# kakaoenterprise/JORLDY

Measured on AMD Instinct MI355X. Metric: env_steps_per_s (PPO CartPole sync, W=8 workers/GPU, T=128), higher is better.
Workload: dtype f32

## Files before the change

include/jorldy_hip.h:

```cpp
#ifndef JORLDY_HIP_H
#define JORLDY_HIP_H

#include <stdint.h>

#ifdef __cplusplus
extern "C" {
#endif

#define JH_ABI_VERSION 2

typedef enum {
  JH_OK = 0,
  JH_ERR_HIP = -1,
  JH_ERR_ARG = -2,
  JH_ERR_STATE = -3,
  JH_ERR_NOMEM = -4,
  JH_ERR_NODEVICE = -5
} jh_status;

typedef enum { JH_U8 = 0, JH_F32 = 1, JH_I64 = 2, JH_F64 = 3, JH_I32 = 4 } jh_dtype;

typedef struct jh_ctx jh_ctx;
typedef struct jh_store jh_store;
typedef struct jh_per jh_per;
// ... 89 lines not shown
                       const float* d_adv, const float* d_ret, const float* d_value_old, const float* d_logp_old, float eps_clip, float vf_coef,
                       float ent_coef, float* d_grad_heads, float* d_dv2, float* d_critic_sums, float* d_stats, jh_stream stream);
int jh_ppo_critic_select_strided(jh_ctx* ctx, int32_t B, const float* d_critic_sums, float vf_coef, float ent_coef, float* d_grad_value, int32_t ldv,
                                 const float* d_dv2, const float* d_stats_local, float* d_stats, jh_stream stream);
int jh_heads_unpack(jh_ctx* ctx, int64_t rows, int32_t A, const float* d_packed, int32_t ld, float* d_h0, float* d_h1, float* d_value, jh_stream stream);
int jh_policy_act_discrete(jh_ctx* ctx, int32_t W, int32_t A, const float* d_heads, int32_t ld, uint64_t seed, uint64_t counter, int32_t training,
                           int64_t* d_action, jh_stream stream);

#define JH_TD_DOUBLE 1
#define JH_TD_PER 2
int jh_td_loss(jh_ctx* ctx, int32_t B, int32_t A, int32_t n_step, int32_t flags, const float* d_q,
               const float* d_q_next_online, const float* d_q_next_target, const float* d_action,
               const float* d_reward, const float* d_done, const float* d_weights, float gamma, float alpha,
               float* d_grad_q, float* d_prio, float* d_stats, jh_stream stream);

int jh_mdqn_loss(jh_ctx* ctx, int32_t B, int32_t A, const float* d_q, const float* d_q_target, const float* d_q_next_target,
                 const float* d_action, const float* d_reward, const float* d_done, float gamma, float alpha, float tau, float l_0,
                 float* d_grad_q, float* d_stats, jh_stream stream);

#define JH_C51_DOUBLE 1
#define JH_C51_PER 2
#define JH_C51_SHIFT_MAX 4
int jh_c51_loss(jh_ctx* ctx, int32_t B, int32_t A, int32_t K, int32_t n_step, int32_t flags, const float* d_logit,
                const float* d_next_logit_online, const float* d_target_logit, const float* d_action,
                const float* d_reward, const float* d_done, const float* d_weights, float v_min, float v_max,
                float gamma, float alpha, float* d_grad_logit, float* d_prio, float* d_kl, float* d_stats,
                jh_stream stream);

int jh_value_act(jh_ctx* ctx, int32_t N, int32_t A, int32_t K, const float* d_logits, float v_min, float v_max,
                 const float* h_eps, const double* h_u, const int64_t* h_rand_action, int64_t* d_action,
                 float* d_q_taken, float* d_q_all, jh_stream stream);

int jh_qr_loss(jh_ctx* ctx, int32_t B, int32_t A, int32_t N, const float* d_logit, const float* d_next_logit_online,
               const float* d_target_logit, const float* d_action, const float* d_reward, const float* d_done,
               const float* d_tau, float gamma, float* d_grad_logit, float* d_stats, jh_stream stream);

int jh_quantile_act(jh_ctx* ctx, int32_t R, int32_t A, int32_t N, const float* d_logits, const float* h_eps, const double* h_u,
                    const int64_t* h_rand_action, int64_t* d_action, float* d_q_taken, float* d_q_all, jh_stream stream);

typedef struct jh_iqnnet jh_iqnnet;
int64_t jh_iqnnet_param_count_for(int32_t state_size, int32_t hidden, int32_t embedding_dim, int32_t num_sample, int32_t action_size);
int jh_iqnnet_create(jh_ctx* ctx, int32_t state_size, int32_t hidden, int32_t embedding_dim, int32_t num_sample, int32_t action_size,
                     int32_t max_batch, float* d_params, float* d_target, float* d_grads, float* d_m, float* d_v, jh_iqnnet** out);
void jh_iqnnet_destroy(jh_iqnnet* n);
int32_t jh_iqnnet_segment_count(void);
int jh_iqnnet_segment(const jh_iqnnet* n, int32_t i, int64_t* offset, int32_t* rows, int32_t* cols);
int jh_iqnnet_set_hyper(jh_iqnnet* n, double lr, double beta1, double beta2, double eps, int64_t step, jh_stream stream);
int jh_iqnnet_set_lr(jh_iqnnet* n, double lr, jh_stream stream);
int jh_iqnnet_sync_target(jh_iqnnet* n, jh_stream stream);
int jh_iqnnet_forward(jh_iqnnet* n, int32_t which, const float* d_x, int32_t rows, const float* d_tau, float* d_logits, jh_stream stream);
int jh_iqnnet_learn_forward(jh_iqnnet* n, const float* d_x, int32_t B, const float* d_tau, float* d_logits, jh_stream stream);
int jh_iqnnet_learn_forward_m(jh_iqnnet* n, const float* d_x, int32_t B, const float* d_tau, float* d_logits, jh_stream stream);
int jh_iqnnet_backward(jh_iqnnet* n, const float* d_g, jh_stream stream);
int jh_iqnnet_optim_step(jh_iqnnet* n, float max_norm, jh_stream stream);
int jh_iqn_cos_features(jh_ctx* ctx, int64_t rows, int32_t E, const float* d_tau, float* d_out, jh_stream stream);
int jh_iqn_hadamard(jh_ctx* ctx, int32_t B, int32_t N, int32_t H, const float* d_psi, const float* d_phi, float* d_out, jh_stream stream);
int jh_iqn_hadamard_backward(jh_ctx* ctx, int32_t B, int32_t N, int32_t H, const float* d_grad_embed, const float* d_psi, const float* d_phi,
                             float* d_grad_phi_pre, float* d_grad_psi_pre, jh_stream stream);
int jh_iqn_loss(jh_ctx* ctx, int32_t B, int32_t A, int32_t N, const float* d_logit, const float* d_next_logit_online,
                const float* d_target_logit, const float* d_action, const float* d_reward, const float* d_done, const float* d_tau,
                float gamma, float* d_grad_logit, float* d_stats, jh_stream stream);
int jh_miqn_loss(jh_ctx* ctx, int32_t B, int32_t A, int32_t N, const float* d_logit, const float* d_logit_again, const float* d_target_logit,
                 const float* d_action, const float* d_reward, const float* d_done, const float* d_tau, float gamma, float alpha, float tau_e,
                 float l_0, float* d_grad_logit, float* d_stats, jh_stream stream);
int jh_iqn_act(jh_ctx* ctx, int32_t R, int32_t A, int32_t N, const float* d_logits, const float* h_eps, const double* h_u,
               const int64_t* h_rand_action, int64_t* d_action, float* d_q_taken, float* d_q_all, jh_stream stream);

typedef struct jh_pponet jh_pponet;
int64_t jh_pponet_param_count(int32_t S, int32_t H, int32_t A, int32_t continuous);
int jh_pponet_create(jh_ctx* ctx, int32_t S, int32_t H, int32_t A, int32_t continuous, int32_t max_rows,
                     float* d_params, float* d_grads, float* d_m, float* d_v, uint64_t seed, jh_pponet** out);
void jh_pponet_destroy(jh_pponet* n);
int jh_pponet_set_hyper(jh_pponet* n, double lr, double beta1, double beta2, double eps, double step, jh_stream stream);
int jh_pponet_set_lr(jh_pponet* n, double lr, jh_stream stream);
int jh_pponet_forward(jh_pponet* n, int32_t B, const float* d_x, const int64_t* d_idx, float* d_head0,
                      float* d_head1, float* d_value, jh_stream stream);
int jh_pponet_backward(jh_pponet* n, int32_t B, const float* d_x, const int64_t* d_idx, const float* d_g_head0,
                       const float* d_g_head1, const float* d_g_value, jh_stream stream);
int jh_pponet_adam_step(jh_pponet* n, float max_norm, float* d_norm_out, jh_stream stream);
int jh_pponet_ppo_update(jh_pponet* n, int32_t B, const float* d_x, const int64_t* d_idx, const float* d_action,
                         const float* d_adv, const float* d_ret, const float* d_value_old, const float* d_logp_old,
                         float eps_clip, float vf_coef, float ent_coef, float max_norm, int32_t do_adam, float* d_stats,
                         jh_stream stream);
int jh_pponet_ppo_update_rows(jh_pponet* n, int32_t B, const float* d_x, const int64_t* d_idx, const float* d_action, const float* d_adv, const float* d_ret,
                              const float* d_value_old, const float* d_logp_old, float eps_clip, float vf_coef, float ent_coef, float max_norm,
                              int32_t do_adam, float* d_stats, jh_stream stream);
int jh_pponet_ppo_update_dp_begin(jh_pponet* n, int32_t B, const float* d_x, const int64_t* d_idx, const float* d_action, const float* d_adv,
                                  const float* d_ret, const float* d_value_old, const float* d_logp_old, float eps_clip, float vf_coef,
                                  float ent_coef, float* d_critic_sums, jh_stream stream);
int jh_pponet_ppo_update_dp_end(jh_pponet* n, int32_t B, const float* d_x, const int64_t* d_idx, const float* d_critic_sums, float vf_coef,
                                float ent_coef, float* d_stats, jh_stream stream);
struct jh_peer;
int jh_pponet_ppo_update_dp_end_peer(jh_pponet* n, struct jh_peer* peer, int32_t B, const float* d_x, const int64_t* d_idx, float* d_critic_sums,
                                     float vf_coef, float ent_coef, float* d_stats, jh_stream stream);
void* jh_pponet_hyper_ptr(jh_pponet* n);
int jh_pponet_act_rng(jh_pponet* n, uint64_t* seed, uint64_t* counter, int32_t set);
int jh_pponet_act_discrete(jh_pponet* n, int32_t W, const float* h_obs, int64_t* h_action, float* h_logits_out,
                           float* h_value_out, int32_t training, jh_stream stream);
int jh_pponet_act_continuous(jh_pponet* n, int32_t W, const float* h_obs, float* h_action, float* h_mu_raw_out,
                             float* h_log_std_raw_out, float* h_value_out, int32_t training, jh_stream stream);

int jh_cartpole_create(int32_t W, uint64_t seed, jh_cartpole** out);
void jh_cartpole_destroy(jh_cartpole* e);
int jh_cartpole_obs(const jh_cartpole* e, float* h_obs );
int jh_cartpole_step(jh_cartpole* e, const int64_t* h_action , float* h_next_obs ,
                     float* h_reward , uint8_t* h_done );

typedef struct jh_control jh_control;
int jh_control_create(int32_t W, int32_t S, int32_t A, uint64_t seed, jh_control** out);
void jh_control_destroy(jh_control* e);
int jh_control_obs(const jh_control* e, float* h_obs );
int jh_control_step(jh_control* e, const float* h_action , float* h_next_obs ,
                    float* h_reward , uint8_t* h_done );

typedef struct jh_collector jh_collector;

typedef struct jh_env_vtbl {
  int32_t W, S, A, continuous;
  int (*obs)(void* env, int32_t r0, int32_t r1, float* h_obs);
  int (*step)(void* env, int32_t r0, int32_t r1, const void* h_action, float* h_next_obs, float* h_reward, uint8_t* h_done);
  void* (*fork_alloc)(void* env, int32_t rows);
  void (*fork_free)(void* scratch);
  void (*copy_row)(void* dst, int32_t di, const void* src, int32_t si);
} jh_env_vtbl;
int jh_collector_create_env(jh_ctx* ctx, jh_pponet* net, const jh_env_vtbl* vt, void* env, jh_store* store, const int32_t* cols,
                            jh_collector** out);

int jh_collector_create(jh_ctx* ctx, jh_pponet* net, jh_cartpole* env, jh_store* store, const int32_t* cols,
                        jh_collector** out);
int jh_collector_create_control(jh_ctx* ctx, jh_pponet* net, jh_control* env, jh_store* store, const int32_t* cols,
                                jh_collector** out);
void jh_collector_destroy(jh_collector* c);
int jh_collector_run(jh_collector* c, int32_t T, int32_t training, jh_stream stream);
int jh_collector_set_capture(jh_collector* c, float* d_h0, float* d_h1, float* d_value, float* d_next_value, int64_t rows);
int jh_collector_begin(jh_collector* c, int32_t T, jh_stream stream);
int jh_collector_loop(jh_collector* c, int32_t training, jh_stream stream);
int jh_collector_set_ride_along(jh_collector* c, int32_t slot, const void* d_src_mapped, void* d_dst, int64_t bytes);
int jh_collector_prelaunch(jh_collector* c, int32_t T, jh_stream stream);
int jh_collector_stats(jh_collector* c, double* act_us_per_step, double* env_us_per_step, int32_t reset);
int jh_collector_stats_detail(jh_collector* c, double* out6);

int jh_normal_fill(jh_ctx* ctx, int64_t n, float* d_out, uint64_t* d_state, jh_stream stream);

typedef struct jh_rbnet jh_rbnet;
int64_t jh_rbnet_param_count_for(int32_t kind, int32_t head_cnn, int32_t channels_or_state_size, int32_t height, int32_t width,
                                 int32_t hidden, int32_t action_size, int32_t num_support);
int jh_rbnet_create(jh_ctx* ctx, int32_t kind, int32_t head_cnn, int32_t channels_or_state_size, int32_t height, int32_t width,
                    int32_t hidden, int32_t action_size, int32_t num_support, int32_t max_batch, float* d_params,
                    float* d_target, float* d_grads, float* d_m, float* d_v, jh_rbnet** out);
void jh_rbnet_destroy(jh_rbnet* n);
int64_t jh_rbnet_param_count(const jh_rbnet* n);
int32_t jh_rbnet_segment_count(void);
int jh_rbnet_segment(const jh_rbnet* n, int32_t i, int64_t* offset, int32_t* rows, int32_t* cols);
int64_t jh_rbnet_noise_len(const jh_rbnet* n);
int jh_rbnet_set_hyper(jh_rbnet* n, double lr, double beta1_or_alpha, double beta2, double eps, int64_t step, int32_t centered,
                       jh_stream stream);
int jh_rbnet_set_lr(jh_rbnet* n, double lr, jh_stream stream);
int jh_rbnet_sync_target(jh_rbnet* n, jh_stream stream);
int jh_rbnet_forward(jh_rbnet* n, int32_t which, const void* d_x, int32_t x_dtype, int32_t rows, const float* d_noise,
                     float* d_logits, jh_stream stream);
int jh_rbnet_forward_keep(jh_rbnet* n, const void* d_x, int32_t x_dtype, int32_t B, float* d_logits, jh_stream stream);
int jh_rbnet_learn_forward(jh_rbnet* n, const void* d_x, int32_t x_dtype, int32_t B, const float* d_noise, float* d_logits,
                           jh_stream stream);
int jh_rbnet_reserve_target_rows(jh_rbnet* n, int32_t rows);
int jh_rbnet_learn_forward_m(jh_rbnet* n, const void* d_x, int32_t x_dtype, int32_t B, const float* d_noise, float* d_logits,
                             jh_stream stream);
// ... 75 lines not shown
```

jorldy_amd/_lib.py:

```python
import ctypes as C
import os

_HERE = os.path.dirname(os.path.abspath(__file__))
LIB_PATH = os.path.join(_HERE, "csrc", "libjorldy_hip.so")

JH_U8, JH_F32, JH_I64, JH_F64, JH_I32 = 0, 1, 2, 3, 4
JH_TD_DOUBLE, JH_TD_PER = 1, 2
JH_C51_DOUBLE, JH_C51_PER, JH_C51_SHIFT_MAX = 1, 2, 4


class JhError(RuntimeError):
    pass


class ColDesc(C.Structure):
    _fields_ = [("dtype", C.c_int32), ("elems", C.c_int64)]


_vp, _i32, _i64, _f32, _f64 = C.c_void_p, C.c_int32, C.c_int64, C.c_float, C.c_double
_pp = C.POINTER(C.c_void_p)

_PROTOS = {
    "jh_abi_version": (C.c_int, []),
    "jh_stream_abort_capture": (C.c_int, [_vp]),
# ... 3 lines not shown
    "jh_ctx_destroy": (None, [_vp]),
    "jh_ctx_sync": (C.c_int, [_vp, _vp]),
    "jh_ctx_local_cpulist": (C.c_int, [_vp, C.c_char_p, _i64]),
    "jh_prof_enable": (C.c_int, [_i32]),
    "jh_prof_report": (C.c_int, [C.c_char_p, _i64]),
    "jh_prof_calibrate": (C.c_int, [_i32, _vp]),
    "jh_calib_stream": (C.c_int, [_vp, _vp, _i64, _i32, _vp, _vp]),
    "jh_host_wait_marks": (C.c_int, [_vp, _vp, _i32, _f32, _f64]),
    "jh_host_wait_words": (C.c_int, [_vp, _vp, _i32, C.c_uint32, _f64]),
    "jh_np_legacy_shuffles": (C.c_int, [_vp, _vp, _vp, _i64, _i32, _vp]),
    "jh_pinned_alloc": (C.c_int, [_vp, _i64, _pp, _pp]),
    "jh_pinned_free": (None, [_vp]),
    "jh_store_create": (C.c_int, [_vp, _i64, _i32, C.POINTER(ColDesc), _pp]),
    "jh_store_destroy": (None, [_vp]),
    "jh_store_push": (C.c_int, [_vp, _i64, _pp, _vp]),
    "jh_store_push_device": (C.c_int, [_vp, _i64, _pp, _vp]),
    "jh_store_stage_begin": (C.c_int, [_vp, _i64, _pp]),
    "jh_store_stage_commit": (C.c_int, [_vp, _vp]),
    "jh_store_write_rows": (C.c_int, [_vp, _i64, _vp, _pp, _vp]),
    "jh_store_gather": (C.c_int, [_vp, _i64, _vp, _i64, _i32, C.POINTER(_i32), _pp, C.POINTER(_i32), _vp]),
    "jh_store_col_ptr": (_vp, [_vp, _i32]),
    "jh_store_size": (_i64, [_vp]),
    "jh_store_index": (_i64, [_vp]),
    "jh_store_capacity": (_i64, [_vp]),
    "jh_store_clear": (None, [_vp]),
    "jh_store_set_position": (C.c_int, [_vp, _i64, _i64]),
    "jh_per_create": (C.c_int, [_vp, _i64, _f64, _pp]),
    "jh_per_destroy": (None, [_vp]),
    "jh_per_push": (C.c_int, [_vp, _i64, _vp, _vp]),
    "jh_per_push_device": (C.c_int, [_vp, _i64, _vp, _vp]),
    "jh_per_update": (C.c_int, [_vp, _i64, _vp, _vp, _i32, _vp]),
    "jh_per_sample": (C.c_int, [_vp, _i64, _f64, _i64, _vp, _vp, _vp, _vp, _vp, _vp, _vp]),
    "jh_per_state": (C.c_int, [_vp, C.POINTER(_f64), C.POINTER(_f64), C.POINTER(_i64), C.POINTER(_i64), _vp]),
    "jh_per_tree_ptr": (_vp, [_vp]),
    "jh_per_shard_stats": (C.c_int, [_vp, _i64, _vp, _vp]),
    "jh_per_weights_sharded": (C.c_int, [_vp, _i64, _f64, _vp, _i32, _vp, _vp, _vp]),
    "jh_per_tree_size": (_i64, [_vp]),
    "jh_per_load": (C.c_int, [_vp, _vp, _f64, _i64, _i64]),
    "jh_per_dump": (C.c_int, [_vp, _vp, _vp]),
    "jh_gae": (C.c_int, [_vp, _i32, _i32, _f32, _f32, _vp, _vp, _vp, _vp, _vp, _vp, _i32, _vp]),
    "jh_ppo_minibatch_rows": (C.c_int, [_vp, _i64, _vp, _i32, _vp, _vp, _vp, _vp]),
    "jh_mean_f32": (C.c_int, [_vp, _i64, _vp, _vp, _vp]),
    "jh_logp_discrete": (C.c_int, [_vp, _i64, _i32, _vp, _vp, _vp, _vp]),
    "jh_logp_continuous": (C.c_int, [_vp, _i64, _i32, _vp, _vp, _vp, _vp, _vp]),
    "jh_ppo_loss_discrete": (C.c_int, [_vp, _i32, _i32, _vp, _vp, _vp, _vp, _vp, _vp, _vp, _vp, _f32, _f32, _f32, _vp, _vp, _vp, _vp]),
    "jh_ppo_loss_continuous": (C.c_int, [_vp, _i32, _i32, _vp, _vp, _vp, _vp, _vp, _vp, _vp, _vp, _vp, _f32, _f32, _f32, _vp, _vp, _vp, _vp, _vp]),
    "jh_normal_fill": (C.c_int, [_vp, _i64, _vp, _vp, _vp]),
    "jh_value_act": (C.c_int, [_vp, _i32, _i32, _i32, _vp, _f32, _f32, _vp, _vp, _vp, _vp, _vp, _vp, _vp]),
    "jh_td_loss": (C.c_int, [_vp, _i32, _i32, _i32, _i32, _vp, _vp, _vp, _vp, _vp, _vp, _vp, _f32, _f32, _vp, _vp, _vp, _vp]),
    "jh_c51_loss": (C.c_int, [_vp, _i32, _i32, _i32, _i32, _i32, _vp, _vp, _vp, _vp, _vp, _vp, _vp, _f32, _f32, _f32, _f32, _vp, _vp, _vp, _vp, _vp]),
    "jh_mdqn_loss": (C.c_int, [_vp, _i32, _i32, _vp, _vp, _vp, _vp, _vp, _vp, _f32, _f32, _f32, _f32, _vp, _vp, _vp]),
    "jh_qr_loss": (C.c_int, [_vp, _i32, _i32, _i32, _vp, _vp, _vp, _vp, _vp, _vp, _vp, _f32, _vp, _vp, _vp]),
    "jh_quantile_act": (C.c_int, [_vp, _i32, _i32, _i32, _vp, _vp, _vp, _vp, _vp, _vp, _vp, _vp]),
    "jh_iqnnet_param_count_for": (_i64, [_i32, _i32, _i32, _i32, _i32]),
    "jh_iqnnet_create": (C.c_int, [_vp, _i32, _i32, _i32, _i32, _i32, _i32, _vp, _vp, _vp, _vp, _vp, _pp]),
    "jh_iqnnet_destroy": (None, [_vp]),
    "jh_iqnnet_segment_count": (_i32, []),
    "jh_iqnnet_segment": (C.c_int, [_vp, _i32, C.POINTER(_i64), C.POINTER(_i32), C.POINTER(_i32)]),
    "jh_iqnnet_set_hyper": (C.c_int, [_vp, _f64, _f64, _f64, _f64, _i64, _vp]),
    "jh_iqnnet_set_lr": (C.c_int, [_vp, _f64, _vp]),
    "jh_iqnnet_sync_target": (C.c_int, [_vp, _vp]),
    "jh_iqnnet_forward": (C.c_int, [_vp, _i32, _vp, _i32, _vp, _vp, _vp]),
    "jh_iqnnet_learn_forward": (C.c_int, [_vp, _vp, _i32, _vp, _vp, _vp]),
    "jh_iqnnet_learn_forward_m": (C.c_int, [_vp, _vp, _i32, _vp, _vp, _vp]),
    "jh_iqnnet_backward": (C.c_int, [_vp, _vp, _vp]),
    "jh_iqnnet_optim_step": (C.c_int, [_vp, _f32, _vp]),
    "jh_iqn_cos_features": (C.c_int, [_vp, _i64, _i32, _vp, _vp, _vp]),
    "jh_iqn_hadamard": (C.c_int, [_vp, _i32, _i32, _i32, _vp, _vp, _vp, _vp]),
    "jh_iqn_hadamard_backward": (C.c_int, [_vp, _i32, _i32, _i32, _vp, _vp, _vp, _vp, _vp, _vp]),
    "jh_iqn_loss": (C.c_int, [_vp, _i32, _i32, _i32, _vp, _vp, _vp, _vp, _vp, _vp, _vp, _f32, _vp, _vp, _vp]),
    "jh_miqn_loss": (C.c_int, [_vp, _i32, _i32, _i32, _vp, _vp, _vp, _vp, _vp, _vp, _vp, _f32, _f32, _f32, _f32, _vp, _vp, _vp]),
    "jh_iqn_act": (C.c_int, [_vp, _i32, _i32, _i32, _vp, _vp, _vp, _vp, _vp, _vp, _vp, _vp]),
    "jh_pponet_param_count": (_i64, [_i32, _i32, _i32, _i32]),
    "jh_pponet_create": (C.c_int, [_vp, _i32, _i32, _i32, _i32, _i32, _vp, _vp, _vp, _vp, C.c_uint64, _pp]),
    "jh_pponet_destroy": (None, [_vp]),
    "jh_pponet_set_hyper": (C.c_int, [_vp, _f64, _f64, _f64, _f64, _f64, _vp]),
    "jh_pponet_set_lr": (C.c_int, [_vp, _f64, _vp]),
    "jh_pponet_hyper_ptr": (_vp, [_vp]),
    "jh_pponet_act_rng": (C.c_int, [_vp, C.POINTER(C.c_uint64), C.POINTER(C.c_uint64), _i32]),
    "jh_pponet_forward": (C.c_int, [_vp, _i32, _vp, _vp, _vp, _vp, _vp, _vp]),
    "jh_pponet_backward": (C.c_int, [_vp, _i32, _vp, _vp, _vp, _vp, _vp, _vp]),
    "jh_pponet_adam_step": (C.c_int, [_vp, _f32, _vp, _vp]),
    "jh_pponet_ppo_update": (C.c_int, [_vp, _i32, _vp, _vp, _vp, _vp, _vp, _vp, _vp, _f32, _f32, _f32, _f32, _i32, _vp, _vp]),
    "jh_pponet_ppo_update_rows": (C.c_int, [_vp, _i32, _vp, _vp, _vp, _vp, _vp, _vp, _vp, _f32, _f32, _f32, _f32, _i32, _vp, _vp]),
    "jh_ppo_loss_deferred": (C.c_int, [_vp, _i32, _i32, _i32, _vp, _vp, _vp, _vp, _vp, _vp, _vp, _vp, _vp, _f32, _f32, _f32, _vp, _vp, _vp, _vp, _vp, _vp, _vp]),
    "jh_ppo_loss_packed": (C.c_int, [_vp, _i32, _i32, _i32, _vp, _i32, _vp, _vp, _vp, _vp, _vp, _vp, _f32, _f32, _f32, _vp, _vp, _vp, _vp, _vp]),
    "jh_ppo_critic_select_strided": (C.c_int, [_vp, _i32, _vp, _f32, _f32, _vp, _i32, _vp, _vp, _vp, _vp]),
    "jh_heads_unpack": (C.c_int, [_vp, _i64, _i32, _vp, _i32, _vp, _vp, _vp, _vp]),
    "jh_policy_act_discrete": (C.c_int, [_vp, _i32, _i32, _vp, _i32, C.c_uint64, C.c_uint64, _i32, _vp, _vp]),
    "jh_ppo_critic_select_rows": (C.c_int, [_vp, _i32, _vp, _f32, _f32, _vp, _vp, _vp, _vp, _vp]),
    "jh_pponet_ppo_update_dp_begin": (C.c_int, [_vp, _i32, _vp, _vp, _vp, _vp, _vp, _vp, _vp, _f32, _f32, _f32, _vp, _vp]),
    "jh_pponet_ppo_update_dp_end": (C.c_int, [_vp, _i32, _vp, _vp, _vp, _f32, _f32, _vp, _vp]),
    "jh_pponet_ppo_update_dp_end_peer": (C.c_int, [_vp, _vp, _i32, _vp, _vp, _vp, C.c_float, C.c_float, _vp, _vp]),
    "jh_pponet_act_discrete": (C.c_int, [_vp, _i32, _vp, _vp, _vp, _vp, _i32, _vp]),
    "jh_pponet_act_continuous": (C.c_int, [_vp, _i32, _vp, _vp, _vp, _vp, _vp, _i32, _vp]),
    "jh_control_create": (C.c_int, [_i32, _i32, _i32, C.c_uint64, _pp]),
    "jh_control_destroy": (None, [_vp]),
    "jh_control_obs": (C.c_int, [_vp, _vp]),
    "jh_control_step": (C.c_int, [_vp, _vp, _vp, _vp, _vp]),
    "jh_collector_create_control": (C.c_int, [_vp, _vp, _vp, _vp, C.POINTER(_i32), _pp]),
    "jh_collector_create": (C.c_int, [_vp, _vp, _vp, _vp, C.POINTER(_i32), _pp]),
    "jh_collector_create_env": (C.c_int, [_vp, _vp, _vp, _vp, _vp, C.POINTER(_i32), _pp]),
    "jh_collector_destroy": (None, [_vp]),
    "jh_rbnet_param_count_for": (_i64, [_i32, _i32, _i32, _i32, _i32, _i32, _i32, _i32]),
    "jh_rbnet_create": (C.c_int, [_vp, _i32, _i32, _i32, _i32, _i32, _i32, _i32, _i32, _i32, _vp, _vp, _vp, _vp, _vp, _pp]),
    "jh_rbnet_destroy": (None, [_vp]),
    "jh_rbnet_param_count": (_i64, [_vp]),
    "jh_rbnet_segment_count": (_i32, []),
    "jh_rbnet_segment": (C.c_int, [_vp, _i32, C.POINTER(_i64), C.POINTER(_i32), C.POINTER(_i32)]),
    "jh_rbnet_noise_len": (_i64, [_vp]),
    "jh_rbnet_set_hyper": (C.c_int, [_vp, _f64, _f64, _f64, _f64, _i64, _i32, _vp]),
    "jh_rbnet_optim_step": (C.c_int, [_vp, _i32, _f32, _vp]),
    "jh_rbnet_set_lr": (C.c_int, [_vp, _f64, _vp]),
    "jh_rbnet_sync_target": (C.c_int, [_vp, _vp]),
    "jh_rbnet_forward": (C.c_int, [_vp, _i32, _vp, _i32, _i32, _vp, _vp, _vp]),
    "jh_rbnet_forward_keep": (C.c_int, [_vp, _vp, _i32, _i32, _vp, _vp]),
    "jh_rbnet_learn_forward": (C.c_int, [_vp, _vp, _i32, _i32, _vp, _vp, _vp]),
    "jh_rbnet_learn_forward_m": (C.c_int, [_vp, _vp, _i32, _i32, _vp, _vp, _vp]),
    "jh_rbnet_reserve_target_rows": (C.c_int, [_vp, _i32]),
    "jh_rbnet_prepare_noise": (C.c_int, [_vp, _vp, _vp]),
    "jh_rbnet_learn_trunk": (C.c_int, [_vp, _vp, _i32, _i32, _vp]),
    "jh_rbnet_learn_heads": (C.c_int, [_vp, _i32, _vp, _vp, _vp]),
    "jh_rbnet_backward": (C.c_int, [_vp, _vp, _vp]),
    "jh_rbnet_backward_deferred": (C.c_int, [_vp, _vp, _vp]),
    "jh_rbnet_flush_grads": (C.c_int, [_vp, _vp]),
    "jh_rbnet_learn_heads_raw": (C.c_int, [_vp, _i32, _vp, _vp]),
    "jh_rbnet_c51_step": (C.c_int, [_vp, _vp, _i32, _i32, _i32, _vp, _vp, _vp, _vp, _vp, _f32, _f32, _f32, _f32, _vp, _vp, _vp, _vp, _vp]),
    "jh_rbnet_adam_step": (C.c_int, [_vp, _vp]),
    "jh_tgemm_dense": (C.c_int, [_vp, _i32, _i32, _i32, _vp, _i32, _i32, _vp, _i32, _i32, _vp, _i32, _i32, _vp, _vp, _i32, _vp, _vp]),
    "jh_tgemm_dense_group": (C.c_int, [_vp, _i32, _i32, _i32, _i32, _vp, _vp, _vp, _vp]),
    "jh_tgemm_set_cfg": (C.c_int, [C.c_char_p]),
    "jh_ring_create": (C.c_int, [_vp, _i64, _i32, C.POINTER(ColDesc), _i32, _pp]),
    "jh_ring_destroy": (None, [_vp]),
    "jh_ring_produce": (C.c_int, [_vp, _i64, _pp, _vp, _i32]),
    "jh_ring_drain": (C.c_int, [_vp, _vp, _vp, _i64, _vp, C.POINTER(_i64)]),
    "jh_ring_consume_host": (C.c_int, [_vp, _i64, _pp, _vp, C.POINTER(_i64)]),
    "jh_ring_reclaim": (C.c_int, [_vp, _i32]),
    "jh_ring_stats": (C.c_int, [_vp, C.POINTER(_i64), C.POINTER(_i64), C.POINTER(_f64)]),
    "jh_feed_create": (C.c_int, [_vp, _i32, _i32, _i64, _i32, _f32, _i64, _i64, _pp]),
    "jh_feed_destroy": (None, [_vp]),
    "jh_feed_tick": (C.c_int, [_vp, _vp, _vp, _vp, _vp, _vp, _vp, _vp, _f64, _vp, _vp, _vp, _vp, _vp, _vp, C.POINTER(_i32), _vp]),
    "jh_feed_push_stacks": (C.c_int, [_vp, _vp, _vp, _vp, _vp]),
    "jh_feed_push_frames": (C.c_int, [_vp, _vp, _vp, _vp, _vp, _vp]),
    "jh_feed_emit": (C.c_int, [_vp, _vp, _vp, _vp, _vp, _f64, _vp, _vp, _vp, _vp, _vp, _vp, C.POINTER(_i32), _vp]),
    "jh_feed_state": (C.c_int, [_vp, C.POINTER(_i32), C.POINTER(_i64), _vp]),
    "jh_feed_state_bytes": (_i64, [_vp]),
    "jh_feed_save": (C.c_int, [_vp, _vp, _i64, _vp]),
    "jh_feed_load": (C.c_int, [_vp, _vp, _i64, _vp]),
    "jh_collector_stats": (C.c_int, [_vp, C.POINTER(_f64), C.POINTER(_f64), _i32]),
    "jh_collector_run": (C.c_int, [_vp, _i32, _i32, _vp]),
    "jh_collector_stats_detail": (C.c_int, [_vp, C.POINTER(_f64)]),
    "jh_collector_set_capture": (C.c_int, [_vp, _vp, _vp, _vp, _vp, _i64]),
    "jh_collector_prelaunch": (C.c_int, [_vp, _i32, _vp]),
    "jh_collector_begin": (C.c_int, [_vp, _i32, _vp]),
    "jh_collector_loop": (C.c_int, [_vp, _i32, _vp]),
    "jh_collector_set_ride_along": (C.c_int, [_vp, _i32, _vp, _vp, _i64]),
    "jh_cartpole_create": (C.c_int, [_i32, C.c_uint64, _pp]),
    "jh_cartpole_destroy": (None, [_vp]),
    "jh_cartpole_obs": (C.c_int, [_vp, _vp]),
    "jh_cartpole_step": (C.c_int, [_vp, _vp, _vp, _vp, _vp]),
    "jh_comm_unique_id": (C.c_int, [_vp]),
    "jh_comm_create": (C.c_int, [_vp, _i32, _i32, _vp, _pp]),
    "jh_comm_destroy": (None, [_vp]),
    "jh_comm_info": (C.c_int, [_vp, C.POINTER(_i32), C.POINTER(_i32)]),
    "jh_comm_allreduce_mean_f32": (C.c_int, [_vp, _vp, _i64, _vp]),
    "jh_comm_broadcast": (C.c_int, [_vp, _vp, _i64, _i32, _vp]),
# ... 74 lines not shown
```

jorldy_amd/core/agent/ppo.py:

```python
import os

import numpy as np
import torch

from ... import np_rng, ops
from ..buffer import RolloutBuffer
from ..network import Network
from ..optimizer import Optimizer
from .base import BaseAgent


MAX_HEAD_OUTPUTS = 40
NATIVE_ELIGIBLE = ("PPO runs on libjorldy_hip only: network in {discrete_policy_value, continuous_policy_value}, head='mlp', int state_size, "
                   "hidden_size % 16 == 0, optim_config name 'adam' without weight_decay / amsgrad, and action_size + 1 (discrete) or "
                   f"2 * action_size + 1 (continuous) <= {MAX_HEAD_OUTPUTS} head outputs (config.ppo.cartpole, config.ppo.mujoco on all its envs; up to 8 outputs "
                   "-- CartPole, Hopper -- on the four-launch minibatch update and the persistent acting kernel, beyond that on the separate calls / the tiled engine); "
                   "head='cnn' with a (C, H, W) state_size and network 'discrete_policy_value' runs on the convolutional engine (core/agent/ppo_cnn.py: config.ppo.atari, ppo.procgen)")


class PPO(BaseAgent):

    def __new__(cls, *args, **kwargs):
        if cls is PPO and kwargs.get("head", args[4] if len(args) > 4 else "mlp") == "cnn":
            from .ppo_cnn import PPOConv
# ... 149 lines not shown
        if os.environ.get("JH_PPO_MAPPED_STATS", "1") == "1":
            pin = ops.PinnedBuffer((n_upd + 1, 8), np.float32, self.device.index)
            pin.np[:] = 0.0
            st["stats_pin"] = pin
            st["stats"] = ops._wrap_device(pin.dev_ptr.value, (n_upd + 1, 8), torch.float32, self.device, owner=pin)
        E = self.n_epoch
        if self.fused_update and all(self._net.fused_ok(min(B, M - o)) for o in range(0, M, B)):
            srcs = [st["tr"]["state"], st["tr"]["action"], st["adv"], st["ret"], st["value"], st["logp_old"]]
            st["mb"] = [f(E * M, int(t.numel() // M)) for t in srcs]
            st["rows"] = ops.MinibatchRows(srcs, st["mb"])
        st["idx_pin"] = [ops.PinnedBuffer((self.n_epoch * M,), np.int64, self.device.index) for _ in range(2)]
        st["idx_alias"] = [ops._wrap_device(p.dev_ptr.value, (self.n_epoch * M,), torch.int64, self.device, owner=p) for p in st["idx_pin"]]
        st["idx_ev"] = [None, None]
        st["idx_k"] = 0
        st["idx_ready"] = False
        self._stats = st["stats"]
        return st

    def _capture_targets(self, M):
        self._grow_native(2 * M if 2 * M <= 8192 else M)
        if self._static is None or self._static["M"] != M:
            self._drop_rides()
            self._static, self._graphs = self._alloc_static(M), {}
        st = self._static
        return st["h0"], st["h1"], st["value"], st["next_value"]

    def _drop_rides(self):
        if self._ride is not None:
            self._ride.clear_rides()
        self._ride_wait.clear()
        if self._static is not None:
            self._static["idx_ready"] = False

    def _upload_idx(self, st, draw, ride=False):
        k = st["idx_k"]
        st["idx_k"] = 1 - k
        if st["idx_ev"][k] is not None:
            st["idx_ev"][k].synchronize()
            st["idx_ev"][k] = None
        ok = draw(st["idx_pin"][k].np)
        if ok is False:
            return False
        if ride and self._ride is not None:
            self._ride.ride_along(0, st["idx_pin"][k].dev_ptr.value, st["idx"].data_ptr(), st["idx"].numel() * 8, keep=(st["idx_pin"][k], st["idx"]))
            self._ride_wait["idx"] = k
            return True
        self._ride_wait.pop("idx", None)
        st["idx"].copy_(st["idx_alias"][k])
        ev = torch.cuda.Event()
        ev.record()
        st["idx_ev"][k] = ev
        return True

    def _enqueue_learn(self, st):
        self._enqueue_pre(st)
        self._enqueue_main(st)

    def _enqueue_pre(self, st, captured=False):
        net, M = self._net, st["M"]
        cont = net.cont
        tr = st["tr"]
        self.memory._store.gather(st["arange"], as_float=True, out={k: tr[k] for k in tr})
        if captured:
            pass
        elif 2 * M <= min(net.max_rows, 8192):
            net.forward(st["x_all"], out=(st["h0_all"], st["h1_all"], st["v_all"]))
        else:
            net.forward(tr["next_state"], out=(st["nh0"], st["nh1"], st["next_value"]))
            net.forward(tr["state"], out=(st["h0"], st["h1"], st["value"]))
        if cont:
            logp_old = ops.logp_continuous(st["h0"], st["h1"], tr["action"], out=st["logp_old"])
        else:
            logp_old = ops.logp_discrete(st["h0"], tr["action"], out=st["logp_old"])
        adv, ret = ops.gae(tr["reward"], tr["done"], st["value"], st["next_value"], self.n_step, self.gamma, self._lambda, self.use_standardization,
                           out=(st["adv"], st["ret"]))
        ops.mean_into(ret, st["stats"][st["n_upd"], 0:1])

    def _enqueue_main(self, st):
        net, M, B = self._net, st["M"], self.batch_size
        cont = net.cont
        tr, adv, ret, logp_old = st["tr"], st["adv"], st["ret"], st["logp_old"]
        k = 0
        if "rows" in st:
            xs, acts, advs, rets, vals, lps = st["rows"](st["idx"])
            exact = self.grad_sync is not None and self.dp_exact_critic
            if exact and "critic_sums" not in st:
                st["critic_sums"] = torch.zeros(st["n_upd"], 2, dtype=torch.float32, device=self.device)
            for e in range(self.n_epoch):
                for offset in range(0, M, B):
                    o0, o1 = e * M + offset, e * M + min(offset + B, M)
                    if exact:
                        net.ppo_update_dp(xs[o0:o1], None, acts[o0:o1], advs[o0:o1], rets[o0:o1], vals[o0:o1], lps[o0:o1], self.epsilon_clip, self.vf_coef,
                                          self.ent_coef, st["stats"][k], self.grad_sync.reduce_flat, st["critic_sums"][k],
                                          peer=getattr(getattr(self.grad_sync, "transport", None), "peer", None))
                    else:
                        net.ppo_update(xs[o0:o1], None, acts[o0:o1], advs[o0:o1], rets[o0:o1], vals[o0:o1], lps[o0:o1], self.epsilon_clip, self.vf_coef,
                                       self.ent_coef, self.clip_grad_norm, st["stats"][k], do_adam=self.grad_sync is None)
                    if self.grad_sync is not None:
                        self.grad_sync.reduce_flat(net.grads)
                        net.adam_step(self.clip_grad_norm)
                    k += 1
            return
        exact = self.grad_sync is not None and self.dp_exact_critic
        if exact and "dp_work" not in st:
            st["dp_work"] = torch.zeros(st["n_upd"], B + 16, dtype=torch.float32, device=self.device)
        onepass = not exact and os.environ.get("JH_PPO_ONEPASS", "1") == "1"
        for e in range(self.n_epoch):
            for offset in range(0, M, B):
                b = min(B, M - offset)
                idx = st["idx"][e * M + offset : e * M + offset + b]
                if onepass:
                    net.ppo_update_rows(tr["state"], idx, tr["action"], adv, ret, st["value"], logp_old, self.epsilon_clip, self.vf_coef, self.ent_coef, self.clip_grad_norm,
                                        st["stats"][k], do_adam=self.grad_sync is None)
                    if self.grad_sync is not None:
                        self.grad_sync.reduce_flat(net.grads)
                        net.adam_step(self.clip_grad_norm)
                    k += 1
                    continue
                if cont:
                    mu, ls, vp = net.forward(tr["state"], idx=idx, out=(st["mb_h0"][:b], st["mb_h1"][:b], st["mb_v"][:b]))
                    if exact:
                        g_mu, g_ls, g_v = ops.ppo_loss_dp(mu, ls, vp, idx, tr["action"], adv, ret, st["value"], logp_old, self.epsilon_clip, self.vf_coef, self.ent_coef,
                                                          st["stats"][k], self.grad_sync.reduce_flat, st["dp_work"][k])
                    else:
                        g_mu, g_ls, g_v, _ = ops.ppo_loss_continuous(mu, ls, vp, idx, tr["action"], adv, ret, st["value"], logp_old, self.epsilon_clip, self.vf_coef, self.ent_coef, stats=st["stats"][k])
                    net.backward(tr["state"], idx, g_mu, g_ls, g_v)
                else:
                    z, vp = net.forward(tr["state"], idx=idx, out=(st["mb_h0"][:b], None, st["mb_v"][:b]))
                    if exact:
                        g_z, g_v = ops.ppo_loss_dp(z, None, vp, idx, tr["action"], adv, ret, st["value"], logp_old, self.epsilon_clip, self.vf_coef, self.ent_coef,
                                                   st["stats"][k], self.grad_sync.reduce_flat, st["dp_work"][k])
                    else:
                        g_z, g_v, _ = ops.ppo_loss_discrete(z, vp, idx, tr["action"], adv, ret, st["value"], logp_old, self.epsilon_clip, self.vf_coef, self.ent_coef, stats=st["stats"][k])
                    net.backward(tr["state"], idx, g_z, None, g_v)
                if self.grad_sync is not None:
                    self.grad_sync.reduce_flat(net.grads)
                net.adam_step(self.clip_grad_norm)
                k += 1

    def _learn_native(self):
        self._learn_launch()
        return self._learn_finish()

    def early_ready(self):
        st = self._static
        return bool(st is not None and st["idx_ready"] and ("one", True) in getattr(self, "_graphs", {}) and self._predraw is not None and self._predraw.valid)

    def _learn_launch(self, allow_capture=True):
        M = self.memory.size
        self._grow_native(2 * M if 2 * M <= 8192 else M)
        if self._static is None or self._static["M"] != M:
            self._drop_rides()
            self._static, self._graphs = self._alloc_static(M), {}
        st = self._static
        E = self.n_epoch
        captured = self._captured == M
        self._captured = 0
        rode, self._ride_done = self._ride_done, False
        if self._ride_wait and not rode:
            if "lr" in self._ride_wait:
                self._net.set_lr(float(self._lr_word.np[0]))
            if "idx" in self._ride_wait and st["idx_ready"]:
                st["idx"].copy_(st["idx_alias"][self._ride_wait["idx"]])
        self._ride_wait.clear()

        def shuffles():
            self._upload_idx(st, lambda out: np_rng.epoch_shuffles(M, E, out))

        pin = st.get("stats_pin")
        if pin is not None:
            pin.np[st["n_upd"] - 1, 2] = -1.0
            pin.np[st["n_upd"] - 1, 7] = -1.0
        graphable = (self.use_graph and not ops._PROF["on"] and not ops._PROF["lib"] and not getattr(self, "_graph_failed", False)
                     and (self.grad_sync is None or (self.graph_with_collective and getattr(self.grad_sync, "capturable", True))))
        have_idx = bool(st["idx_ready"]) and self._predraw is not None and self._predraw.commit(M, E)
        st["idx_ready"] = False
        split = not have_idx and os.environ.get("JH_PPO_SPLIT_GRAPH", "1") == "1"
        key = ("split" if split else "one", captured)
        graphs = getattr(self, "_graphs", None)
        if graphs is None:
            graphs = self._graphs = {}
        warm = getattr(self, "_warm_keys", None)
        if warm is None:
            warm = self._warm_keys = set()
# ... 163 lines not shown
```

jorldy_amd/csrc/jh_common.h:

```cpp
#pragma once
#include <hip/hip_runtime.h>
#include <math.h>
#include <stdint.h>
#include <stdio.h>
#include <string.h>

#include <deque>
#include <mutex>
#include <string>
#include <vector>

#include "../../include/jorldy_hip.h"

#define JH_EXPORT extern "C" __attribute__((visibility("default")))

std::string& jh_err_slot();
int jh_fail(int code, const char* fmt, ...);

#define JH_HIP(expr)                                                                          \
  do {                                                                                        \
    hipError_t _e = (expr);                                                                   \
    if (_e != hipSuccess)                                                                     \
      return jh_fail(JH_ERR_HIP, "%s:%d %s -> %s", __FILE__, __LINE__, #expr, hipGetErrorString(_e)); \
  } while (0)
// ... 65 lines not shown
int jh_ctx_slab_release(jh_ctx* ctx, jh_pinned_slab* slab, hipStream_t stream);
int jh_ctx_scratch(jh_ctx* ctx, size_t bytes, void** out);
struct jh_draws {
  jh_pinned_slab* slab;
  const float* eps;
  const double* u;
  const int64_t* rand_action;
};
int jh_ctx_stage_draws(jh_ctx* ctx, size_t rows, const float* h_eps, const double* h_u, const int64_t* h_rand_action, jh_draws* out);

struct jh_store {
  jh_ctx* ctx = nullptr;
  int64_t capacity = 0;
  int n_cols = 0;
  std::vector<jh_col_desc> cols;
  std::vector<void*> dev;
  std::vector<size_t> row_bytes;
  int64_t index = 0;
  int64_t counter = 0;
  jh_pinned_slab* staged = nullptr;
  int64_t staged_n = 0;
  std::vector<size_t> staged_off;
};

int jh_store_append(jh_store* s, int64_t n, const void* const* cols, hipMemcpyKind kind, hipStream_t st);
int jh_store_stage_commit_extra(jh_store* s, int n_extra, const void* const* x_src, void* const* x_dst, const int64_t* x_bytes, hipStream_t st);
bool jh_store_commit_is_one_launch(const jh_store* s, int64_t n);
int jh_store_stage_abort(jh_store* s, hipStream_t st);
int jh_store_stage_commit_gated(jh_store* s, int n_extra, const void* const* x_src, void* const* x_dst, const int64_t* x_bytes, const unsigned* gate,
                                unsigned gate_val, hipStream_t st);

struct jh_cartpole {
  int W = 0;
  std::vector<double> s;
  std::vector<int64_t> t;
  std::vector<uint64_t> rng;
};

struct jh_control {
  int W = 0, S = 0, A = 0;
  std::vector<double> s;
  std::vector<int64_t> t;
  std::vector<uint64_t> rng;
};

void jh_cartpole_obs_rows(const jh_cartpole* e, int r0, int r1, float* h_obs);
void jh_cartpole_step_rows(jh_cartpole* e, int r0, int r1, const int64_t* h_action, float* h_next_obs, float* h_reward, uint8_t* h_done);
struct jh_control;
void jh_control_obs_rows(const jh_control* e, int r0, int r1, float* h_obs);
void jh_control_step_rows(jh_control* e, int r0, int r1, const float* h_action, float* h_next_obs, float* h_reward, uint8_t* h_done);

struct jh_pponet {
  jh_ctx* ctx = nullptr;
  int S = 0, H = 0, A = 0, cont = 0, max_rows = 0;
  int n_out = 0;
  int gld = 8;
  int64_t n_params = 0;
  float *params = nullptr, *grads = nullptr, *m = nullptr, *v = nullptr;
  int64_t o_w1, o_b1, o_w2, o_b2, o_wh0, o_bh0, o_wh1, o_bh1, o_wv, o_bv;
  float *h1 = nullptr, *h2 = nullptr, *dh1 = nullptr, *dh2 = nullptr;
  float* g_all = nullptr;
  float* dv2 = nullptr;
  float* stats_tmp = nullptr;
  int max_act_rows = 0;
  float *obs_pin_h = nullptr, *obs_pin_d = nullptr;
  float *part_pin_h = nullptr, *part_pin_d = nullptr;
  unsigned *flag_pin_h = nullptr, *flag_pin_d = nullptr;
  unsigned act_seq = 0;
  float *act_out_h = nullptr, *act_out_d = nullptr;
  uint64_t act_seed = 0, act_ctr = 0;
  float* fwd_part = nullptr;
  float* part_w1 = nullptr;
  float* ssq_part = nullptr;
  float* norm_partial = nullptr;
  int norm_slots = 0;
  float* hyper = nullptr;
  float* upd_ws = nullptr;
  size_t upd_floats = 0;
  float* xg = nullptr;
  float* tg_ws = nullptr;
  size_t tg_ws_floats = 0;
  unsigned* tg_cnt = nullptr;
  int tg_cnt_slots = 0;
};

static inline uint64_t jh_mix64(uint64_t x) {
  x += 0x9E3779B97F4A7C15ull;
  x = (x ^ (x >> 30)) * 0xBF58476D1CE4E5B9ull;
  x = (x ^ (x >> 27)) * 0x94D049BB133111EBull;
  return x ^ (x >> 31);
}
static inline double jh_u01_of(uint64_t key) { return (double)(jh_mix64(key) >> 11) * (1.0 / 9007199254740992.0); }

static inline int64_t jh_sample_discrete(const jh_pponet* n, const float* z, int wq, int training) {
  const int A = n->A;
  int act = 0;
  float mx = z[0];
  for (int k = 1; k < A; ++k)
    if (z[k] > mx) { mx = z[k]; act = k; }
  if (!training) return act;
  float e[40], se = 0.f;
  for (int k = 0; k < A; ++k) { e[k] = expf(z[k] - mx); se += e[k]; }
  const float u = (float)jh_u01_of(n->act_seed * 0x100000001B3ull + n->act_ctr * 0x9E3779B97F4A7C15ull + (uint64_t)wq) * se;
  float c = 0.f;
  act = A - 1;
  for (int k = 0; k < A; ++k) {
    c += e[k];
    if (u < c) { act = k; break; }
  }
  return act;
}

static inline void jh_sample_continuous(const jh_pponet* n, const float* z, int wq, int training, float* action) {
  const int A = n->A;
  for (int k = 0; k < A; ++k) {
    const float mu = fminf(fmaxf(z[k], -5.f), 5.f);
    float v = mu;
    if (training) {
      const float sd = expf(tanhf(z[A + k]));
      const uint64_t key = n->act_seed * 0x100000001B3ull + n->act_ctr * 0x9E3779B97F4A7C15ull + (uint64_t)wq * 64u + (uint64_t)k;
      const double u1 = 1.0 - jh_u01_of(key * 2 + 1), u2 = jh_u01_of(key * 2 + 2);
      v = mu + sd * (float)(sqrt(-2.0 * log(u1)) * cos(6.283185307179586 * u2));
    }
    action[k] = tanhf(v);
  }
}

enum {
  JH_HY_LR = 0, JH_HY_B1 = 1, JH_HY_B2 = 2, JH_HY_EPS = 3, JH_HY_STEP = 4,
  JH_HY_BC1 = 5,
  JH_HY_BC2S = 6,
  JH_HY_OMB1 = 7,
  JH_HY_OMB2 = 8,
  JH_HY_B1D = 10,
  JH_HY_B2D = 12,
  JH_HY_FLOATS = 16
};
static inline void jh_hyper_fill(float* h, double lr, double beta1, double beta2, double eps, double step) {
  h[JH_HY_LR] = (float)lr; h[JH_HY_B1] = (float)beta1; h[JH_HY_B2] = (float)beta2; h[JH_HY_EPS] = (float)eps; h[JH_HY_STEP] = (float)step;
  h[JH_HY_BC1] = 0.f; h[JH_HY_BC2S] = 0.f;
  h[JH_HY_OMB1] = (float)(1.0 - beta1); h[JH_HY_OMB2] = (float)(1.0 - beta2); h[9] = 0.f;
  memcpy(h + JH_HY_B1D, &beta1, 8); memcpy(h + JH_HY_B2D, &beta2, 8);
  h[14] = h[15] = 0.f;
}

#ifdef __HIPCC__
__device__ __forceinline__ void jh_adam_bias_corrections(const float* hyper, float t, float& bc1, float& bc2s) {
  const double b1 = *reinterpret_cast<const double*>(hyper + JH_HY_B1D), b2 = *reinterpret_cast<const double*>(hyper + JH_HY_B2D);
  bc1 = (float)(1.0 - pow(b1, (double)t));
  bc2s = (float)sqrt(1.0 - pow(b2, (double)t));
}
__device__ __forceinline__ void jh_adam_advance(float* hyper) {
  const float t = hyper[JH_HY_STEP] + 1.f;
  float bc1, bc2s;
  jh_adam_bias_corrections(hyper, t, bc1, bc2s);
  hyper[JH_HY_STEP] = t;
  hyper[JH_HY_BC1] = bc1;
  hyper[JH_HY_BC2S] = bc2s;
}
__device__ __forceinline__ float jh_wave_sum(float v) {
#pragma unroll
  for (int o = 32; o > 0; o >>= 1) v += __shfl_xor(v, o, 64);
  return v;
}
__device__ __forceinline__ double jh_wave_sum(double v) {
#pragma unroll
  for (int o = 32; o > 0; o >>= 1) v += __shfl_xor(v, o, 64);
  return v;
}
__device__ __forceinline__ float jh_wave_max(float v) {
#pragma unroll
  for (int o = 32; o > 0; o >>= 1) v = fmaxf(v, __shfl_xor(v, o, 64));
  return v;
}
__device__ __forceinline__ float jh_wave_min(float v) {
#pragma unroll
  for (int o = 32; o > 0; o >>= 1) v = fminf(v, __shfl_xor(v, o, 64));
  return v;
}
__device__ __forceinline__ double jh_wave_max(double v) {
#pragma unroll
  for (int o = 32; o > 0; o >>= 1) v = fmax(v, __shfl_xor(v, o, 64));
  return v;
}
template <typename T, typename Op>
__device__ __forceinline__ T jh_block_reduce(T v, T* red, Op op, T ident) {
  const int lane = threadIdx.x & 63, wid = threadIdx.x >> 6, nw = (blockDim.x + 63) >> 6;
#pragma unroll
  for (int o = 32; o > 0; o >>= 1) v = op(v, __shfl_xor(v, o, 64));
  __syncthreads();
  if (lane == 0) red[wid] = v;
  __syncthreads();
  T r = ident;
  for (int w = 0; w < nw; ++w) r = op(r, red[w]);
  return r;
}
struct JhAdd { template <typename T> __device__ T operator()(T a, T b) const { return a + b; } };
struct JhMax { template <typename T> __device__ T operator()(T a, T b) const { return a > b ? a : b; } };
struct JhMin { template <typename T> __device__ T operator()(T a, T b) const { return a < b ? a : b; } };
#endif
```

jorldy_amd/csrc/jh_mlp.hip:

```cpp
#include "jh_ppo_mb.h"
#include "jh_tgemm.h"
#include "jh_ppo_finish.h"

typedef float f32x4 __attribute__((ext_vector_type(4)));

namespace {
constexpr int kNormBlocks = 256;
constexpr int kNormSlots = kNormBlocks + 256;
constexpr int kMaxHeadOutputs = 40;
}

constexpr int kL1Rows = 16;
__global__ void __launch_bounds__(256) jh_mlp_l1_kernel(int B, int S, int H, const float* __restrict__ x,
                                                        const int64_t* __restrict__ idx, const float* __restrict__ W1,
                                                        const float* __restrict__ b1, float* __restrict__ h1) {
  __shared__ __attribute__((aligned(16))) float sx[kL1Rows][16];
  const int jb = (H + 255) / 256;
  const int rb = blockIdx.x / jb, j = (blockIdx.x - rb * jb) * 256 + threadIdx.x;
  const int b0 = rb * kL1Rows, nb = b0 + kL1Rows < B ? kL1Rows : B - b0;
  const bool lds_rows = S <= 16;
  if (lds_rows) {
    const int rr = threadIdx.x >> 4, sc = threadIdx.x & 15;
    float v = 0.f;
    if (rr < nb && sc < S) {
// ... 351 lines not shown
  if (!on && !(dv2 && fin.partial)) return;
  const int b = on ? (int)(i4 / h4) : 0, k = on ? 4 * (int)(i4 - (int64_t)b * h4) : 0;
  float gv[8];
  float4 w[8];
#pragma unroll
  for (int o = 0; o < 8; ++o) {
    gv[o] = hf.g[o][(size_t)b * hf.ld[o]];
    w[o] = *reinterpret_cast<const float4*>(hf.w[o] + k);
  }
  if (dv2) {
    float w1, w2;
    const float g2 = dv2[b];
    if (fin.partial) {
      float t[6];
      ppo_reduce_partials_wave(fin.partial, fin.nb, t);
      ppo_finish_stats(t[0], t[1], t[2], t[3], t[4], t[5], fin.B, fin.ent_count, fin.vf, fin.ent, w1, w2, (blockIdx.x == 0 && threadIdx.x == 0) ? fin.stats : nullptr);
    } else {
      w1 = mix[0]; w2 = mix[1];
    }
    if (!on) return;
#pragma unroll
    for (int o = 0; o < 8; ++o)
      if (o == ov) gv[o] = w1 * gv[o] + w2 * g2;
  }
  float4 acc = first ? make_float4(0.f, 0.f, 0.f, 0.f) : *reinterpret_cast<const float4*>(dh2 + (size_t)b * H + k);
  const float4 hv = *reinterpret_cast<const float4*>(h2 + (size_t)b * H + k);
  float mine[4] = {0.f, 0.f, 0.f, 0.f};
#pragma unroll
  for (int o = 0; o < 8; ++o) {
    if (o < hf.n) {
      acc.x = fmaf(gv[o], w[o].x, acc.x); acc.y = fmaf(gv[o], w[o].y, acc.y); acc.z = fmaf(gv[o], w[o].z, acc.z); acc.w = fmaf(gv[o], w[o].w, acc.w);
#pragma unroll
      for (int j = 0; j < 4; ++j) mine[j] = (o0 + o == k + j) ? gv[o] : mine[j];
    }
  }
  if (last) acc = make_float4(hv.x > 0.f ? acc.x : 0.f, hv.y > 0.f ? acc.y : 0.f, hv.z > 0.f ? acc.z : 0.f, hv.w > 0.f ? acc.w : 0.f);
  *reinterpret_cast<float4*>(dh2 + (size_t)b * H + k) = acc;
  if (k < gld) {
    float* dst = g_all + (size_t)b * gld + k;
    if (first) {
      *reinterpret_cast<float4*>(dst) = make_float4(mine[0], mine[1], mine[2], mine[3]);
    } else {
#pragma unroll
      for (int j = 0; j < 4; ++j)
        if (k + j >= o0 && k + j < o0 + hf.n) dst[j] = mine[j];
    }
  }
  if (H < gld && k == H - 4) {
    for (int kk = H; kk < gld; kk += 4) {
      float* dst = g_all + (size_t)b * gld + kk;
#pragma unroll
      for (int j = 0; j < 4; ++j) {
        float v = 0.f;
#pragma unroll
        for (int o = 0; o < 8; ++o) v = (o < hf.n && o0 + o == kk + j) ? gv[o] : v;
        if (first || (kk + j >= o0 && kk + j < o0 + hf.n)) dst[j] = v;
      }
    }
  }
}

__global__ void __launch_bounds__(256) jh_gradnorm_kernel(int64_t n, const float* __restrict__ g,
                                                          float* __restrict__ partial, float* __restrict__ hyper) {
  __shared__ float s_red[16];
  float acc = 0.f;
  const int64_t stride = (int64_t)gridDim.x * 256;
  for (int64_t i0 = (int64_t)blockIdx.x * 256 + threadIdx.x; i0 < n; i0 += 8 * stride) {
    float v[8];
#pragma unroll
    for (int u = 0; u < 8; ++u) {
      const int64_t i = i0 + u * stride;
      v[u] = g[i < n ? i : i0];
    }
#pragma unroll
    for (int u = 0; u < 8; ++u)
      if (i0 + u * stride < n) acc = fmaf(v[u], v[u], acc);
  }
  acc = jh_block_reduce(acc, s_red, JhAdd(), 0.f);
  if (threadIdx.x == 0) partial[blockIdx.x] = acc;
  if (blockIdx.x == 0 && threadIdx.x == 0) jh_adam_advance(hyper);
}

template <bool FUSED>
__global__ void __launch_bounds__(256) jh_adam_kernel(int64_t n, float* __restrict__ p, float* __restrict__ g,
                                                      float* __restrict__ m, float* __restrict__ v,
                                                      const float* __restrict__ partial, int n_partial,
                                                      const float* __restrict__ hyper, float max_norm,
                                                      float* __restrict__ norm_out, const float* __restrict__ part,
                                                      int tiles_m, int64_t n_head) {
  __shared__ float s_red[16];
  const int64_t n4 = n >> 2;
  float4 *p4 = reinterpret_cast<float4*>(p), *g4 = reinterpret_cast<float4*>(g), *m4 = reinterpret_cast<float4*>(m), *v4 = reinterpret_cast<float4*>(v);
  const int64_t i_first = (int64_t)blockIdx.x * 256 + threadIdx.x;
  const int64_t i_fc = i_first < n4 ? i_first : 0;
  const float4 pp0 = p4[i_fc], mm0 = m4[i_fc], vv0 = v4[i_fc], gg0 = g4[i_fc];
  float acc = 0.f;
  bool partials_added = false;
  auto add_partials = [&]() {
    const int ia = threadIdx.x, ib = threadIdx.x + 256;
    const float pa = partial[ia < n_partial ? ia : 0], pb = partial[ib < n_partial ? ib : 0];
    acc += ia < n_partial ? pa : 0.f;
    acc += ib < n_partial ? pb : 0.f;
    for (int i = threadIdx.x + 512; i < n_partial; i += 256) acc += partial[i];
    partials_added = true;
  };
  float4 mine = make_float4(0.f, 0.f, 0.f, 0.f);
  const int64_t h4 = n_head >> 2;
  if (FUSED) {
    const float4* part4 = reinterpret_cast<const float4*>(part);
    constexpr int JU = 3, TU = 16;
    for (int64_t j0 = 0; j0 * 256 < h4; j0 += JU) {
      float4 w[JU][TU];
#pragma unroll
      for (int ju = 0; ju < JU; ++ju) {
        const int64_t i = threadIdx.x + 256 * (j0 + ju);
        const int64_t ic = i < h4 ? i : h4 - 1;
#pragma unroll
        for (int tu = 0; tu < TU; ++tu) w[ju][tu] = part4[(size_t)(tu < tiles_m ? tu : tiles_m - 1) * h4 + ic];
      }
      if (!partials_added) add_partials();
#pragma unroll
      for (int ju = 0; ju < JU; ++ju) {
        const int64_t i = threadIdx.x + 256 * (j0 + ju);
        float4 q = make_float4(0.f, 0.f, 0.f, 0.f);
#pragma unroll
        for (int tu = 0; tu < TU; ++tu)
          if (tu < tiles_m) { q.x += w[ju][tu].x; q.y += w[ju][tu].y; q.z += w[ju][tu].z; q.w += w[ju][tu].w; }
        if (i < h4) {
          acc = fmaf(q.x, q.x, acc); acc = fmaf(q.y, q.y, acc); acc = fmaf(q.z, q.z, acc); acc = fmaf(q.w, q.w, acc);
          if (j0 + ju == blockIdx.x) mine = q;
        }
      }
    }
  }
  if (!partials_added) add_partials();
  const float total = sqrtf(jh_block_reduce(acc, s_red, JhAdd(), 0.f));
  const float bc1 = hyper[5], bc2s = hyper[6];
  float coef = 1.f;
  if (max_norm > 0.f) coef = fminf(max_norm / (total + 1e-6f), 1.f);
  if (blockIdx.x == 0 && threadIdx.x == 0 && norm_out) *norm_out = total;
  const float lr = hyper[JH_HY_LR], b2 = hyper[JH_HY_B2], eps = hyper[JH_HY_EPS];
  const float omb1 = hyper[JH_HY_OMB1], omb2 = hyper[JH_HY_OMB2];
  const float step_size = lr / bc1;
  auto upd = [&](float& pi, float& gi_, float& mi_, float& vi_) {
    const float gi = gi_ * coef;
    gi_ = gi;
    const float mi = mi_ + omb1 * (gi - mi_);
    const float vi = vi_ * b2 + omb2 * gi * gi;
    mi_ = mi;
    vi_ = vi;
    const float denom = sqrtf(vi) / bc2s + eps;
    pi = pi - step_size * (mi / denom);
  };
  for (int64_t i = i_first; i < n4; i += (int64_t)gridDim.x * 256) {
    const bool first = i == i_first;
    float4 pp = first ? pp0 : p4[i], mm = first ? mm0 : m4[i], vv = first ? vv0 : v4[i];
    float4 gg = (FUSED && i < h4) ? mine : (first ? gg0 : g4[i]);
    upd(pp.x, gg.x, mm.x, vv.x); upd(pp.y, gg.y, mm.y, vv.y); upd(pp.z, gg.z, mm.z, vv.z); upd(pp.w, gg.w, mm.w, vv.w);
    p4[i] = pp; g4[i] = gg; m4[i] = mm; v4[i] = vv;
  }
  if (blockIdx.x == 0 && threadIdx.x < (int)(n - (n4 << 2))) {
    const int64_t i = (n4 << 2) + threadIdx.x;
    upd(p[i], g[i], m[i], v[i]);
  }
}

static int64_t pponet_layout(jh_pponet* n) {
  const int64_t S = n->S, H = n->H, A = n->A;
  int64_t o = 0;
  n->o_w1 = o; o += H * S;
  n->o_b1 = o; o += H;
  n->o_w2 = o; o += H * H;
  n->o_b2 = o; o += H;
  n->o_wh0 = o; o += A * H;
  n->o_bh0 = o; o += A;
  if (n->cont) {
    n->o_wh1 = o; o += A * H;
    n->o_bh1 = o; o += A;
  } else {
    n->o_wh1 = n->o_bh1 = -1;
  }
  n->o_wv = o; o += H;
  n->o_bv = o; o += 1;
  return o;
}

JH_EXPORT int64_t jh_pponet_param_count(int32_t S, int32_t H, int32_t A, int32_t continuous) {
  jh_pponet t;
  t.S = S; t.H = H; t.A = A; t.cont = continuous;
  return pponet_layout(&t);
}

JH_EXPORT int jh_pponet_create(jh_ctx* ctx, int32_t S, int32_t H, int32_t A, int32_t continuous, int32_t max_rows,
                               float* d_params, float* d_grads, float* d_m, float* d_v, uint64_t seed,
                               jh_pponet** out) {
  JH_ARG(ctx && out && d_params && d_grads && d_m && d_v);
  JH_ARG(S > 0 && A > 0 && max_rows > 0);
  JH_ARG(H >= 16 && H % 16 == 0);
  JH_ARG((continuous ? 2 * A + 1 : A + 1) <= kMaxHeadOutputs);
  JH_HIP(hipSetDevice(ctx->device));
  jh_pponet* n = new jh_pponet();
  n->ctx = ctx; n->S = S; n->H = H; n->A = A; n->cont = continuous ? 1 : 0; n->max_rows = max_rows;
  n->n_params = pponet_layout(n);
  n->params = d_params; n->grads = d_grads; n->m = d_m; n->v = d_v;
  const size_t act = sizeof(float) * (size_t)max_rows * (size_t)H;
  JH_HIP(hipMalloc((void**)&n->h1, act));
  JH_HIP(hipMalloc((void**)&n->h2, act));
  JH_HIP(hipMalloc((void**)&n->dh1, act));
  JH_HIP(hipMalloc((void**)&n->dh2, act));
  n->n_out = continuous ? 2 * A + 1 : A + 1;
  n->gld = n->n_out <= 8 ? 8 : (n->n_out + 3) / 4 * 4;
  JH_HIP(hipMalloc((void**)&n->g_all, sizeof(float) * (size_t)n->gld * (size_t)max_rows));
  n->max_act_rows = max_rows < 1024 ? max_rows : 1024;
  {
    const size_t tiles = (size_t)((n->max_act_rows + 15) / 16) * (size_t)(H / 16);
    JH_HIP(hipHostMalloc((void**)&n->obs_pin_h, sizeof(float) * (size_t)n->max_act_rows * (size_t)S, hipHostMallocMapped));
    JH_HIP(hipHostGetDevicePointer((void**)&n->obs_pin_d, n->obs_pin_h, 0));
    JH_HIP(hipHostMalloc((void**)&n->part_pin_h, sizeof(float) * 8 * (size_t)n->max_act_rows * (size_t)(H / 16), hipHostMallocMapped));
    JH_HIP(hipHostGetDevicePointer((void**)&n->part_pin_d, n->part_pin_h, 0));
    JH_HIP(hipHostMalloc((void**)&n->flag_pin_h, sizeof(unsigned) * tiles, hipHostMallocMapped));
    JH_HIP(hipHostGetDevicePointer((void**)&n->flag_pin_d, n->flag_pin_h, 0));
    memset(n->flag_pin_h, 0, sizeof(unsigned) * tiles);
    n->act_seed = seed;
    if (n->n_out > 8) {
      JH_HIP(hipHostMalloc((void**)&n->act_out_h, sizeof(float) * (size_t)n->max_act_rows * (size_t)n->n_out, hipHostMallocMapped));
      JH_HIP(hipHostGetDevicePointer((void**)&n->act_out_d, n->act_out_h, 0));
    }
  }
  n->tg_ws_floats = (size_t)4 << 20;
  n->tg_cnt_slots = 4096;
  JH_HIP(hipMalloc((void**)&n->xg, sizeof(float) * (size_t)max_rows * (size_t)S));
  JH_HIP(hipMalloc((void**)&n->tg_ws, sizeof(float) * n->tg_ws_floats));
  JH_HIP(hipMalloc((void**)&n->tg_cnt, sizeof(unsigned) * (size_t)n->tg_cnt_slots * kTgemmCntStride));
  JH_HIP(hipMemset(n->tg_cnt, 0, sizeof(unsigned) * (size_t)n->tg_cnt_slots * kTgemmCntStride));
  {
    const size_t part_bytes = sizeof(float) * 8 * (size_t)max_rows * (size_t)(H / 16);
    JH_HIP(hipMalloc((void**)&n->fwd_part, part_bytes));
    JH_HIP(hipMemset(n->fwd_part, 0, part_bytes));
    JH_HIP(hipMemset(n->g_all, 0, sizeof(float) * (size_t)n->gld * (size_t)max_rows));
    JH_HIP(hipMalloc((void**)&n->dv2, sizeof(float) * ((size_t)(max_rows < 1024 ? max_rows : 1024) + 8)));
    n->stats_tmp = n->dv2 + (max_rows < 1024 ? max_rows : 1024);
    const size_t slabs = (size_t)(((max_rows < 1024 ? max_rows : 1024) + 15) / 16);
    JH_HIP(hipMalloc((void**)&n->part_w1, sizeof(float) * slabs * ((size_t)H * S + H + 8 * (size_t)H)));
    JH_HIP(hipMalloc((void**)&n->ssq_part, sizeof(float) * ((size_t)(H / 32) * (H / 32) + H / 32 + 1)));
  }
  {
    const size_t rows = (size_t)max_rows, per = 4 * (size_t)A + 3;
    n->upd_floats = rows * per + 8 * ((rows + 255) / 256) + 16;
    JH_HIP(hipMalloc((void**)&n->upd_ws, sizeof(float) * n->upd_floats));
    JH_HIP(hipMemset(n->upd_ws, 0, sizeof(float) * n->upd_floats));
  }
  JH_HIP(hipMalloc((void**)&n->norm_partial, sizeof(float) * kNormSlots));
  JH_HIP(hipMalloc((void**)&n->hyper, sizeof(float) * JH_HY_FLOATS));
  float hy[JH_HY_FLOATS];
  jh_hyper_fill(hy, 1e-3, 0.9, 0.999, 1e-8, 0.0);
  JH_HIP(hipMemcpy(n->hyper, hy, sizeof(hy), hipMemcpyHostToDevice));
  *out = n;
  return JH_OK;
}

JH_EXPORT void jh_pponet_destroy(jh_pponet* n) {
  if (!n) return;
  (void)hipSetDevice(n->ctx->device);
  (void)hipDeviceSynchronize();
  (void)hipFree(n->h1); (void)hipFree(n->h2); (void)hipFree(n->dh1); (void)hipFree(n->dh2);
  (void)hipFree(n->g_all);
  (void)hipHostFree(n->obs_pin_h); (void)hipHostFree(n->part_pin_h); (void)hipHostFree(n->flag_pin_h);
  if (n->act_out_h) (void)hipHostFree(n->act_out_h);
  (void)hipFree(n->norm_partial); (void)hipFree(n->hyper); (void)hipFree(n->dv2);
  (void)hipFree(n->fwd_part); (void)hipFree(n->part_w1); (void)hipFree(n->ssq_part);
  (void)hipFree(n->tg_ws); (void)hipFree(n->tg_cnt); (void)hipFree(n->xg); (void)hipFree(n->upd_ws);
  delete n;
}

JH_EXPORT void* jh_pponet_hyper_ptr(jh_pponet* n) { return n ? (void*)n->hyper : nullptr; }

JH_EXPORT int jh_pponet_act_rng(jh_pponet* n, uint64_t* seed, uint64_t* counter, int32_t set) {
  JH_ARG(n && seed && counter);
  if (set) { n->act_seed = *seed; n->act_ctr = *counter; }
  else { *seed = n->act_seed; *counter = n->act_ctr; }
  return JH_OK;
}

JH_EXPORT int jh_pponet_set_hyper(jh_pponet* n, double lr, double beta1, double beta2, double eps, double step,
                                  jh_stream stream) {
  JH_ARG(n != nullptr);
  jh_pinned_slab* slab = nullptr;
  int rc = jh_ctx_slab(n->ctx, 64, &slab);
  if (rc) return rc;
  float* h = (float*)slab->host;
  jh_hyper_fill(h, lr, beta1, beta2, eps, step < 0 ? 0.0 : step);
  if (step >= 0) {
    JH_HIP(hipMemcpyAsync(n->hyper, h, sizeof(float) * JH_HY_FLOATS, hipMemcpyHostToDevice, jh_s(stream)));
  } else {
    JH_HIP(hipMemcpyAsync(n->hyper, h, sizeof(float) * 4, hipMemcpyHostToDevice, jh_s(stream)));
    JH_HIP(hipMemcpyAsync(n->hyper + JH_HY_OMB1, h + JH_HY_OMB1, sizeof(float) * (JH_HY_FLOATS - JH_HY_OMB1), hipMemcpyHostToDevice, jh_s(stream)));
  }
  return jh_ctx_slab_release(n->ctx, slab, jh_s(stream));
}

JH_EXPORT int jh_pponet_set_lr(jh_pponet* n, double lr, jh_stream stream) {
  JH_ARG(n != nullptr);
  jh_pinned_slab* slab = nullptr;
  int rc = jh_ctx_slab(n->ctx, 64, &slab);
  if (rc) return rc;
  *(float*)slab->host = (float)lr;
  JH_HIP(hipMemcpyAsync(n->hyper, slab->host, sizeof(float), hipMemcpyHostToDevice, jh_s(stream)));
  return jh_ctx_slab_release(n->ctx, slab, jh_s(stream));
}

static HeadPtrs head_ptrs(jh_pponet* n, float* out0, float* out1, float* outv, const float* g0, const float* g1,
                          const float* gv) {
  HeadPtrs hp{};
  int g = 0;
  hp.w[g] = n->params + n->o_wh0; hp.b[g] = n->params + n->o_bh0; hp.out[g] = out0; hp.g[g] = g0; hp.n[g] = n->A; ++g;
  if (n->cont) {
    hp.w[g] = n->params + n->o_wh1; hp.b[g] = n->params + n->o_bh1; hp.out[g] = out1; hp.g[g] = g1; hp.n[g] = n->A; ++g;
  }
  hp.w[g] = n->params + n->o_wv; hp.b[g] = n->params + n->o_bv; hp.out[g] = outv; hp.g[g] = gv; hp.n[g] = 1; ++g;
  hp.groups = g;
  return hp;
}

static HeadFlat head_flat(jh_pponet* n, const HeadPtrs& hp, int o0) {
  HeadFlat hf{};
  int o_flat = 0, k = 0;
  for (int g = 0; g < hp.groups; ++g)
    for (int o = 0; o < hp.n[g]; ++o, ++o_flat) {
      if (o_flat < o0 || k >= 8) continue;
      hf.w[k] = hp.w[g] + (size_t)o * n->H;
      hf.b[k] = hp.b[g] + o;
      hf.out[k] = hp.out[g] ? hp.out[g] + o : nullptr;
      hf.g[k] = hp.g[g] ? hp.g[g] + o : nullptr;
      hf.ld[k] = hp.n[g];
      ++k;
    }
  hf.n = k;
  for (; k < 8; ++k) {
    hf.w[k] = hf.w[0]; hf.b[k] = hf.b[0]; hf.out[k] = hf.out[0]; hf.g[k] = hf.g[0]; hf.ld[k] = hf.ld[0];
  }
  return hf;
}

static int head_rows(jh_pponet* n, const float** w, float** dw, const float** b, float** db) {
  int o = 0;
  for (int a = 0; a < n->A; ++a, ++o) {
    w[o] = n->params + n->o_wh0 + (int64_t)a * n->H; dw[o] = n->grads + n->o_wh0 + (int64_t)a * n->H;
    b[o] = n->params + n->o_bh0 + a; db[o] = n->grads + n->o_bh0 + a;
  }
  if (n->cont)
    for (int a = 0; a < n->A; ++a, ++o) {
      w[o] = n->params + n->o_wh1 + (int64_t)a * n->H; dw[o] = n->grads + n->o_wh1 + (int64_t)a * n->H;
      b[o] = n->params + n->o_bh1 + a; db[o] = n->grads + n->o_bh1 + a;
    }
  w[o] = n->params + n->o_wv; dw[o] = n->grads + n->o_wv; b[o] = n->params + n->o_bv; db[o] = n->grads + n->o_bv;
  return o + 1;
}

constexpr int kTiledRows = 1024;
static inline bool pponet_use_tiled(int B) { return B >= kTiledRows; }

static PmbHeads pmb_heads(jh_pponet* n) {
  PmbHeads hd{};
  hd.n_out = head_rows(n, hd.w, hd.dw, hd.b, hd.db);
  return hd;
}

__global__ void __launch_bounds__(256) jh_rowgather_f32_kernel(int B, int S, const float* __restrict__ x, const int64_t* __restrict__ idx, float* __restrict__ out) {
  const int64_t i = (int64_t)blockIdx.x * 256 + threadIdx.x;
  if (i >= (int64_t)B * S) return;
  const int b = (int)(i / S), s = (int)(i - (int64_t)b * S);
  out[i] = x[(idx ? idx[b] : (int64_t)b) * S + s];
}

constexpr int kNormFoldY = 8;
struct NormJob {
  const float* g;
  int64_t n;
  float* partial;
  int y0;
};
template <int SP>
__global__ void __launch_bounds__(256) jh_ppo_dw1_partial_kernel(int B, int H, int S, int rows_per, const float* __restrict__ dh1, const float* __restrict__ x,
                                                                 const int64_t* __restrict__ idx, float* __restrict__ partial, const float* __restrict__ h2,
                                                                 const float* __restrict__ g8, NormJob nj) {
  extern __shared__ float s_dyn[];
  if (nj.g && (int)blockIdx.y >= nj.y0) {
    const int id = ((int)blockIdx.y - nj.y0) * (int)gridDim.x + (int)blockIdx.x, nblk = kNormFoldY * (int)gridDim.x;
    float acc = 0.f;
    const int64_t stride = (int64_t)nblk * 256;
    for (int64_t i0 = (int64_t)id * 256 + threadIdx.x; i0 < nj.n; i0 += 8 * stride) {
      float v[8];
#pragma unroll
      for (int u = 0; u < 8; ++u) {
        const int64_t i = i0 + u * stride;
        v[u] = nj.g[i < nj.n ? i : i0];
      }
#pragma unroll
      for (int u = 0; u < 8; ++u)
        if (i0 + u * stride < nj.n) acc = fmaf(v[u], v[u], acc);
    }
    acc = jh_block_reduce(acc, s_dyn, JhAdd(), 0.f);
    if (threadIdx.x == 0) nj.partial[id] = acc;
    return;
  }
  const bool heads = h2 != nullptr;
  constexpr int NA = SP + 1 + 8;
  float* s_x = s_dyn;
  float* s_g = s_dyn + (size_t)rows_per * SP;
  float* s_acc = s_g + (size_t)rows_per * 8;
  const int hl = threadIdx.x & 63, rl = threadIdx.x >> 6;
  const int h = blockIdx.x * 64 + hl;
  const int z = blockIdx.y, b0 = z * rows_per;
  int nb = B - b0;
  if (nb > rows_per) nb = rows_per;
  constexpr int RU = 8;
  const int hc = h < H ? h : H - 1;
  const float* h2c = heads ? h2 : dh1;
  auto fetch = [&](int r0, float (&g)[RU], float (&a2)[RU]) {
#pragma unroll
    for (int u = 0; u < RU; ++u) {
      const int r = r0 + 4 * u;
      const int rc = r < nb ? r : nb - 1;
      g[u] = dh1[(size_t)(b0 + rc) * H + hc];
      a2[u] = h2c[(size_t)(b0 + rc) * H + hc];
    }
  };
  float gA[RU], aA[RU], gB[RU], aB[RU];
  fetch(rl, gA, aA);
  fetch(rl + 4 * RU, gB, aB);
  float* dummy = s_acc + threadIdx.x;
  const float4* g4 = (const float4*)((heads ? g8 : dh1) + (size_t)b0 * 8);
  const int ng = heads ? nb * 2 : 0;
  const float4 g_first = g4[(int)threadIdx.x < ng ? threadIdx.x : 0];
  __builtin_amdgcn_sched_barrier(0);
  {
    constexpr int SU = 4;
    const int nx = nb * SP;
    for (int i0 = threadIdx.x; i0 < nx; i0 += 256 * SU) {
      int64_t row[SU];
      int qq[SU];
#pragma unroll
      for (int u = 0; u < SU; ++u) {
        const int i = i0 + 256 * u;
        const int ic = i < nx ? i : nx - 1;
        const int r = ic / SP;
        qq[u] = ic - r * SP;
        row[u] = idx ? idx[b0 + r] : (int64_t)(b0 + r);
      }
// ... 107 lines not shown
    wrote = true;
    if (q < S) dW1[(size_t)h * S + q] = v;
    else if (q == S) db1[h] = v;
    else if (q - S - 1 < hg.n_out) hg.dw[q - S - 1][h] = v;
    else wrote = false;
  }
  if (ssq) {
    const float sq = jh_block_reduce(wrote ? v * v : 0.f, s_ssq, JhAdd(), 0.f);
    if (threadIdx.x == 0) ssq[blockIdx.x] = sq;
  }
}

static size_t pponet_dw1_plan(int B, int S, int* slabs_out, int* rows_per_out) {
  int slabs = (B + 63) / 64;
  if (slabs > 64) slabs = 64;
  const int rows_per = (B + slabs - 1) / slabs;
  slabs = (B + rows_per - 1) / rows_per;
  const int sp = (S + 3) / 4 * 4;
  if (slabs_out) *slabs_out = slabs;
  if (rows_per_out) *rows_per_out = rows_per;
  return sizeof(float) * ((size_t)rows_per * (sp + 8) + 4 * 64 * (size_t)(sp + 1 + 8));
}
static bool pponet_dw1_reduce_fits(int B, int S) { return S <= 16 && pponet_dw1_plan(B, S, nullptr, nullptr) <= 60 * 1024; }

static int pponet_dw1_reduce(jh_pponet* n, int B, const float* d_x, const int64_t* d_idx, bool heads, hipStream_t st, bool with_norm = false) {
  const int H = n->H, S = n->S;
  int slabs, rows_per;
  const size_t lds = pponet_dw1_plan(B, S, &slabs, &rows_per);
  const dim3 grid((unsigned)((H + 63) / 64), (unsigned)(slabs + (with_norm ? kNormFoldY : 0)));
  NormJob nj{};
  const int n_rest = kNormFoldY * (int)grid.x;
  if (with_norm) {
    nj.g = n->grads + n->o_w2; nj.n = (heads ? n->o_wh0 : n->n_params) - n->o_w2; nj.partial = n->norm_partial; nj.y0 = slabs;
  }
  const int sp = (S + 3) / 4 * 4;
  if (lds > 60 * 1024) return jh_fail(JH_ERR_ARG, "dW1 reduction: %zu bytes of LDS for %d rows per slab", lds, rows_per);
  HeadGradOut hg{};
  const float* h2 = nullptr;
  if (heads) {
    const float* w[8]; const float* b[8];
    hg.n_out = head_rows(n, w, hg.dw, b, hg.db);
    hg.g8 = n->g_all; hg.B = B;
    h2 = n->h2;
  }
  const double flops = 2.0 * B * (double)H * (S + 1 + (heads ? hg.n_out : 0));
  if (sp == 4) JH_LAUNCH_IDEM("jh_ppo_dw1_partial", flops, jh_ppo_dw1_partial_kernel<4>, grid, dim3(256), lds, st, B, H, S, rows_per, (const float*)n->dh1, d_x, d_idx, n->part_w1, h2, hg.g8, nj);
  else if (sp == 8) JH_LAUNCH_IDEM("jh_ppo_dw1_partial", flops, jh_ppo_dw1_partial_kernel<8>, grid, dim3(256), lds, st, B, H, S, rows_per, (const float*)n->dh1, d_x, d_idx, n->part_w1, h2, hg.g8, nj);
  else if (sp == 12) JH_LAUNCH_IDEM("jh_ppo_dw1_partial", flops, jh_ppo_dw1_partial_kernel<12>, grid, dim3(256), lds, st, B, H, S, rows_per, (const float*)n->dh1, d_x, d_idx, n->part_w1, h2, hg.g8, nj);
  else if (sp == 16) JH_LAUNCH_IDEM("jh_ppo_dw1_partial", flops, jh_ppo_dw1_partial_kernel<16>, grid, dim3(256), lds, st, B, H, S, rows_per, (const float*)n->dh1, d_x, d_idx, n->part_w1, h2, hg.g8, nj);
  else return jh_fail(JH_ERR_ARG, "dW1 reduction: observation width %d", S);
  JH_LAUNCH_CHECK();
  const int PS = S + 1 + (heads ? 8 : 0);
  const int n_comb = (H * PS + 255) / 256 + (heads ? 1 : 0);
  if (with_norm && n_rest + n_comb > kNormSlots) return jh_fail(JH_ERR_ARG, "dW1 reduction: %d norm slots", n_rest + n_comb);
  JH_LAUNCH(jh_ppo_dw1_combine_kernel, dim3((unsigned)n_comb), dim3(256), 0, st, H, S, slabs, (const float*)n->part_w1, n->grads + n->o_w1,
            n->grads + n->o_b1, hg, with_norm ? n->norm_partial + n_rest : nullptr, with_norm ? n->hyper : nullptr);
  JH_LAUNCH_CHECK();
  n->norm_slots = with_norm ? n_rest + n_comb : 0;
  return JH_OK;
}

static int pponet_l1(jh_pponet* n, int B, const float* d_x, const int64_t* d_idx, hipStream_t st) {
  const unsigned grid = (unsigned)(((B + kL1Rows - 1) / kL1Rows) * ((n->H + 255) / 256));
  JH_LAUNCH(jh_mlp_l1_kernel, dim3(grid), dim3(256), 0, st, B, n->S, n->H, d_x, d_idx,
            n->params + n->o_w1, n->params + n->o_b1, n->h1);
  JH_LAUNCH_CHECK();
  return JH_OK;
}

static int pponet_forward_partials(jh_pponet* n, int B, const float* d_x, const int64_t* d_idx, hipStream_t st) {
  const PmbHeads hd = pmb_heads(n);
  static const int gen_max = (getenv("JH_PMB_GEN16") && atoi(getenv("JH_PMB_GEN16")) == 1) ? 16 : 8;
  if (n->S <= gen_max) return jh_pmb_forward(n, B, d_x, d_idx, hd, nullptr, true, st);
  int rc = pponet_l1(n, B, d_x, d_idx, st);
  if (rc) return rc;
  return jh_pmb_forward(n, B, d_x, d_idx, hd, n->h1, true, st);
}

JH_EXPORT int jh_pponet_forward(jh_pponet* n, int32_t B, const float* d_x, const int64_t* d_idx, float* d_head0,
                                float* d_head1, float* d_value, jh_stream stream) {
  JH_ARG(n && d_x && d_head0 && d_value);
  JH_ARG(B > 0 && B <= n->max_rows);
  JH_ARG(!n->cont || d_head1);
  hipStream_t st = jh_s(stream);
  const int H = n->H;
  static const int kFwdTiledRows = getenv("JH_PPO_FWD_TILED_ROWS") ? atoi(getenv("JH_PPO_FWD_TILED_ROWS")) : 2048;
  if (jh_pmb_eligible(n, B) && B < kFwdTiledRows) {
    int rc = pponet_forward_partials(n, B, d_x, d_idx, st);
    if (rc) return rc;
    return jh_pmb_heads_finish(n, B, d_head0, d_head1, d_value, st);
  }
  int rc = pponet_l1(n, B, d_x, d_idx, st);
  if (rc) return rc;
  if (pponet_use_tiled(B)) {
    TGemm tg = mk_gemm(B, H, H, op_dense(OP_KCONT, n->h1, H), op_dense(OP_KCONT, n->params + n->o_w2, H), n->h2, H, TEPI_BIAS_RELU, n->params + n->o_b2);
    TGemmWorkspace tw;
    tw.ws = n->tg_ws; tw.ws_floats = n->tg_ws_floats; tw.cnt = n->tg_cnt; tw.cnt_slots = n->tg_cnt_slots;
    rc = jh_tgemm_launch(tw, "jh_tgemm_ppo_fwd_h2", &tg, 1, st);
  } else {
    GemmArgs g{};
    g.M = B; g.N = H; g.K = H; g.A = n->h1; g.lda = H; g.B = n->params + n->o_w2; g.ldb = H; g.C = n->h2; g.ldc = H;
    g.aux = n->params + n->o_b2;
    rc = launch_gemm<0, true, EPI_BIAS_RELU, false, 1, 1>("jh_gemm16_fwd_h2", g, st);
  }
  if (rc) return rc;
  HeadPtrs hp = head_ptrs(n, d_head0, d_head1, d_value, nullptr, nullptr, nullptr);
  for (int o0 = 0; o0 < n->n_out; o0 += 8) {
    JH_LAUNCH(jh_mlp_heads_fwd_kernel, dim3((B + 3) / 4), dim3(256), 0, st, B, H, n->h2, head_flat(n, hp, o0));
    JH_LAUNCH_CHECK();
  }
  return JH_OK;
}

static int pponet_backward(jh_pponet* n, int32_t B, const float* d_x, const int64_t* d_idx, const float* d_g_head0, const float* d_g_head1,
                           const float* d_g_value, const float* d_dv2, const float* d_mix, hipStream_t st, bool with_norm = false, const PpoFinish* fin = nullptr);
JH_EXPORT int jh_pponet_backward(jh_pponet* n, int32_t B, const float* d_x, const int64_t* d_idx,
                                 const float* d_g_head0, const float* d_g_head1, const float* d_g_value,
                                 jh_stream stream) {
  JH_ARG(n && d_x && d_g_head0 && d_g_value);
  JH_ARG(B > 0 && B <= n->max_rows);
  JH_ARG(!n->cont || d_g_head1);
  return pponet_backward(n, B, d_x, d_idx, d_g_head0, d_g_head1, d_g_value, nullptr, nullptr, jh_s(stream));
}
static int pponet_backward(jh_pponet* n, int32_t B, const float* d_x, const int64_t* d_idx, const float* d_g_head0, const float* d_g_head1,
                           const float* d_g_value, const float* d_dv2, const float* d_mix, hipStream_t st, bool with_norm, const PpoFinish* fin) {
  const int H = n->H, S = n->S;
  n->norm_slots = 0;
  const int64_t bh = (int64_t)B * H;
  HeadPtrs hp = head_ptrs(n, nullptr, nullptr, nullptr, d_g_head0, d_g_head1, d_g_value);
  for (int o0 = 0; o0 < n->n_out; o0 += 8) {
    const int ov = n->n_out - 1 - o0;
    JH_LAUNCH(jh_mlp_heads_bwd_dh_kernel, dim3((unsigned)((bh / 4 + 255) / 256)), dim3(256), 0, st, B, H, n->h2, n->dh2,
              n->g_all, head_flat(n, hp, o0), n->gld, o0, o0 == 0 ? 1 : 0, o0 + 8 >= n->n_out ? 1 : 0,
              (d_dv2 && ov >= 0 && ov < 8) ? d_dv2 : nullptr, d_mix, ov, fin ? *fin : PpoFinish{});
    JH_LAUNCH_CHECK();
  }
  const float* w[kMaxHeadOutputs]; float* dw[kMaxHeadOutputs]; const float* b[kMaxHeadOutputs]; float* db[kMaxHeadOutputs];
  const int n_out = head_rows(n, w, dw, b, db);
  const int gld = n->gld;
  int rc;
  if (pponet_use_tiled(B)) {
    const int A = n->A;
    TGemm g[6];
    int ng = 0;
    (void)n_out;
    g[ng++] = mk_gemm(H, H, B, op_dense(OP_XCONT, n->dh2, H), op_dense(OP_XCONT, n->h1, H), n->grads + n->o_w2, H, TEPI_NONE, nullptr, nullptr, 0, n->grads + n->o_b2);
    g[ng++] = mk_gemm(B, H, H, op_dense(OP_KCONT, n->dh2, H), op_dense(OP_XCONT, n->params + n->o_w2, H), n->dh1, H, TEPI_MASK, nullptr, n->h1, H);
    static const bool kDw1Gemm = getenv("JH_PPO_DW1_GEMM") && atoi(getenv("JH_PPO_DW1_GEMM")) != 0;
    const bool reduce = !kDw1Gemm && pponet_dw1_reduce_fits(B, S);
    const bool reduce_heads = reduce && n->n_out <= 8;
    if (!reduce_heads) {
      g[ng++] = mk_gemm(A, H, B, op_dense(OP_XCONT, n->g_all, gld), op_dense(OP_XCONT, n->h2, H), n->grads + n->o_wh0, H, TEPI_NONE, nullptr, nullptr, 0, n->grads + n->o_bh0);
      int col = A;
      if (n->cont) {
        g[ng++] = mk_gemm(A, H, B, op_dense(OP_XCONT, n->g_all + col, gld), op_dense(OP_XCONT, n->h2, H), n->grads + n->o_wh1, H, TEPI_NONE, nullptr, nullptr, 0, n->grads + n->o_bh1);
        col += A;
      }
      g[ng++] = mk_gemm(1, H, B, op_dense(OP_XCONT, n->g_all + col, gld), op_dense(OP_XCONT, n->h2, H), n->grads + n->o_wv, H, TEPI_NONE, nullptr, nullptr, 0, n->grads + n->o_bv);
    }
    TGemmWorkspace tw;
    tw.ws = n->tg_ws; tw.ws_floats = n->tg_ws_floats; tw.cnt = n->tg_cnt; tw.cnt_slots = n->tg_cnt_slots;
    rc = jh_tgemm_launch(tw, "jh_tgemm_ppo_bwd", g, ng, st);
    if (rc) return rc;
    if (reduce) return pponet_dw1_reduce(n, B, d_x, d_idx, reduce_heads, st, with_norm);
    JH_LAUNCH(jh_rowgather_f32_kernel, dim3((unsigned)(((int64_t)B * S + 255) / 256)), dim3(256), 0, st, B, S, d_x, d_idx, n->xg);
    JH_LAUNCH_CHECK();
    g[0] = mk_gemm(H, S, B, op_dense(OP_XCONT, n->dh1, H), op_dense(OP_XCONT, n->xg, S), n->grads + n->o_w1, S, TEPI_NONE, nullptr, nullptr, 0, n->grads + n->o_b1);
    return jh_tgemm_launch(tw, "jh_tgemm_ppo_bwd_dW1", g, 1, st);
  }
  for (int o0 = 0; o0 < n_out; o0 += 8) {
    GemmArgs g{};
    g.M = n_out - o0 < 8 ? n_out - o0 : 8; g.N = H; g.K = B; g.A = n->g_all + o0; g.lda = gld; g.B = n->h2; g.ldb = H;
    for (int o = 0; o < g.M; ++o) { g.rowptr[o] = dw[o0 + o]; g.rowsum_ptr[o] = db[o0 + o]; }
    rc = launch_gemm<1, false, EPI_ROWPTR, true, 1, 1>("jh_gemm16_bwd_dWheads", g, st);
    if (rc) return rc;
  }
  {
    GemmArgs g{};
    g.M = H; g.N = H; g.K = B; g.A = n->dh2; g.lda = H; g.B = n->h1; g.ldb = H; g.C = n->grads + n->o_w2; g.ldc = H;
    g.rowsum = n->grads + n->o_b2;
    rc = launch_gemm<1, false, EPI_NONE, true, 1, 1>("jh_gemm16_bwd_dW2", g, st);
    if (rc) return rc;
  }
  {
    GemmArgs g{};
    g.M = B; g.N = H; g.K = H; g.A = n->dh2; g.lda = H; g.B = n->params + n->o_w2; g.ldb = H; g.C = n->dh1; g.ldc = H;
    g.aux = n->h1; g.ldaux = H;
    rc = launch_gemm<0, false, EPI_MASK, false, 1, 1>("jh_gemm16_bwd_dh1", g, st);
    if (rc) return rc;
  }
  {
    GemmArgs g{};
    g.M = H; g.N = S; g.K = B; g.A = n->dh1; g.lda = H; g.B = d_x; g.ldb = S; g.b_rows = d_idx;
    g.C = n->grads + n->o_w1; g.ldc = S; g.rowsum = n->grads + n->o_b1;
    rc = launch_gemm<1, false, EPI_NONE, true, 1, 1>("jh_gemm16_bwd_dW1", g, st);
    if (rc) return rc;
  }
  return JH_OK;
}

static int pponet_adam(jh_pponet* n, float max_norm, float* d_norm_out, hipStream_t st, int n_partial = kNormBlocks) {
  JH_LAUNCH(jh_adam_kernel<false>, dim3(kNormBlocks), dim3(256), 0, st, n->n_params, n->params, n->grads, n->m, n->v,
            n->norm_partial, n_partial, n->hyper, max_norm, d_norm_out, (const float*)nullptr, 0, (int64_t)0);
  JH_LAUNCH_CHECK();
  return JH_OK;
}

static bool pponet_adam_fused_ok(const jh_pponet* n, int B) {
  static const bool off = getenv("JH_PMB_NO_FUSED_ADAM") != nullptr;
  const int64_t n_head = (int64_t)n->H * n->S + n->H;
  const int64_t tiles_m = (B + 15) / 16;
  return !off && tiles_m <= 16 && n_head * tiles_m <= 65536 && n_head / 4 <= (int64_t)kNormBlocks * 256;
}
static int pponet_adam_fused(jh_pponet* n, int B, float max_norm, float* d_norm_out, hipStream_t st) {
  const int t32 = n->H / 32;
  JH_LAUNCH(jh_adam_kernel<true>, dim3(kNormBlocks), dim3(256), 0, st, n->n_params, n->params, n->grads, n->m, n->v,
            n->ssq_part, t32 * t32 + t32, n->hyper, max_norm, d_norm_out, (const float*)n->part_w1, (B + 15) / 16,
            (int64_t)n->H * n->S + n->H);
  JH_LAUNCH_CHECK();
  return JH_OK;
}

JH_EXPORT int jh_pponet_adam_step(jh_pponet* n, float max_norm, float* d_norm_out, jh_stream stream) {
  JH_ARG(n != nullptr);
  hipStream_t st = jh_s(stream);
  JH_LAUNCH(jh_gradnorm_kernel, dim3(kNormBlocks), dim3(256), 0, st, n->n_params, n->grads, n->norm_partial, n->hyper);
  JH_LAUNCH_CHECK();
  return pponet_adam(n, max_norm, d_norm_out, st);
}

int jh_ppo_loss_from_partials(jh_ctx* ctx, int continuous, int B, int A, const float* d_hpart, int tiles, int part_rows, int part_ld,
                              const int64_t* d_idx, const float* d_action, const float* d_adv, const float* d_ret,
                              const float* d_value_old, const float* d_logp_old, float eps_clip, float vf_coef, float ent_coef,
                              float* d_g_all, float* d_stats, float* d_hyper_advance, float* d_defer_dv2, float* d_critic_sums, hipStream_t st);
struct jh_peer;
int jh_ppo_critic_select(int B, float* d_sums, float vf, float ent, float* d_gv, int ldv, const float* d_dv2, const float* d_stats_local,
                         float* d_stats_out, hipStream_t st, jh_peer* peer);

JH_EXPORT int jh_pponet_ppo_update(jh_pponet* n, int32_t B, const float* d_x, const int64_t* d_idx, const float* d_action,
                                   const float* d_adv, const float* d_ret, const float* d_value_old,
                                   const float* d_logp_old, float eps_clip, float vf_coef, float ent_coef, float max_norm,
                                   int32_t do_adam, float* d_stats, jh_stream stream) {
  JH_ARG(n && d_x && d_action && d_adv && d_ret && d_value_old && d_logp_old);
  JH_ARG(B > 0 && B <= 1024 && B <= n->max_rows);
  if (!jh_pmb_eligible(n, B)) return jh_fail(JH_ERR_ARG, "jh_pponet_ppo_update needs hidden_size %% 32 == 0 and at most 8 head outputs (H = %d, %d outputs: A + 1 discrete, 2 A + 1 continuous)", n->H, n->n_out);
  hipStream_t st = jh_s(stream);
  int rc = pponet_forward_partials(n, B, d_x, d_idx, st);
  if (rc) return rc;
  const bool fused = do_adam && pponet_adam_fused_ok(n, B);
  rc = jh_ppo_loss_from_partials(n->ctx, n->cont, B, n->A, n->fwd_part, n->H / 16, n->max_rows, (n->cont ? 2 * n->A + 1 : n->A + 1) <= 4 ? 4 : 8, d_idx, d_action, d_adv, d_ret,
                                 d_value_old, d_logp_old, eps_clip, vf_coef, ent_coef, n->g_all, d_stats, fused ? n->hyper : nullptr, nullptr, nullptr, st);
  if (rc) return rc;
  rc = jh_pmb_backward(n, B, d_x, d_idx, pmb_heads(n), fused, st);
  if (rc) return rc;
  if (fused) return pponet_adam_fused(n, B, max_norm, nullptr, st);
  rc = jh_pmb_finalize(n, B, do_adam != 0, st);
  if (rc) return rc;
  return do_adam ? pponet_adam(n, max_norm, nullptr, st) : JH_OK;
}

int jh_ppo_loss_onepass(int continuous, int B, int A, const float* d_head0, const float* d_head1, const float* d_value_pred, const int64_t* d_idx,
                        const float* d_action, const float* d_adv, const float* d_ret, const float* d_value_old, const float* d_logp_old, float eps_clip,
                        float vf_coef, float ent_coef, float* d_g0, float* d_g1, float* d_gv, float* d_dv2, float* d_mix, unsigned* d_ticket, float* d_partial,
                        float* d_stats, hipStream_t st);
JH_EXPORT int jh_pponet_ppo_update_rows(jh_pponet* n, int32_t B, const float* d_x, const int64_t* d_idx, const float* d_action, const float* d_adv,
                                        const float* d_ret, const float* d_value_old, const float* d_logp_old, float eps_clip, float vf_coef, float ent_coef,
                                        float max_norm, int32_t do_adam, float* d_stats, jh_stream stream) {
  JH_ARG(n && d_x && d_action && d_adv && d_ret && d_value_old && d_logp_old);
  JH_ARG(B > 0 && B <= n->max_rows);
  const size_t rows = (size_t)n->max_rows, A = (size_t)n->A;
  float* ws = n->upd_ws;
  float *h0 = ws, *h1 = h0 + rows * A, *hv = h1 + rows * A, *g0 = hv + rows, *g1 = g0 + rows * A, *gv = g1 + rows * A, *dv2 = gv + rows;
  float* partial = dv2 + rows;
  float* mix = partial + 8 * ((rows + 255) / 256);
  unsigned* ticket = reinterpret_cast<unsigned*>(mix + 8);
  int rc = jh_pponet_forward(n, B, d_x, d_idx, h0, n->cont ? h1 : nullptr, hv, stream);
  if (rc) return rc;
  hipStream_t st = jh_s(stream);
  const bool fold = do_adam && max_norm > 0.f && !(getenv("JH_PPO_NORM_FOLD") && atoi(getenv("JH_PPO_NORM_FOLD")) == 0);
  if (B <= 1024) {
    rc = n->cont ? jh_ppo_loss_continuous(n->ctx, B, n->A, h0, h1, hv, d_idx, d_action, d_adv, d_ret, d_value_old, d_logp_old, eps_clip, vf_coef, ent_coef, g0, g1, gv, d_stats, stream)
                 : jh_ppo_loss_discrete(n->ctx, B, n->A, h0, hv, d_idx, d_action, d_adv, d_ret, d_value_old, d_logp_old, eps_clip, vf_coef, ent_coef, g0, gv, d_stats, stream);
    if (rc) return rc;
    rc = pponet_backward(n, B, d_x, d_idx, g0, n->cont ? g1 : nullptr, gv, nullptr, nullptr, st, fold);
  } else {
    const int nb = (B + 255) / 256;
    const bool by_consumer = nb <= 64 && !(getenv("JH_PPO_LOSS_TICKET") && atoi(getenv("JH_PPO_LOSS_TICKET")) != 0);
    rc = jh_ppo_loss_onepass(n->cont, B, n->A, h0, n->cont ? h1 : nullptr, hv, d_idx, d_action, d_adv, d_ret, d_value_old, d_logp_old, eps_clip, vf_coef, ent_coef,
                             g0, n->cont ? g1 : nullptr, gv, dv2, mix, by_consumer ? nullptr : ticket, partial, by_consumer ? nullptr : d_stats, st);
    if (rc) return rc;
    PpoFinish fin{};
    if (by_consumer) { fin.partial = partial; fin.nb = nb; fin.B = B; fin.ent_count = n->cont ? B * n->A : B; fin.vf = vf_coef; fin.ent = ent_coef; fin.stats = d_stats; }
    rc = pponet_backward(n, B, d_x, d_idx, g0, n->cont ? g1 : nullptr, gv, dv2, mix, st, fold, by_consumer ? &fin : nullptr);
  }
  if (rc || !do_adam) return rc;
  if (n->norm_slots > 0) return pponet_adam(n, max_norm, nullptr, st, n->norm_slots);
  return jh_pponet_adam_step(n, max_norm, nullptr, stream);
}

JH_EXPORT int jh_pponet_ppo_update_dp_begin(jh_pponet* n, int32_t B, const float* d_x, const int64_t* d_idx, const float* d_action, const float* d_adv,
                                            const float* d_ret, const float* d_value_old, const float* d_logp_old, float eps_clip, float vf_coef,
                                            float ent_coef, float* d_critic_sums, jh_stream stream) {
  JH_ARG(n && d_x && d_action && d_adv && d_ret && d_value_old && d_logp_old && d_critic_sums);
  JH_ARG(B > 0 && B <= 1024 && B <= n->max_rows);
  if (!jh_pmb_eligible(n, B)) return jh_fail(JH_ERR_ARG, "jh_pponet_ppo_update_dp_begin needs hidden_size %% 32 == 0 and at most 8 head outputs (H = %d, %d outputs: A + 1 discrete, 2 A + 1 continuous)", n->H, n->n_out);
  hipStream_t st = jh_s(stream);
  int rc = pponet_forward_partials(n, B, d_x, d_idx, st);
  if (rc) return rc;
  return jh_ppo_loss_from_partials(n->ctx, n->cont, B, n->A, n->fwd_part, n->H / 16, n->max_rows, (n->cont ? 2 * n->A + 1 : n->A + 1) <= 4 ? 4 : 8, d_idx, d_action, d_adv,
                                   d_ret, d_value_old, d_logp_old, eps_clip, vf_coef, ent_coef, n->g_all, n->stats_tmp, nullptr, n->dv2, d_critic_sums, st);
}

static int pponet_dp_end(jh_pponet* n, jh_peer* peer, int32_t B, const float* d_x, const int64_t* d_idx, float* d_critic_sums, float vf_coef, float ent_coef,
                         float* d_stats, jh_stream stream, const char* who) {
  JH_ARG(n && d_x && d_critic_sums);
  JH_ARG(B > 0 && B <= 1024 && B <= n->max_rows);
  if (!jh_pmb_eligible(n, B))
    return jh_fail(JH_ERR_ARG, "%s needs hidden_size %% 32 == 0 and at most 8 head outputs (H = %d, %d outputs: A + 1 discrete, 2 A + 1 continuous)", who, n->H, n->n_out);
  hipStream_t st = jh_s(stream);
  const int vcol = n->cont ? 2 * n->A : n->A;
  int rc = jh_ppo_critic_select(B, d_critic_sums, vf_coef, ent_coef, n->g_all + vcol, n->gld, n->dv2, n->stats_tmp, d_stats, st, peer);
  if (rc) return rc;
  rc = jh_pmb_backward(n, B, d_x, d_idx, pmb_heads(n), false, st);
  if (rc) return rc;
  return jh_pmb_finalize(n, B, false, st);
}

JH_EXPORT int jh_pponet_ppo_update_dp_end(jh_pponet* n, int32_t B, const float* d_x, const int64_t* d_idx, const float* d_critic_sums, float vf_coef,
                                          float ent_coef, float* d_stats, jh_stream stream) {
  return pponet_dp_end(n, nullptr, B, d_x, d_idx, const_cast<float*>(d_critic_sums), vf_coef, ent_coef, d_stats, stream, "jh_pponet_ppo_update_dp_end");
}

JH_EXPORT int jh_pponet_ppo_update_dp_end_peer(jh_pponet* n, jh_peer* peer, int32_t B, const float* d_x, const int64_t* d_idx, float* d_critic_sums, float vf_coef,
                                               float ent_coef, float* d_stats, jh_stream stream) {
  JH_ARG(peer != nullptr);
  return pponet_dp_end(n, peer, B, d_x, d_idx, d_critic_sums, vf_coef, ent_coef, d_stats, stream, "jh_pponet_ppo_update_dp_end_peer");
}

static inline int pponet_zld(const jh_pponet* n) { return n->n_out <= 8 ? 8 : n->n_out; }
static int pponet_act_raw(jh_pponet* n, int32_t W, const float* h_obs, float* z_out, hipStream_t st) {
  const int H = n->H;
  if (n->n_out > 8) {
    memcpy(n->obs_pin_h, h_obs, sizeof(float) * (size_t)W * n->S);
    const int A = n->A;
    float* d0 = n->act_out_d;
    float* d1 = n->cont ? d0 + (size_t)W * A : nullptr;
    float* dv = d0 + (size_t)(n->cont ? 2 : 1) * W * A;
    int rc = jh_pponet_forward(n, W, n->obs_pin_d, nullptr, d0, d1, dv, (jh_stream)st);
    if (rc) return rc;
    JH_HIP(hipStreamSynchronize(st));
    const float *h0 = n->act_out_h, *h1 = h0 + (size_t)W * A, *hv = h0 + (size_t)(n->cont ? 2 : 1) * W * A;
    for (int wq = 0; wq < W; ++wq) {
      float* z = z_out + (size_t)n->n_out * wq;
      memcpy(z, h0 + (size_t)wq * A, sizeof(float) * A);
      if (n->cont) memcpy(z + A, h1 + (size_t)wq * A, sizeof(float) * A);
      z[n->n_out - 1] = hv[wq];
    }
    return JH_OK;
  }
  const int tiles_n = H / 16, tiles = ((W + 15) / 16) * tiles_n;
  memcpy(n->obs_pin_h, h_obs, sizeof(float) * (size_t)W * n->S);
  const float* w[8]; float* dw[8]; const float* b[8]; float* db[8];
  const int n_out = head_rows(n, w, dw, b, db);
  GemmArgs g{};
  g.M = W; g.N = H; g.K = H; g.B = n->params + n->o_w2; g.ldb = H; g.C = nullptr; g.aux = n->params + n->o_b2;
  g.x = n->obs_pin_d; g.x_rows = nullptr; g.W1 = n->params + n->o_w1; g.b1 = n->params + n->o_b1; g.S = n->S;
  for (int o = 0; o < n_out; ++o) { g.wh[o] = w[o]; g.hbias[o] = b[o]; }
  g.n_out = n_out; g.part = n->part_pin_d; g.part_rows = n->max_act_rows;
  const unsigned seq = ++n->act_seq;
  g.tile_flag = n->flag_pin_d; g.flag_seq = seq;
  int rc = launch_gemm<2, true, EPI_HEADPART, false, 1, 1>("jh_gemm16_act_fused", g, st);
  if (rc) return rc;
  volatile unsigned* flags = n->flag_pin_h;
  bool all = false;
  for (long spin = 0; spin < 50000000L && !all; ++spin) {
    all = true;
    for (int t = 0; t < tiles; ++t)
      if (flags[t] != seq) { all = false; break; }
    if (!all) __builtin_ia32_pause();
  }
  if (!all) {
    JH_HIP(hipStreamSynchronize(st));
    for (int t = 0; t < tiles; ++t)
      if (flags[t] != seq) return jh_fail(JH_ERR_STATE, "acting kernel finished without publishing tile %d", t);
  }
  __atomic_thread_fence(__ATOMIC_ACQUIRE);
  const float* part = n->part_pin_h;
  for (int wq = 0; wq < W; ++wq) {
    float* z = z_out + 8 * (size_t)wq;
    for (int o = 0; o < 8; ++o) z[o] = 0.f;
    for (int t = 0; t < tiles_n; ++t) {
      const float* p = part + ((size_t)t * n->max_act_rows + wq) * 8;
      for (int o = 0; o < n_out; ++o) z[o] += p[o];
    }
  }
  return JH_OK;
}

JH_EXPORT int jh_pponet_act_discrete(jh_pponet* n, int32_t W, const float* h_obs, int64_t* h_action,
                                     float* h_logits_out, float* h_value_out, int32_t training, jh_stream stream) {
  JH_ARG(n && h_obs && h_action);
  JH_ARG(!n->cont);
  JH_ARG(W > 0 && W <= n->max_act_rows);
  const size_t zld = (size_t)pponet_zld(n);
  std::vector<float> z(zld * (size_t)W);
  int rc = pponet_act_raw(n, W, h_obs, z.data(), jh_s(stream));
  if (rc) return rc;
  for (int wq = 0; wq < W; ++wq) {
    h_action[wq] = jh_sample_discrete(n, z.data() + zld * (size_t)wq, wq, training);
    if (h_logits_out) memcpy(h_logits_out + (size_t)wq * n->A, z.data() + zld * (size_t)wq, sizeof(float) * n->A);
    if (h_value_out) h_value_out[wq] = z[zld * (size_t)wq + n->A];
  }
  n->act_ctr += 1;
  return JH_OK;
}

JH_EXPORT int jh_pponet_act_continuous(jh_pponet* n, int32_t W, const float* h_obs, float* h_action, float* h_mu_raw_out,
                                       float* h_log_std_raw_out, float* h_value_out, int32_t training, jh_stream stream) {
  JH_ARG(n && h_obs && h_action);
  JH_ARG(n->cont);
  JH_ARG(W > 0 && W <= n->max_act_rows);
  const size_t zld = (size_t)pponet_zld(n);
  std::vector<float> z(zld * (size_t)W);
// ... 13 lines not shown
```

jorldy_amd/csrc/jh_persist.hip:

```cpp
#if defined(__x86_64__)
#include <emmintrin.h>
#endif

#include "jh_common.h"

typedef float f32x4 __attribute__((ext_vector_type(4)));

struct PersistArgs {
  int W, S, H, n_out, T, G;
  const float *W1, *b1, *W2, *b2;
  const float* wh[12];
  const float* hbias[12];
  const unsigned long long* obs_gran;
  float4* part;
  int rows_ld;
  unsigned* abort_flag;
  unsigned seq0;
  long max_polls;
  unsigned long long* dbg;
  int period;
  unsigned long long* mbox;
  float4* dpart;
  int split;
};
// ... 275 lines not shown
    }
    if (p.dbg && blockIdx.x == 0 && threadIdx.x == 0) { p.dbg[(t - 1) * 8 + 4] = wall_clock64(); p.dbg[(t - 1) * 8 + 5] = __builtin_readcyclecounter(); }
  }
  asm volatile("s_waitcnt vmcnt(0)" ::: "memory");
}

constexpr int kPersistMaxGranules = 512;
struct jh_persist {
  jh_pponet* net = nullptr;
  unsigned long long* gran_h = nullptr;
  unsigned long long* gran_d = nullptr;
  float4 *part_h = nullptr, *part_d = nullptr;
  unsigned *flag_h = nullptr, *flag_d = nullptr;
  unsigned seq = 0;
  int tiles = 0, n_out = 0, G = 0;
  int rows_ld = 16;
  unsigned long long *dbg_h = nullptr, *dbg_d = nullptr;
  unsigned long long* mbox = nullptr;
  float4* dpart = nullptr;
  bool reduced = false;
  int rows_published = 0;
  bool split = false;
};

static int persist_heads(const jh_pponet* n) { return (n->cont ? 2 * n->A : n->A) + 1; }

int jh_persist_create(jh_pponet* n, jh_persist** out) {
  JH_ARG(n && out);
  const int H = n->H, S = n->S;
  JH_ARG(S >= 1 && S <= 16 && (H == 64 || H == 128 || H == 256 || H == 512) && persist_heads(n) <= 12);
  jh_persist* p = new jh_persist();
  p->net = n;
  p->tiles = H / 16;
  p->n_out = persist_heads(n);
  p->G = (p->n_out + 2) / 3;
  JH_HIP(hipHostMalloc((void**)&p->gran_h, sizeof(unsigned long long) * kPersistMaxGranules, hipHostMallocMapped));
  JH_HIP(hipHostGetDevicePointer((void**)&p->gran_d, p->gran_h, 0));
  const size_t part_bytes = sizeof(float4) * 32 * (size_t)p->tiles * p->G;
  JH_HIP(hipHostMalloc((void**)&p->part_h, part_bytes, hipHostMallocMapped));
  memset(p->part_h, 0, part_bytes);
  JH_HIP(hipHostGetDevicePointer((void**)&p->part_d, p->part_h, 0));
  JH_HIP(hipHostMalloc((void**)&p->flag_h, sizeof(unsigned) * 16, hipHostMallocMapped));
  JH_HIP(hipHostGetDevicePointer((void**)&p->flag_d, p->flag_h, 0));
  JH_HIP(hipMalloc((void**)&p->mbox, sizeof(unsigned long long) * kPersistMaxGranules));
  JH_HIP(hipMemset(p->mbox, 0, sizeof(unsigned long long) * kPersistMaxGranules));
  JH_HIP(hipMalloc((void**)&p->dpart, sizeof(float4) * (2 * 4 * 16 * (size_t)p->tiles + 8)));
  JH_HIP(hipMemset(p->dpart, 0, sizeof(float4) * (2 * 4 * 16 * (size_t)p->tiles + 8)));
  memset(p->gran_h, 0, sizeof(unsigned long long) * kPersistMaxGranules);
  memset(p->flag_h, 0, sizeof(unsigned) * 16);
  if (getenv("JH_PERSIST_DEBUG")) {
    p->dbg_h = (unsigned long long*)malloc(sizeof(unsigned long long) * 8 * 4096);
    JH_HIP(hipMalloc((void**)&p->dbg_d, sizeof(unsigned long long) * 8 * 4096));
  }
  p->seq = 1000;
  *out = p;
  return JH_OK;
}

void jh_persist_destroy(jh_persist* p) {
  if (!p) return;
  (void)hipHostFree(p->gran_h);
  (void)hipHostFree(p->part_h);
  (void)hipHostFree(p->flag_h);
  (void)hipFree(p->mbox);
  (void)hipFree(p->dpart);
  if (p->dbg_d) (void)hipFree(p->dbg_d);
  free(p->dbg_h);
  delete p;
}

template <int SP, int NCH>
static void persist_launch(int depth, int pi, int grid, hipStream_t st, const PersistArgs& a) {
  if (pi == 2) JH_LAUNCH_NAMED("jh_act_persist_kernel", (jh_act_persist_kernel<SP, NCH, 4, 2>), dim3(grid), dim3(256), 0, st, a);
  else if (pi == 3) JH_LAUNCH_NAMED("jh_act_persist_kernel", (jh_act_persist_kernel<SP, NCH, 4, 3>), dim3(grid), dim3(256), 0, st, a);
  else if (pi == 4) JH_LAUNCH_NAMED("jh_act_persist_kernel", (jh_act_persist_kernel<SP, NCH, 4, 4>), dim3(grid), dim3(256), 0, st, a);
  else if (depth >= 4) JH_LAUNCH_NAMED("jh_act_persist_kernel", (jh_act_persist_kernel<SP, NCH, 4, 1>), dim3(grid), dim3(256), 0, st, a);
  else if (depth >= 2) JH_LAUNCH_NAMED("jh_act_persist_kernel", (jh_act_persist_kernel<SP, NCH, 2, 1>), dim3(grid), dim3(256), 0, st, a);
  else JH_LAUNCH_NAMED("jh_act_persist_kernel", (jh_act_persist_kernel<SP, NCH, 1, 1>), dim3(grid), dim3(256), 0, st, a);
}

int jh_persist_begin(jh_persist* p, int W, int T, hipStream_t st, int split) {
  jh_pponet* n = p->net;
  JH_ARG(W > 0 && W <= 32 && W * n->S <= kPersistMaxGranules && T > 0 && (!split || W == 32));
  const int win = split ? 16 * n->S : W * n->S;
  const int pi = ((win + 1) / 2 + 63) / 64;
  PersistArgs a{};
  a.W = W; a.S = n->S; a.H = n->H; a.T = T; a.G = p->G;
  a.W1 = n->params + n->o_w1; a.b1 = n->params + n->o_b1; a.W2 = n->params + n->o_w2; a.b2 = n->params + n->o_b2;
  int o = 0;
  for (int k = 0; k < n->A; ++k, ++o) { a.wh[o] = n->params + n->o_wh0 + (int64_t)k * n->H; a.hbias[o] = n->params + n->o_bh0 + k; }
  if (n->cont)
    for (int k = 0; k < n->A; ++k, ++o) { a.wh[o] = n->params + n->o_wh1 + (int64_t)k * n->H; a.hbias[o] = n->params + n->o_bh1 + k; }
  a.wh[o] = n->params + n->o_wv; a.hbias[o] = n->params + n->o_bv; ++o;
  a.n_out = o;
  a.obs_gran = p->gran_d; a.part = p->part_d; a.abort_flag = p->flag_d;
  a.seq0 = p->seq;
  a.dbg = p->dbg_d;
  static const int depth = getenv("JH_PERSIST_DEPTH") ? atoi(getenv("JH_PERSIST_DEPTH")) : 4;
  static const int period = getenv("JH_PERSIST_PERIOD") ? atoi(getenv("JH_PERSIST_PERIOD")) : 10;
  a.period = depth > 1 ? period : 0;
  static const int relay = getenv("JH_PERSIST_RELAY") ? atoi(getenv("JH_PERSIST_RELAY")) : 1;
  a.mbox = relay ? p->mbox : nullptr;
  const int reduce = getenv("JH_PERSIST_REDUCE") ? atoi(getenv("JH_PERSIST_REDUCE")) : (split ? 1 : 0);
  p->reduced = reduce == 1;
  a.dpart = p->reduced ? p->dpart : nullptr;
  a.split = split ? 1 : 0;
  p->split = split != 0;
  a.max_polls = 600000;
  p->flag_h[0] = 0;
  const int nch = n->H / 64;
  const int sp = (n->S + 3) / 4 * 4;
  const int rt = W > 16 ? 2 : 1;
  p->rows_ld = 16 * rt;
  a.rows_ld = p->rows_ld;
  const int grid = p->tiles * rt;
#define JH_PERSIST_CASE(NCH)                                   \
  if (nch == NCH) {                                            \
    if (sp == 4) persist_launch<4, NCH>(depth, pi, grid, st, a);   \
    else if (sp == 8) persist_launch<8, NCH>(depth, pi, grid, st, a);   \
    else if (sp == 12) persist_launch<12, NCH>(depth, pi, grid, st, a); \
    else persist_launch<16, NCH>(depth, pi, grid, st, a);          \
  }
  JH_PERSIST_CASE(1) else JH_PERSIST_CASE(2) else JH_PERSIST_CASE(4) else JH_PERSIST_CASE(8)
#undef JH_PERSIST_CASE
  JH_LAUNCH_CHECK();
  return JH_OK;
}

unsigned jh_persist_publish(jh_persist* p, int W, const float* h_obs) {
  const unsigned tag = ++p->seq;
  p->rows_published = W;
  const int n = W * p->net->S;
  for (int i = 0; i < n; ++i) {
    unsigned bits;
    memcpy(&bits, h_obs + i, 4);
    __atomic_store_n(p->gran_h + i, ((unsigned long long)tag << 32) | bits, __ATOMIC_RELEASE);
  }
  return tag;
}

unsigned jh_persist_seq(const jh_persist* p) { return p->seq; }
void jh_persist_publish_rows(jh_persist* p, int r0, int r1, const float* h_obs, unsigned tag) {
  const int S = p->net->S;
  if (r1 > p->rows_published) p->rows_published = r1;
  for (int i = r0 * S; i < r1 * S; ++i) {
    unsigned bits;
    memcpy(&bits, h_obs + i, 4);
    __atomic_store_n(p->gran_h + i, ((unsigned long long)tag << 32) | bits, __ATOMIC_RELEASE);
  }
  if ((int)(tag - p->seq) > 0) p->seq = tag;
}

static int persist_collect(jh_persist* p, const int* rows, int n_rows, unsigned tag, float* h_heads, int r_first, bool block_order);
int jh_persist_collect_rows(jh_persist* p, const int* rows, int n_rows, unsigned tag, float* h_heads) {
  return persist_collect(p, rows, n_rows, tag, h_heads, 0, !rows && n_rows > 16);
}
int jh_persist_collect_range(jh_persist* p, int r0, int n_rows, unsigned tag, float* h_heads) { return persist_collect(p, nullptr, n_rows, tag, h_heads, r0, true); }
static int persist_collect(jh_persist* p, const int* rows, int n_rows, unsigned tag, float* h_heads, int r_first, bool block_order) {
  const int n_out = p->n_out, G = p->G, ld = p->rows_ld, tiles = p->reduced ? 1 : p->tiles;
  volatile unsigned* abort_w = p->flag_h;
  struct alignas(16) Gran16 { unsigned w[4]; };
  const Gran16* part = reinterpret_cast<const Gran16*>(p->part_h);
  float z[32][12];
  unsigned char have[32];
  JH_ARG(n_rows <= 32);
  if (block_order) {
// ... 102 lines not shown
```

jorldy_amd/csrc/jh_ppo_mb.h:

```cpp
#pragma once
#include "jh_common.h"

struct PmbHeads {
  const float* w[8];
  const float* b[8];
  float* dw[8];
  float* db[8];
  int n_out;
};

bool jh_pmb_eligible(const jh_pponet* n, int B);
int jh_pmb_forward(jh_pponet* n, int M, const float* d_x, const int64_t* d_idx, const PmbHeads& hd, const float* h1_in,
                   bool store_act, hipStream_t st);
int jh_pmb_heads_finish(jh_pponet* n, int M, float* d_head0, float* d_head1, float* d_value, hipStream_t st);
int jh_pmb_backward(jh_pponet* n, int B, const float* d_x, const int64_t* d_idx, const PmbHeads& hd, bool emit_ssq, hipStream_t st);
int jh_pmb_finalize(jh_pponet* n, int B, bool with_norm, hipStream_t st);
```

jorldy_amd/csrc/jh_ppo_mb.hip:

```cpp
#include "jh_ppo_mb.h"

typedef float f32x4 __attribute__((ext_vector_type(4)));

struct PmbFwd {
  int M, H, S;
  const float* x;
  const int64_t* x_rows;
  const float *W1, *b1, *W2, *b2;
  const float* h1_in;
  float* h1_out;
  float* h2_out;
  const float* wh[8];
  const float* hb[8];
  int n_out;
  float* part;
  int part_rows, part_ld;
};

template <int SV, bool GEN, int U>
__global__ void __launch_bounds__(256) jh_pmb_fwd_kernel(PmbFwd g) {
  constexpr bool VEC = SV == 1 || SV == 2;
  constexpr int XS = SV == 3 ? 16 : 8;
  __shared__ float s_acc[4][64][4];
  extern __shared__ __attribute__((aligned(16))) float s_dyn[];
  const int lane = threadIdx.x & 63, wid = threadIdx.x >> 6, r = lane & 15, kq = lane >> 4;
  const int K = g.H, tiles_n = K / 16;
  const int tm = blockIdx.x / tiles_n, tn = blockIdx.x - tm * tiles_n;
  const int m0 = tm * 16, n = tn * 16 + r;
  const int kper = ((K + 63) / 64) * 16, kbeg = wid * kper;
  const int kend = kbeg + kper < K ? kbeg + kper : K;
  const int m = m0 + r;
  const bool m_ok = m < g.M;
  const int mc = m_ok ? m : g.M - 1;
  float xr[XS];
  int64_t row = mc;
  if (GEN && g.x_rows) row = g.x_rows[mc];
  const int ws = SV == 3 ? ((g.S + 3) & ~3) : g.S;
  float* w1s = s_dyn + (size_t)wid * kper * (ws + 1);
  float* b1s = w1s + (size_t)kper * ws;
  const int kn = kend > kbeg ? kend - kbeg : 0;
  constexpr int WB = 4;
  float4 w1t0 = make_float4(0.f, 0.f, 0.f, 0.f), w1t1 = w1t0, w1t2 = w1t0, w1t3 = w1t0, b1t = w1t0;
  const int n_el = kn * g.S;
  const int wi0 = lane * 4 < n_el ? lane * 4 : 0, wi1 = (lane + 64) * 4 < n_el ? (lane + 64) * 4 : 0;
  const int wi2 = (lane + 128) * 4 < n_el ? (lane + 128) * 4 : 0, wi3 = (lane + 192) * 4 < n_el ? (lane + 192) * 4 : 0;
  const int bi0 = 4 * lane < kn ? 4 * lane : 0;
  if (GEN && VEC) {
    const int kb0 = kn > 0 ? kbeg : 0;
    const float* src = g.W1 + (size_t)kb0 * g.S;
    w1t0 = *reinterpret_cast<const float4*>(src + wi0);
    w1t1 = *reinterpret_cast<const float4*>(src + wi1);
    w1t2 = *reinterpret_cast<const float4*>(src + wi2);
    w1t3 = *reinterpret_cast<const float4*>(src + wi3);
    b1t = *reinterpret_cast<const float4*>(g.b1 + kb0 + bi0);
    __builtin_amdgcn_sched_barrier(0);
  }
  if (GEN) {
    if (VEC) {
#pragma unroll
      for (int q = 0; q < SV; ++q) {
        const float4 v = *reinterpret_cast<const float4*>(g.x + row * g.S + 4 * q);
        xr[4 * q] = v.x; xr[4 * q + 1] = v.y; xr[4 * q + 2] = v.z; xr[4 * q + 3] = v.w;
      }
    } else {
#pragma unroll
      for (int s = 0; s < XS; ++s) xr[s] = s < g.S ? g.x[row * g.S + s] : 0.f;
    }
  }
  float4 bw[U];
#pragma unroll
  for (int u = 0; u < U; ++u) {
    const int kb = kbeg + 16 * u + 4 * kq;
    const int kc = kb < kend ? kb : (kbeg < K ? kbeg : 0);
    bw[u] = *reinterpret_cast<const float4*>(g.W2 + (size_t)n * K + kc);
  }
  const float b2 = g.b2[n];
  float whv[8];
#pragma unroll
  for (int o = 0; o < 8; ++o) whv[o] = o < g.n_out ? g.wh[o][n] : 0.f;
  if (GEN) {
    if (VEC) {
      *reinterpret_cast<float4*>(w1s + wi0) = w1t0;
      *reinterpret_cast<float4*>(w1s + wi1) = w1t1;
      *reinterpret_cast<float4*>(w1s + wi2) = w1t2;
      *reinterpret_cast<float4*>(w1s + wi3) = w1t3;
      for (int i = (lane + 64 * WB) * 4; i < n_el; i += 256) *reinterpret_cast<float4*>(w1s + i) = *reinterpret_cast<const float4*>(g.W1 + (size_t)kbeg * g.S + i);
      *reinterpret_cast<float4*>(b1s + bi0) = b1t;
      for (int i = 4 * (lane + 64); i < kn; i += 256) *reinterpret_cast<float4*>(b1s + i) = *reinterpret_cast<const float4*>(g.b1 + kbeg + i);
    } else {
      const float* src = g.W1 + (size_t)kbeg * g.S;
      if (SV == 3) {
        for (int i = lane; i < n_el; i += 64) {
          const int rr = i / g.S, cc = i - rr * g.S;
          w1s[rr * ws + cc] = src[i];
        }
        for (int i = lane; i < kn * (ws - g.S); i += 64) {
          const int rr = i / (ws - g.S), cc = g.S + (i - rr * (ws - g.S));
          w1s[rr * ws + cc] = 0.f;
        }
      } else {
        for (int i = lane; i < n_el; i += 64) w1s[i] = src[i];
      }
      for (int i = lane; i < kn; i += 64) b1s[i] = g.b1[kbeg + i];
    }
    __builtin_amdgcn_wave_barrier();
    __builtin_amdgcn_fence(__ATOMIC_RELEASE, "workgroup");
  }
  f32x4 acc = (f32x4){0.f, 0.f, 0.f, 0.f};
  const bool st_h1 = GEN && g.h1_out && tn == 0;
  for (int k0 = kbeg; k0 < kend; k0 += 16 * U) {
    float4 av[U], bwn[U];
    if (!GEN) {
#pragma unroll
      for (int u = 0; u < U; ++u) {
        const int kb = k0 + 16 * u + 4 * kq;
        const int kc = kb < kend ? kb : kbeg;
        av[u] = *reinterpret_cast<const float4*>(g.h1_in + (size_t)mc * K + kc);
      }
    }
    const bool more = k0 + 16 * U < kend;
    if (more) {
#pragma unroll
      for (int u = 0; u < U; ++u) {
        const int kb = k0 + 16 * U + 16 * u + 4 * kq;
        const int kc = kb < kend ? kb : kbeg;
        bwn[u] = *reinterpret_cast<const float4*>(g.W2 + (size_t)n * K + kc);
      }
    }
#pragma unroll
    for (int u = 0; u < U; ++u) {
      const int kb = k0 + 16 * u + 4 * kq;
      const int kc = kb < kend ? kb : kbeg;
      const bool ok = m_ok && kb < kend;
      if (GEN) {
        const float4 bb = *reinterpret_cast<const float4*>(b1s + (kc - kbeg));
        const float bj[4] = {bb.x, bb.y, bb.z, bb.w};
        float a[4];
#pragma unroll
        for (int j = 0; j < 4; ++j) {
          float t = 0.f;
          if (VEC) {
#pragma unroll
            for (int q = 0; q < SV; ++q) {
              const float4 w = *reinterpret_cast<const float4*>(w1s + (size_t)(kc - kbeg + j) * g.S + 4 * q);
              t = fmaf(xr[4 * q], w.x, t); t = fmaf(xr[4 * q + 1], w.y, t); t = fmaf(xr[4 * q + 2], w.z, t); t = fmaf(xr[4 * q + 3], w.w, t);
            }
          } else if (SV == 3) {
#pragma unroll
            for (int q = 0; q < XS / 4; ++q) {
              if (4 * q < ws) {
                const float4 w = *reinterpret_cast<const float4*>(w1s + (size_t)(kc - kbeg + j) * ws + 4 * q);
                t = fmaf(xr[4 * q], w.x, t); t = fmaf(xr[4 * q + 1], w.y, t); t = fmaf(xr[4 * q + 2], w.z, t); t = fmaf(xr[4 * q + 3], w.w, t);
              }
            }
          } else {
#pragma unroll
            for (int s = 0; s < XS; ++s)
              if (s < g.S) t = fmaf(xr[s], w1s[(size_t)(kc - kbeg + j) * g.S + s], t);
          }
          t += bj[j];
          a[j] = t > 0.f ? t : 0.f;
        }
        av[u] = make_float4(a[0], a[1], a[2], a[3]);
        if (st_h1 && ok) *reinterpret_cast<float4*>(g.h1_out + (size_t)m * K + kb) = av[u];
      }
      if (!ok) av[u] = make_float4(0.f, 0.f, 0.f, 0.f);
    }
#pragma unroll
    for (int u = 0; u < U; ++u) {
      acc = __builtin_amdgcn_mfma_f32_16x16x4f32(av[u].x, bw[u].x, acc, 0, 0, 0);
      acc = __builtin_amdgcn_mfma_f32_16x16x4f32(av[u].y, bw[u].y, acc, 0, 0, 0);
      acc = __builtin_amdgcn_mfma_f32_16x16x4f32(av[u].z, bw[u].z, acc, 0, 0, 0);
      acc = __builtin_amdgcn_mfma_f32_16x16x4f32(av[u].w, bw[u].w, acc, 0, 0, 0);
    }
    if (more) {
#pragma unroll
      for (int u = 0; u < U; ++u) bw[u] = bwn[u];
    }
  }
#pragma unroll
  for (int i = 0; i < 4; ++i) s_acc[wid][lane][i] = acc[i];
  __syncthreads();
  if (wid != 0) return;
  float hv[4];
#pragma unroll
  for (int i = 0; i < 4; ++i) {
    const int mm = m0 + kq * 4 + i;
    float v = ((s_acc[0][lane][i] + s_acc[1][lane][i]) + s_acc[2][lane][i]) + s_acc[3][lane][i];
    v += b2;
    v = v > 0.f ? v : 0.f;
    hv[i] = mm < g.M ? v : 0.f;
    if (mm < g.M && g.h2_out) g.h2_out[(size_t)mm * K + n] = v;
  }
#pragma unroll
  for (int o = 0; o < 8; ++o) {
    if (o >= g.n_out) break;
    const float w = whv[o];
#pragma unroll
    for (int i = 0; i < 4; ++i) {
      float p = hv[i] * w;
      p += __shfl_xor(p, 1, 64);
      p += __shfl_xor(p, 2, 64);
      p += __shfl_xor(p, 4, 64);
      p += __shfl_xor(p, 8, 64);
      const int mm = m0 + kq * 4 + i;
      if (r == 0 && mm < g.M) {
        if (tn == 0) p += *g.hb[o];
        g.part[((size_t)tn * g.part_rows + mm) * g.part_ld + o] = p;
      }
    }
  }
}

__global__ void __launch_bounds__(256) jh_pmb_heads_finish_kernel(int M, int tiles, int part_rows, int part_ld, const float* __restrict__ part,
                                                                  int A, int cont, float* __restrict__ h0, float* __restrict__ h1,
                                                                  float* __restrict__ v) {
  const int i = blockIdx.x * 256 + threadIdx.x;
  if (i >= M) return;
  float z[8] = {0.f, 0.f, 0.f, 0.f, 0.f, 0.f, 0.f, 0.f};
  const bool wide = part_ld == 8;
  for (int t0 = 0; t0 < tiles; t0 += 8) {
    float4 q0[8], q1[8];
#pragma unroll
    for (int u = 0; u < 8; ++u) {
      const int t = t0 + u < tiles ? t0 + u : tiles - 1;
      const float4* q = reinterpret_cast<const float4*>(part + ((size_t)t * part_rows + i) * part_ld);
      q0[u] = q[0];
      if (wide) q1[u] = q[1];
    }
#pragma unroll
    for (int u = 0; u < 8; ++u) {
      if (t0 + u < tiles) {
        z[0] += q0[u].x; z[1] += q0[u].y; z[2] += q0[u].z; z[3] += q0[u].w;
        if (wide) { z[4] += q1[u].x; z[5] += q1[u].y; z[6] += q1[u].z; z[7] += q1[u].w; }
      }
    }
  }
#pragma unroll
  for (int k = 0; k < 8; ++k) {
    if (k < A) h0[(size_t)i * A + k] = z[k];
    if (cont && k >= A && k < 2 * A) h1[(size_t)i * A + (k - A)] = z[k];
    if (k == (cont ? 2 * A : A)) v[i] = z[k];
  }
}

struct PmbBwd {
  int B, H, S, n_out;
  const float* x;
  const int64_t* x_rows;
  const float *h1, *h2, *g_all, *W2;
  const float* wh[8];
  float* dW2;
  float* db2;
  float* dwh[8];
  float* dbh[8];
  float* part_w1;
  int n_dh1, n_dw2;
  float* ssq_part;
};

__device__ __forceinline__ float pmb_wave_sum(float v) {
#pragma unroll
  for (int o = 32; o > 0; o >>= 1) v += __shfl_xor(v, o, 64);
  return v;
}

template <int NO, int U, bool ROWS>
__device__ __forceinline__ void pmb_role_dh1(const PmbBwd& g, int blk, float (*s_acc)[4][64][4], float* s_wh) {
  const int lane = threadIdx.x & 63, wid = threadIdx.x >> 6, r = lane & 15, kq = lane >> 4;
  const int H = g.H, tiles_n = H / 32;
  const int tm = blk / tiles_n, tn = blk - tm * tiles_n;
  const int m0 = tm * 16, i0 = tn * 32;
  const int m = m0 + r;
  const bool m_ok = m < g.B;
  const int mc = m_ok ? m : g.B - 1;
  constexpr int KW = 2;
  const int wk0 = threadIdx.x < H ? threadIdx.x : 0, wk1 = threadIdx.x + 256 < H ? threadIdx.x + 256 : 0;
  float whs[NO][KW];
#pragma unroll
  for (int j = 0; j < NO; ++j) {
    whs[j][0] = whs[j][1] = 0.f;
    if (j < g.n_out) { whs[j][0] = g.wh[j][wk0]; whs[j][1] = g.wh[j][wk1]; }
  }
  float gj[NO];
  {
    const float4 a = *reinterpret_cast<const float4*>(g.g_all + (size_t)mc * 8);
    gj[0] = a.x; gj[1] = a.y; gj[2] = a.z; gj[3] = a.w;
    if (NO > 4) {
      const float4 b = *reinterpret_cast<const float4*>(g.g_all + (size_t)mc * 8 + 4);
      gj[4] = b.x; gj[5] = b.y; gj[6] = b.z; gj[7] = b.w;
    }
// ... 243 lines not shown
    }
  }
  if (g.ssq_part) {
    hsq = pmb_wave_sum(hsq);
    if (lane == 0) g.ssq_part[g.n_dw2 + tm] = hsq;
  }
}

template <int NO, int U1>
__global__ void __launch_bounds__(256) jh_pmb_bwd_kernel(PmbBwd g) {
  __shared__ float s_acc[4][4][64][4];
  __shared__ float s_rs[4][2][64];
  __shared__ float s_hacc[4][2][64][4];
  __shared__ float s_hrs[4][64];
  extern __shared__ __attribute__((aligned(16))) float s_wh[];
  const int b = blockIdx.x;
  if (b < g.n_dh1) {
    if (g.x_rows) pmb_role_dh1<NO, U1, true>(g, b, s_acc, s_wh);
    else pmb_role_dh1<NO, U1, false>(g, b, s_acc, s_wh);
  } else if ((b - g.n_dh1) % (g.H / 32) == 0) {
    pmb_role_dw2<NO, true>(g, b - g.n_dh1, s_acc, s_rs, s_hacc, s_hrs);
  } else {
    pmb_role_dw2<NO, false>(g, b - g.n_dh1, s_acc, s_rs, s_hacc, s_hrs);
  }
}

__global__ void __launch_bounds__(256) jh_pmb_norm_kernel(int64_t n, float* __restrict__ grads, const float* __restrict__ part,
                                                          int tiles_m, int64_t n_head, float* __restrict__ partial,
                                                          float* __restrict__ hyper, int do_norm) {
  __shared__ float s_red[16];
  float acc = 0.f;
  const int64_t n4 = n >> 2, h4 = n_head >> 2;
  const int64_t lim4 = do_norm ? n4 : h4;
  float4* g4 = reinterpret_cast<float4*>(grads);
  const float4* p4 = reinterpret_cast<const float4*>(part);
  for (int64_t i = (int64_t)blockIdx.x * 256 + threadIdx.x; i < lim4; i += (int64_t)gridDim.x * 256) {
    float4 v;
    if (i < h4) {
      v = make_float4(0.f, 0.f, 0.f, 0.f);
      for (int t0 = 0; t0 < tiles_m; t0 += 8) {
        float4 q[8];
#pragma unroll
        for (int u = 0; u < 8; ++u) q[u] = p4[(size_t)(t0 + u < tiles_m ? t0 + u : tiles_m - 1) * h4 + i];
#pragma unroll
        for (int u = 0; u < 8; ++u)
          if (t0 + u < tiles_m) { v.x += q[u].x; v.y += q[u].y; v.z += q[u].z; v.w += q[u].w; }
      }
      g4[i] = v;
    } else {
      v = g4[i];
    }
    acc = fmaf(v.x, v.x, acc); acc = fmaf(v.y, v.y, acc); acc = fmaf(v.z, v.z, acc); acc = fmaf(v.w, v.w, acc);
  }
  if (!do_norm) return;
  if (blockIdx.x == 0 && threadIdx.x < (int)(n - (n4 << 2))) {
    const float v = grads[(n4 << 2) + threadIdx.x];
    acc = fmaf(v, v, acc);
  }
  acc = jh_block_reduce(acc, s_red, JhAdd(), 0.f);
  if (threadIdx.x == 0) partial[blockIdx.x] = acc;
  if (blockIdx.x == 0 && threadIdx.x == 0) jh_adam_advance(hyper);
}

bool jh_pmb_eligible(const jh_pponet* n, int B) { return n->H % 32 == 0 && B > 0 && B <= n->max_rows && n->n_out <= 8; }

template <int SV, bool GEN>
static int pmb_fwd_launch(const PmbFwd& g, hipStream_t st) {
  const int tiles = ((g.M + 15) / 16) * (g.H / 16);
  const int kper = ((g.H + 63) / 64) * 16;
  const double fl = 2.0 * g.M * (double)g.H * ((GEN ? g.S : 0) + g.H + g.n_out);
  const char* nm = g.M > 1024 ? "jh_pmb_fwd_nograd" : "jh_pmb_fwd";
  const size_t lds = GEN ? sizeof(float) * 4 * (size_t)kper * ((SV == 3 ? ((g.S + 3) & ~3) : g.S) + 1) : 0;
  if (kper > 64) JH_LAUNCH_IDEM(nm, fl, (jh_pmb_fwd_kernel<SV, GEN, 8>), dim3(tiles), dim3(256), lds, st, g);
  else if (kper > 32) JH_LAUNCH_IDEM(nm, fl, (jh_pmb_fwd_kernel<SV, GEN, 4>), dim3(tiles), dim3(256), lds, st, g);
  else JH_LAUNCH_IDEM(nm, fl, (jh_pmb_fwd_kernel<SV, GEN, 2>), dim3(tiles), dim3(256), lds, st, g);
  JH_LAUNCH_CHECK();
  return JH_OK;
}

int jh_pmb_forward(jh_pponet* n, int M, const float* d_x, const int64_t* d_idx, const PmbHeads& hd, const float* h1_in,
                   bool store_act, hipStream_t st) {
  PmbFwd g{};
  g.M = M; g.H = n->H; g.S = n->S; g.x = d_x; g.x_rows = d_idx;
  g.W1 = n->params + n->o_w1; g.b1 = n->params + n->o_b1; g.W2 = n->params + n->o_w2; g.b2 = n->params + n->o_b2;
  g.h1_in = h1_in; g.h1_out = store_act ? n->h1 : nullptr; g.h2_out = store_act ? n->h2 : nullptr;
  for (int o = 0; o < hd.n_out; ++o) { g.wh[o] = hd.w[o]; g.hb[o] = hd.b[o]; }
  g.n_out = hd.n_out; g.part = n->fwd_part; g.part_rows = n->max_rows; g.part_ld = hd.n_out <= 4 ? 4 : 8;
  if (h1_in) return pmb_fwd_launch<0, false>(g, st);
  const bool al = (((uintptr_t)d_x) & 15) == 0 && (((uintptr_t)g.W1) & 15) == 0;
  if (n->S == 4 && al) return pmb_fwd_launch<1, true>(g, st);
  if (n->S == 8 && al) return pmb_fwd_launch<2, true>(g, st);
  if (n->S > 8) return pmb_fwd_launch<3, true>(g, st);
  return pmb_fwd_launch<0, true>(g, st);
}

int jh_pmb_heads_finish(jh_pponet* n, int M, float* d_head0, float* d_head1, float* d_value, hipStream_t st) {
  JH_LAUNCH(jh_pmb_heads_finish_kernel, dim3((M + 255) / 256), dim3(256), 0, st, M, n->H / 16, n->max_rows, (n->cont ? 2 * n->A + 1 : n->A + 1) <= 4 ? 4 : 8, n->fwd_part, n->A,
            n->cont, d_head0, d_head1, d_value);
  JH_LAUNCH_CHECK();
  return JH_OK;
}

int jh_pmb_backward(jh_pponet* n, int B, const float* d_x, const int64_t* d_idx, const PmbHeads& hd, bool emit_ssq, hipStream_t st) {
  PmbBwd g{};
  g.B = B; g.H = n->H; g.S = n->S; g.n_out = hd.n_out; g.x = d_x; g.x_rows = d_idx;
  g.h1 = n->h1; g.h2 = n->h2; g.g_all = n->g_all; g.W2 = n->params + n->o_w2;
  g.dW2 = n->grads + n->o_w2; g.db2 = n->grads + n->o_b2;
  for (int o = 0; o < hd.n_out; ++o) { g.wh[o] = hd.w[o]; g.dwh[o] = hd.dw[o]; g.dbh[o] = hd.db[o]; }
  g.part_w1 = n->part_w1;
  g.ssq_part = emit_ssq ? n->ssq_part : nullptr;
  const int t32 = n->H / 32;
  g.n_dh1 = ((B + 15) / 16) * t32;
  g.n_dw2 = t32 * t32;
  const int grid = g.n_dh1 + g.n_dw2;
  static const int u1 = getenv("JH_PMB_U1") ? atoi(getenv("JH_PMB_U1")) : 8;
  const bool deep = u1 >= 8 && n->H >= 512;
  const double fl = 2.0 * B * (double)n->H * (2.0 * n->H + hd.n_out + n->S + 2.0 * hd.n_out);
  if (hd.n_out <= 4) {
    if (deep) JH_LAUNCH_IDEM("jh_pmb_bwd", fl, (jh_pmb_bwd_kernel<4, 8>), dim3(grid), dim3(256), sizeof(float) * 4 * (size_t)n->H, st, g);
    else JH_LAUNCH_IDEM("jh_pmb_bwd", fl, (jh_pmb_bwd_kernel<4, 4>), dim3(grid), dim3(256), sizeof(float) * 4 * (size_t)n->H, st, g);
  } else {
    if (deep) JH_LAUNCH_IDEM("jh_pmb_bwd", fl, (jh_pmb_bwd_kernel<8, 8>), dim3(grid), dim3(256), sizeof(float) * 8 * (size_t)n->H, st, g);
    else JH_LAUNCH_IDEM("jh_pmb_bwd", fl, (jh_pmb_bwd_kernel<8, 4>), dim3(grid), dim3(256), sizeof(float) * 8 * (size_t)n->H, st, g);
  }
  JH_LAUNCH_CHECK();
  return JH_OK;
}

int jh_pmb_finalize(jh_pponet* n, int B, bool with_norm, hipStream_t st) {
  const int64_t n_head = (int64_t)n->H * n->S + n->H;
  const int tiles_m = (B + 15) / 16;
  const int blocks = with_norm ? 256 : (int)((n_head / 4 + 255) / 256);
  JH_LAUNCH(jh_pmb_norm_kernel, dim3(blocks), dim3(256), 0, st, n->n_params, n->grads, n->part_w1, tiles_m, n_head, n->norm_partial,
            n->hyper, with_norm ? 1 : 0);
  JH_LAUNCH_CHECK();
  return JH_OK;
}
```

jorldy_amd/ops.py:

```python
import contextlib
import ctypes as C

import numpy as np
import torch

from . import _lib as L

_DT = {torch.uint8: L.JH_U8, torch.float32: L.JH_F32, torch.int64: L.JH_I64, torch.float64: L.JH_F64, torch.int32: L.JH_I32, torch.bool: L.JH_U8}
_NP_DT = {np.dtype("uint8"): L.JH_U8, np.dtype("float32"): L.JH_F32, np.dtype("int64"): L.JH_I64, np.dtype("float64"): L.JH_F64, np.dtype("int32"): L.JH_I32, np.dtype("bool"): L.JH_U8}
_TORCH_OF = {L.JH_U8: torch.uint8, L.JH_F32: torch.float32, L.JH_I64: torch.int64, L.JH_F64: torch.float64, L.JH_I32: torch.int32}
_NP_OF = {L.JH_U8: np.uint8, L.JH_F32: np.float32, L.JH_I64: np.int64, L.JH_F64: np.float64, L.JH_I32: np.int32}


_PROF = {"on": False, "ev": {}, "lib": False}


class _timed:
    def __init__(self, name, nbytes, bound="hbm"):
        self.name, self.nbytes, self.bound = name, nbytes, bound

    def __enter__(self):
        if _PROF["on"]:
            self.e0 = torch.cuda.Event(enable_timing=True)
            self.e0.record()
# ... 477 lines not shown
        self.dev_ptr = C.c_void_p(d.value)
        buf = (C.c_char * max(n, 8)).from_address(h.value)
        self.np = np.frombuffer(buf, dtype=dtype, count=int(np.prod(shape))).reshape(shape)

    def __del__(self):
        try:
            if getattr(self, "_h", None):
                self.np = None
                self.lib.jh_pinned_free(self._h)
                self._h = None
        except Exception:
            pass


class PPONet:

    def __init__(self, S, H, A, continuous, max_rows, device, seed=0):
        self.lib = L.load()
        self.device = torch.device(device)
        self.ctx = L.ctx(self.device.index)
        self.S, self.H, self.A, self.cont, self.max_rows = int(S), int(H), int(A), bool(continuous), int(max_rows)
        self.n_params = int(self.lib.jh_pponet_param_count(self.S, self.H, self.A, int(self.cont)))
        mk = lambda: torch.zeros(self.n_params, dtype=torch.float32, device=self.device)
        self.params, self.grads, self.m, self.v = mk(), mk(), mk(), mk()
        self.h = C.c_void_p()
        L.check(self.lib.jh_pponet_create(self.ctx, self.S, self.H, self.A, int(self.cont), self.max_rows, L.ptr(self.params), L.ptr(self.grads), L.ptr(self.m), L.ptr(self.v), C.c_uint64(int(seed)), C.byref(self.h)))
        self._act = None

    def __del__(self):
        try:
            if getattr(self, "h", None):
                self.lib.jh_pponet_destroy(self.h)
                self.h = None
        except Exception:
            pass

    def set_hyper(self, lr, beta1=0.9, beta2=0.999, eps=1e-8, step=-1.0):
        L.check(self.lib.jh_pponet_set_hyper(self.h, float(lr), float(beta1), float(beta2), float(eps), float(step), L.stream_ptr()))

    def set_lr(self, lr):
        L.check(self.lib.jh_pponet_set_lr(self.h, float(lr), L.stream_ptr()))

    def hyper_ptr(self):
        return int(self.lib.jh_pponet_hyper_ptr(self.h))

    def act_rng(self, state=None):
        s, c = C.c_uint64(0), C.c_uint64(0)
        if state is not None:
            s, c = C.c_uint64(int(state[0])), C.c_uint64(int(state[1]))
        L.check(self.lib.jh_pponet_act_rng(self.h, C.byref(s), C.byref(c), int(state is not None)))
        return int(s.value), int(c.value)

    def forward(self, x, idx=None, B=None, out=None):
        B = int(idx.numel()) if idx is not None else (int(x.shape[0]) if B is None else int(B))
        if out is None:
            h0 = torch.empty(B, self.A, dtype=torch.float32, device=self.device)
            h1 = torch.empty(B, self.A, dtype=torch.float32, device=self.device) if self.cont else None
            val = torch.empty(B, 1, dtype=torch.float32, device=self.device)
        else:
            h0, h1, val = out
        flops = 2.0 * B * self.H * (self.S + self.H + (2 * self.A + 1 if self.cont else self.A + 1))
        with _timed("jh_pponet_forward", flops, "mfma"):
            L.check(self.lib.jh_pponet_forward(self.h, B, L.ptr(_f32(x)), L.ptr(idx), L.ptr(h0), L.ptr(h1), L.ptr(val), L.stream_ptr()))
        return (h0, h1, val) if self.cont else (h0, val)

    def backward(self, x, idx, g_head0, g_head1, g_value, B=None):
        B = int(idx.numel()) if idx is not None else (int(x.shape[0]) if B is None else int(B))
        flops = 4.0 * B * self.H * (self.S + self.H + (2 * self.A + 1 if self.cont else self.A + 1))
        with _timed("jh_pponet_backward", flops, "mfma"):
            L.check(self.lib.jh_pponet_backward(self.h, B, L.ptr(_f32(x)), L.ptr(idx), L.ptr(g_head0), L.ptr(g_head1), L.ptr(g_value), L.stream_ptr()))

    def adam_step(self, max_norm, norm_out=None):
        with _timed("jh_gradnorm+adam", 4.0 * self.n_params * 8):
            L.check(self.lib.jh_pponet_adam_step(self.h, float(max_norm if max_norm else 0.0), L.ptr(norm_out), L.stream_ptr()))

    def fused_ok(self, B):
        n_out = (2 * self.A + 1) if self.cont else (self.A + 1)
        return self.H % 32 == 0 and 0 < B < 1024 and n_out <= 8

    def ppo_update(self, x, idx, action, adv, ret, value_old, logp_old, eps_clip, vf_coef, ent_coef, max_norm, stats, do_adam=True):
        B = int(idx.numel()) if idx is not None else int(x.shape[0])
        L.check(self.lib.jh_pponet_ppo_update(self.h, B, L.ptr(_f32(x)), L.ptr(idx), L.ptr(_f32(action)), L.ptr(_f32(adv).reshape(-1)), L.ptr(_f32(ret).reshape(-1)),
                                              L.ptr(_f32(value_old).reshape(-1)), L.ptr(_f32(logp_old)), float(eps_clip), float(vf_coef), float(ent_coef),
                                              float(max_norm if max_norm else 0.0), int(bool(do_adam)), L.ptr(stats), L.stream_ptr()))

    def ppo_update_rows(self, x, idx, action, adv, ret, value_old, logp_old, eps_clip, vf_coef, ent_coef, max_norm, stats, do_adam=True):
        B = int(idx.numel()) if idx is not None else int(x.shape[0])
        L.check(self.lib.jh_pponet_ppo_update_rows(self.h, B, L.ptr(_f32(x)), L.ptr(idx), L.ptr(_f32(action)), L.ptr(_f32(adv).reshape(-1)), L.ptr(_f32(ret).reshape(-1)),
                                                   L.ptr(_f32(value_old).reshape(-1)), L.ptr(_f32(logp_old)), float(eps_clip), float(vf_coef), float(ent_coef),
                                                   float(max_norm if max_norm else 0.0), int(bool(do_adam)), L.ptr(stats), L.stream_ptr()))

    def ppo_update_dp(self, x, idx, action, adv, ret, value_old, logp_old, eps_clip, vf_coef, ent_coef, stats, reduce_mean, critic_sums, peer=None):
        B = int(idx.numel()) if idx is not None else int(x.shape[0])
        L.check(self.lib.jh_pponet_ppo_update_dp_begin(self.h, B, L.ptr(_f32(x)), L.ptr(idx), L.ptr(_f32(action)), L.ptr(_f32(adv).reshape(-1)), L.ptr(_f32(ret).reshape(-1)),
                                                       L.ptr(_f32(value_old).reshape(-1)), L.ptr(_f32(logp_old)), float(eps_clip), float(vf_coef), float(ent_coef),
                                                       L.ptr(critic_sums), L.stream_ptr()))
        if peer is not None and B <= 256:
            L.check(self.lib.jh_pponet_ppo_update_dp_end_peer(self.h, peer, B, L.ptr(_f32(x)), L.ptr(idx), L.ptr(critic_sums), float(vf_coef), float(ent_coef), L.ptr(stats), L.stream_ptr()))
            return
        reduce_mean(critic_sums)
        L.check(self.lib.jh_pponet_ppo_update_dp_end(self.h, B, L.ptr(_f32(x)), L.ptr(idx), L.ptr(critic_sums), float(vf_coef), float(ent_coef), L.ptr(stats), L.stream_ptr()))

    def act_discrete(self, obs, training=True, want_logits=False):
        obs = np.ascontiguousarray(obs, dtype=np.float32)
        W = int(obs.shape[0])
        act = np.empty((W, 1), np.int64)
        logits = np.empty((W, self.A), np.float32) if want_logits else None
        val = np.empty((W, 1), np.float32) if want_logits else None
        L.check(self.lib.jh_pponet_act_discrete(self.h, W, L.ptr(obs), L.ptr(act), L.ptr(logits), L.ptr(val), int(bool(training)), L.stream_ptr()))
        return (act, logits, val) if want_logits else act


class NormalSource:

    def __init__(self, device, seed=None):
        self.lib = L.load()
        self.device = torch.device(device)
        self.ctx = L.ctx(self.device.index)
        if seed is None:
            seed = int(torch.randint(0, 2**62, (1,)).item())
        self.state = torch.tensor([int(seed), 0, 0, 0], dtype=torch.int64, device=self.device)

    def fill(self, t):
        assert t.is_cuda and t.dtype == torch.float32 and t.is_contiguous()
        L.check(self.lib.jh_normal_fill(self.ctx, int(t.numel()), L.ptr(t), L.ptr(self.state), L.stream_ptr()))
        return t


def _act_buffers(R, A, dev, eps, u, rand_action, out, want_q_all):
    act, q = (torch.empty(R, dtype=torch.int64, device=dev), torch.empty(R, dtype=torch.float32, device=dev)) if out is None else out
    q_all = torch.empty(R, A, dtype=torch.float32, device=dev) if want_q_all else None
    if eps is not None:
        eps, u, rand_action = (np.ascontiguousarray(eps, dtype=np.float32), np.ascontiguousarray(u, dtype=np.float64), np.ascontiguousarray(rand_action, dtype=np.int64))
        assert eps.size == R and u.size == R and rand_action.size == R
    return act, q, q_all, eps, u, rand_action


def value_act(logits, v_min=0.0, v_max=0.0, eps=None, u=None, rand_action=None, out=None, want_q_all=False):
    lg = _f32(logits)
    N, A, K = (int(v) for v in lg.shape)
    act, q, q_all, eps, u, rand_action = _act_buffers(N, A, lg.device, eps, u, rand_action, out, want_q_all)
    L.check(L.load().jh_value_act(L.ctx(_dev(lg)), N, A, K, L.ptr(lg), float(v_min), float(v_max), L.ptr(eps), L.ptr(u), L.ptr(rand_action), L.ptr(act), L.ptr(q),
                                  L.ptr(q_all), L.stream_ptr()))
    return act, q, q_all


def _pponet_act_continuous(self, obs, training=True, want_heads=False):
    obs = np.ascontiguousarray(obs, dtype=np.float32)
    W = int(obs.shape[0])
    act = np.empty((W, self.A), np.float32)
    mu = np.empty((W, self.A), np.float32) if want_heads else None
    ls = np.empty((W, self.A), np.float32) if want_heads else None
    L.check(self.lib.jh_pponet_act_continuous(self.h, W, L.ptr(obs), L.ptr(act), L.ptr(mu), L.ptr(ls), None, int(bool(training)), L.stream_ptr()))
    return (act, mu, ls) if want_heads else act


PPONet.act_continuous = _pponet_act_continuous


def td_loss(q, q_next_target, action, reward, done, gamma, q_next_online=None, weights=None, alpha=0.0, n_step=0, stats=None):
    lib = L.load()
    q = _f32(q)
    B, A = q.shape
    flags = (L.JH_TD_DOUBLE if q_next_online is not None else 0) | (L.JH_TD_PER if weights is not None else 0)
    g = torch.empty_like(q)
    prio = torch.empty(B, dtype=torch.float32, device=q.device)
    if stats is None:
# ... 626 lines not shown
```

Before: 1.169 million.

## Defer PPO Adam step and fuse it into the next minibatch forward

Adds a deferred optimizer mode for PPO updates. The Adam step from one minibatch is left pending and applied inside the next minibatch's forward kernel, which reads the old params, m and v from one buffer set and writes the updated state into a shadow double buffer. A final flush applies the last pending step. This removes one separate Adam kernel launch and one pass over the parameters per minibatch. In exchange it adds shadow parameter and optimizer-state buffers, pending-state guards on other entry points, and a more complex forward kernel.

```diff
diff --git a/include/jorldy_hip.h b/include/jorldy_hip.h
--- a/include/jorldy_hip.h
+++ b/include/jorldy_hip.h
@@ -195,6 +195,8 @@
                          const float* d_adv, const float* d_ret, const float* d_value_old, const float* d_logp_old,
                          float eps_clip, float vf_coef, float ent_coef, float max_norm, int32_t do_adam, float* d_stats,
                          jh_stream stream);
+int jh_pponet_adam_flush(jh_pponet* n, jh_stream stream);
+int32_t jh_pponet_adam_pending(const jh_pponet* n);
 int jh_pponet_ppo_update_rows(jh_pponet* n, int32_t B, const float* d_x, const int64_t* d_idx, const float* d_action, const float* d_adv, const float* d_ret,
                               const float* d_value_old, const float* d_logp_old, float eps_clip, float vf_coef, float ent_coef, float max_norm,
                               int32_t do_adam, float* d_stats, jh_stream stream);
diff --git a/jorldy_amd/_lib.py b/jorldy_amd/_lib.py
--- a/jorldy_amd/_lib.py
+++ b/jorldy_amd/_lib.py
@@ -109,6 +109,8 @@
     "jh_pponet_backward": (C.c_int, [_vp, _i32, _vp, _vp, _vp, _vp, _vp, _vp]),
     "jh_pponet_adam_step": (C.c_int, [_vp, _f32, _vp, _vp]),
     "jh_pponet_ppo_update": (C.c_int, [_vp, _i32, _vp, _vp, _vp, _vp, _vp, _vp, _vp, _f32, _f32, _f32, _f32, _i32, _vp, _vp]),
+    "jh_pponet_adam_flush": (C.c_int, [_vp, _vp]),
+    "jh_pponet_adam_pending": (_i32, [_vp]),
     "jh_pponet_ppo_update_rows": (C.c_int, [_vp, _i32, _vp, _vp, _vp, _vp, _vp, _vp, _vp, _f32, _f32, _f32, _f32, _i32, _vp, _vp]),
     "jh_ppo_loss_deferred": (C.c_int, [_vp, _i32, _i32, _i32, _vp, _vp, _vp, _vp, _vp, _vp, _vp, _vp, _vp, _f32, _f32, _f32, _vp, _vp, _vp, _vp, _vp, _vp, _vp]),
     "jh_ppo_loss_packed": (C.c_int, [_vp, _i32, _i32, _i32, _vp, _i32, _vp, _vp, _vp, _vp, _vp, _vp, _f32, _f32, _f32, _vp, _vp, _vp, _vp, _vp]),
diff --git a/jorldy_amd/core/agent/ppo.py b/jorldy_amd/core/agent/ppo.py
--- a/jorldy_amd/core/agent/ppo.py
+++ b/jorldy_amd/core/agent/ppo.py
@@ -255,6 +255,7 @@
         tr, adv, ret, logp_old = st["tr"], st["adv"], st["ret"], st["logp_old"]
         k = 0
         if "rows" in st:
+            step = "defer" if self.grad_sync is None else False
             xs, acts, advs, rets, vals, lps = st["rows"](st["idx"])
             exact = self.grad_sync is not None and self.dp_exact_critic
             if exact and "critic_sums" not in st:
@@ -268,11 +269,12 @@
                                           peer=getattr(getattr(self.grad_sync, "transport", None), "peer", None))
                     else:
                         net.ppo_update(xs[o0:o1], None, acts[o0:o1], advs[o0:o1], rets[o0:o1], vals[o0:o1], lps[o0:o1], self.epsilon_clip, self.vf_coef,
-                                       self.ent_coef, self.clip_grad_norm, st["stats"][k], do_adam=self.grad_sync is None)
+                                       self.ent_coef, self.clip_grad_norm, st["stats"][k], do_adam=step)
                     if self.grad_sync is not None:
                         self.grad_sync.reduce_flat(net.grads)
                         net.adam_step(self.clip_grad_norm)
                     k += 1
+            net.adam_flush()
             return
         exact = self.grad_sync is not None and self.dp_exact_critic
         if exact and "dp_work" not in st:
diff --git a/jorldy_amd/csrc/jh_common.h b/jorldy_amd/csrc/jh_common.h
--- a/jorldy_amd/csrc/jh_common.h
+++ b/jorldy_amd/csrc/jh_common.h
@@ -171,7 +171,15 @@
   size_t tg_ws_floats = 0;
   unsigned* tg_cnt = nullptr;
   int tg_cnt_slots = 0;
-};
+  float *sh_params = nullptr, *sh_m = nullptr, *sh_v = nullptr;
+  int cur = 0;
+  int pend = 0;
+  int pend_B = 0;
+  float pend_max_norm = 0.f;
+};
+static inline float* jh_pponet_cur_p(const jh_pponet* n) { return n->cur ? n->sh_params : n->params; }
+static inline float* jh_pponet_cur_m(const jh_pponet* n) { return n->cur ? n->sh_m : n->m; }
+static inline float* jh_pponet_cur_v(const jh_pponet* n) { return n->cur ? n->sh_v : n->v; }
 
 static inline uint64_t jh_mix64(uint64_t x) {
   x += 0x9E3779B97F4A7C15ull;
@@ -287,4 +295,74 @@
 struct JhAdd { template <typename T> __device__ T operator()(T a, T b) const { return a + b; } };
 struct JhMax { template <typename T> __device__ T operator()(T a, T b) const { return a > b ? a : b; } };
 struct JhMin { template <typename T> __device__ T operator()(T a, T b) const { return a < b ? a : b; } };
+
+template <bool FUSED, typename Keep>
+__device__ __forceinline__ float jh_adam_total_norm(const float* __restrict__ partial, int n_partial, const float* __restrict__ part, int tiles_m,
+                                                    int64_t h4, float* s_red, Keep keep) {
+  float acc = 0.f;
+  bool partials_added = false;
+  auto add_partials = [&]() {
+    const int ia = threadIdx.x, ib = threadIdx.x + 256;
+    const float pa = partial[ia < n_partial ? ia : 0], pb = partial[ib < n_partial ? ib : 0];
+    acc += ia < n_partial ? pa : 0.f;
+    acc += ib < n_partial ? pb : 0.f;
+    for (int i = threadIdx.x + 512; i < n_partial; i += 256) acc += partial[i];
+    partials_added = true;
+  };
+  if (FUSED) {
+    const float4* part4 = reinterpret_cast<const float4*>(part);
+    constexpr int JU = 3, TU = 16;
+    for (int64_t j0 = 0; j0 * 256 < h4; j0 += JU) {
+      float4 w[JU][TU];
+#pragma unroll
+      for (int ju = 0; ju < JU; ++ju) {
+        const int64_t i = threadIdx.x + 256 * (j0 + ju);
+        const int64_t ic = i < h4 ? i : h4 - 1;
+#pragma unroll
+        for (int tu = 0; tu < TU; ++tu) w[ju][tu] = part4[(size_t)(tu < tiles_m ? tu : tiles_m - 1) * h4 + ic];
+      }
+      if (!partials_added) add_partials();
+#pragma unroll
+      for (int ju = 0; ju < JU; ++ju) {
+        const int64_t i = threadIdx.x + 256 * (j0 + ju);
+        float4 q = make_float4(0.f, 0.f, 0.f, 0.f);
+#pragma unroll
+        for (int tu = 0; tu < TU; ++tu)
+          if (tu < tiles_m) { q.x += w[ju][tu].x; q.y += w[ju][tu].y; q.z += w[ju][tu].z; q.w += w[ju][tu].w; }
+        if (i < h4) {
+          acc = fmaf(q.x, q.x, acc); acc = fmaf(q.y, q.y, acc); acc = fmaf(q.z, q.z, acc); acc = fmaf(q.w, q.w, acc);
+          keep(i, q);
+        }
+      }
+    }
+  }
+  if (!partials_added) add_partials();
+  return sqrtf(jh_block_reduce(acc, s_red, JhAdd(), 0.f));
+}
+struct JhAdamStep { float coef, b2, eps, omb1, omb2, bc2s, step_size; };
+__device__ __forceinline__ JhAdamStep jh_adam_step_scalars(const float* __restrict__ hyper, float total, float max_norm) {
+  JhAdamStep a;
+  const float bc1 = hyper[JH_HY_BC1];
+  a.bc2s = hyper[JH_HY_BC2S];
+  a.coef = 1.f;
+  if (max_norm > 0.f) a.coef = fminf(max_norm / (total + 1e-6f), 1.f);
+  const float lr = hyper[JH_HY_LR];
+  a.b2 = hyper[JH_HY_B2]; a.eps = hyper[JH_HY_EPS];
+  a.omb1 = hyper[JH_HY_OMB1]; a.omb2 = hyper[JH_HY_OMB2];
+  a.step_size = lr / bc1;
+  return a;
+}
+__device__ __forceinline__ void jh_adam_upd(const JhAdamStep& a, float& pi, float& gi_, float& mi_, float& vi_) {
+  const float gi = gi_ * a.coef;
+  gi_ = gi;
+  const float mi = mi_ + a.omb1 * (gi - mi_);
+  const float vi = vi_ * a.b2 + a.omb2 * gi * gi;
+  mi_ = mi;
+  vi_ = vi;
+  const float denom = sqrtf(vi) / a.bc2s + a.eps;
+  pi = pi - a.step_size * (mi / denom);
+}
+__device__ __forceinline__ void jh_adam_upd4(const JhAdamStep& a, float4& p, float4& g, float4& m, float4& v) {
+  jh_adam_upd(a, p.x, g.x, m.x, v.x); jh_adam_upd(a, p.y, g.y, m.y, v.y); jh_adam_upd(a, p.z, g.z, m.z, v.z); jh_adam_upd(a, p.w, g.w, m.w, v.w);
+}
 #endif
diff --git a/jorldy_amd/csrc/jh_mlp.hip b/jorldy_amd/csrc/jh_mlp.hip
--- a/jorldy_amd/csrc/jh_mlp.hip
+++ b/jorldy_amd/csrc/jh_mlp.hip
@@ -457,86 +457,37 @@
 }
 
 template <bool FUSED>
-__global__ void __launch_bounds__(256) jh_adam_kernel(int64_t n, float* __restrict__ p, float* __restrict__ g,
-                                                      float* __restrict__ m, float* __restrict__ v,
-                                                      const float* __restrict__ partial, int n_partial,
+__global__ void __launch_bounds__(256) jh_adam_kernel(int64_t n, float* p, float* __restrict__ g, float* m, float* v, const float* ps, const float* ms,
+                                                      const float* vs, const float* __restrict__ partial, int n_partial,
                                                       const float* __restrict__ hyper, float max_norm,
                                                       float* __restrict__ norm_out, const float* __restrict__ part,
                                                       int tiles_m, int64_t n_head) {
   __shared__ float s_red[16];
   const int64_t n4 = n >> 2;
   float4 *p4 = reinterpret_cast<float4*>(p), *g4 = reinterpret_cast<float4*>(g), *m4 = reinterpret_cast<float4*>(m), *v4 = reinterpret_cast<float4*>(v);
+  const float4 *ps4 = reinterpret_cast<const float4*>(ps), *ms4 = reinterpret_cast<const float4*>(ms), *vs4 = reinterpret_cast<const float4*>(vs);
   const int64_t i_first = (int64_t)blockIdx.x * 256 + threadIdx.x;
   const int64_t i_fc = i_first < n4 ? i_first : 0;
-  const float4 pp0 = p4[i_fc], mm0 = m4[i_fc], vv0 = v4[i_fc], gg0 = g4[i_fc];
-  float acc = 0.f;
-  bool partials_added = false;
-  auto add_partials = [&]() {
-    const int ia = threadIdx.x, ib = threadIdx.x + 256;
-    const float pa = partial[ia < n_partial ? ia : 0], pb = partial[ib < n_partial ? ib : 0];
-    acc += ia < n_partial ? pa : 0.f;
-    acc += ib < n_partial ? pb : 0.f;
-    for (int i = threadIdx.x + 512; i < n_partial; i += 256) acc += partial[i];
-    partials_added = true;
-  };
+  const float4 pp0 = ps4[i_fc], mm0 = ms4[i_fc], vv0 = vs4[i_fc], gg0 = g4[i_fc];
   float4 mine = make_float4(0.f, 0.f, 0.f, 0.f);
   const int64_t h4 = n_head >> 2;
-  if (FUSED) {
-    const float4* part4 = reinterpret_cast<const float4*>(part);
-    constexpr int JU = 3, TU = 16;
-    for (int64_t j0 = 0; j0 * 256 < h4; j0 += JU) {
-      float4 w[JU][TU];
-#pragma unroll
-      for (int ju = 0; ju < JU; ++ju) {
-        const int64_t i = threadIdx.x + 256 * (j0 + ju);
-        const int64_t ic = i < h4 ? i : h4 - 1;
-#pragma unroll
-        for (int tu = 0; tu < TU; ++tu) w[ju][tu] = part4[(size_t)(tu < tiles_m ? tu : tiles_m - 1) * h4 + ic];
-      }
-      if (!partials_added) add_partials();
-#pragma unroll
-      for (int ju = 0; ju < JU; ++ju) {
-        const int64_t i = threadIdx.x + 256 * (j0 + ju);
-        float4 q = make_float4(0.f, 0.f, 0.f, 0.f);
-#pragma unroll
-        for (int tu = 0; tu < TU; ++tu)
-          if (tu < tiles_m) { q.x += w[ju][tu].x; q.y += w[ju][tu].y; q.z += w[ju][tu].z; q.w += w[ju][tu].w; }
-        if (i < h4) {
-          acc = fmaf(q.x, q.x, acc); acc = fmaf(q.y, q.y, acc); acc = fmaf(q.z, q.z, acc); acc = fmaf(q.w, q.w, acc);
-          if (j0 + ju == blockIdx.x) mine = q;
-        }
-      }
-    }
-  }
-  if (!partials_added) add_partials();
-  const float total = sqrtf(jh_block_reduce(acc, s_red, JhAdd(), 0.f));
-  const float bc1 = hyper[5], bc2s = hyper[6];
-  float coef = 1.f;
-  if (max_norm > 0.f) coef = fminf(max_norm / (total + 1e-6f), 1.f);
+  const float total = jh_adam_total_norm<FUSED>(partial, n_partial, part, tiles_m, h4, s_red, [&](int64_t i, const float4& q) {
+    if ((i >> 8) == blockIdx.x) mine = q;
+  });
+  const JhAdamStep a = jh_adam_step_scalars(hyper, total, max_norm);
   if (blockIdx.x == 0 && threadIdx.x == 0 && norm_out) *norm_out = total;
-  const float lr = hyper[JH_HY_LR], b2 = hyper[JH_HY_B2], eps = hyper[JH_HY_EPS];
-  const float omb1 = hyper[JH_HY_OMB1], omb2 = hyper[JH_HY_OMB2];
-  const float step_size = lr / bc1;
-  auto upd = [&](float& pi, float& gi_, float& mi_, float& vi_) {
-    const float gi = gi_ * coef;
-    gi_ = gi;
-    const float mi = mi_ + omb1 * (gi - mi_);
-    const float vi = vi_ * b2 + omb2 * gi * gi;
-    mi_ = mi;
-    vi_ = vi;
-    const float denom = sqrtf(vi) / bc2s + eps;
-    pi = pi - step_size * (mi / denom);
-  };
   for (int64_t i = i_first; i < n4; i += (int64_t)gridDim.x * 256) {
     const bool first = i == i_first;
-    float4 pp = first ? pp0 : p4[i], mm = first ? mm0 : m4[i], vv = first ? vv0 : v4[i];
+    float4 pp = first ? pp0 : ps4[i], mm = first ? mm0 : ms4[i], vv = first ? vv0 : vs4[i];
     float4 gg = (FUSED && i < h4) ? mine : (first ? gg0 : g4[i]);
-    upd(pp.x, gg.x, mm.x, vv.x); upd(pp.y, gg.y, mm.y, vv.y); upd(pp.z, gg.z, mm.z, vv.z); upd(pp.w, gg.w, mm.w, vv.w);
+    jh_adam_upd4(a, pp, gg, mm, vv);
     p4[i] = pp; g4[i] = gg; m4[i] = mm; v4[i] = vv;
   }
   if (blockIdx.x == 0 && threadIdx.x < (int)(n - (n4 << 2))) {
     const int64_t i = (n4 << 2) + threadIdx.x;
-    upd(p[i], g[i], m[i], v[i]);
+    float pi = ps[i], gi = g[i], mi = ms[i], vi = vs[i];
+    jh_adam_upd(a, pi, gi, mi, vi);
+    p[i] = pi; g[i] = gi; m[i] = mi; v[i] = vi;
   }
 }
 
@@ -626,6 +577,9 @@
     JH_HIP(hipMemset(n->upd_ws, 0, sizeof(float) * n->upd_floats));
   }
   JH_HIP(hipMalloc((void**)&n->norm_partial, sizeof(float) * kNormSlots));
+  JH_HIP(hipMalloc((void**)&n->sh_params, sizeof(float) * 3 * (size_t)((n->n_params + 3) & ~(int64_t)3)));
+  n->sh_m = n->sh_params + ((n->n_params + 3) & ~(int64_t)3);
+  n->sh_v = n->sh_m + ((n->n_params + 3) & ~(int64_t)3);
   JH_HIP(hipMalloc((void**)&n->hyper, sizeof(float) * JH_HY_FLOATS));
   float hy[JH_HY_FLOATS];
   jh_hyper_fill(hy, 1e-3, 0.9, 0.999, 1e-8, 0.0);
@@ -644,7 +598,7 @@
   if (n->act_out_h) (void)hipHostFree(n->act_out_h);
   (void)hipFree(n->norm_partial); (void)hipFree(n->hyper); (void)hipFree(n->dv2);
   (void)hipFree(n->fwd_part); (void)hipFree(n->part_w1); (void)hipFree(n->ssq_part);
-  (void)hipFree(n->tg_ws); (void)hipFree(n->tg_cnt); (void)hipFree(n->xg); (void)hipFree(n->upd_ws);
+  (void)hipFree(n->tg_ws); (void)hipFree(n->tg_cnt); (void)hipFree(n->xg); (void)hipFree(n->upd_ws); (void)hipFree(n->sh_params);
   delete n;
 }
 
@@ -735,11 +689,15 @@
 constexpr int kTiledRows = 1024;
 static inline bool pponet_use_tiled(int B) { return B >= kTiledRows; }
 
-static PmbHeads pmb_heads(jh_pponet* n) {
+static PmbHeads pmb_heads(jh_pponet* n, const float* params = nullptr) {
   PmbHeads hd{};
   hd.n_out = head_rows(n, hd.w, hd.dw, hd.b, hd.db);
+  if (params && params != n->params)
+    for (int o = 0; o < hd.n_out; ++o) { hd.w[o] = params + (hd.w[o] - n->params); hd.b[o] = params + (hd.b[o] - n->params); }
   return hd;
 }
+#define JH_NO_PENDING(n, what) \
+  if ((n)->pend) return jh_fail(JH_ERR_STATE, what ": a deferred optimizer step is pending (jh_pponet_ppo_update with do_adam == 2): call jh_pponet_adam_flush first")
 
 __global__ void __launch_bounds__(256) jh_rowgather_f32_kernel(int B, int S, const float* __restrict__ x, const int64_t* __restrict__ idx, float* __restrict__ out) {
   const int64_t i = (int64_t)blockIdx.x * 256 + threadIdx.x;
@@ -1013,6 +971,7 @@
   JH_ARG(n && d_x && d_head0 && d_value);
   JH_ARG(B > 0 && B <= n->max_rows);
   JH_ARG(!n->cont || d_head1);
+  JH_NO_PENDING(n, "jh_pponet_forward");
   hipStream_t st = jh_s(stream);
   const int H = n->H;
   static const int kFwdTiledRows = getenv("JH_PPO_FWD_TILED_ROWS") ? atoi(getenv("JH_PPO_FWD_TILED_ROWS")) : 2048;
@@ -1051,6 +1010,7 @@
   JH_ARG(n && d_x && d_g_head0 && d_g_value);
   JH_ARG(B > 0 && B <= n->max_rows);
   JH_ARG(!n->cont || d_g_head1);
+  JH_NO_PENDING(n, "jh_pponet_backward");
   return pponet_backward(n, B, d_x, d_idx, d_g_head0, d_g_head1, d_g_value, nullptr, nullptr, jh_s(stream));
 }
 static int pponet_backward(jh_pponet* n, int32_t B, const float* d_x, const int64_t* d_idx, const float* d_g_head0, const float* d_g_head1,
@@ -1132,7 +1092,7 @@
 
 static int pponet_adam(jh_pponet* n, float max_norm, float* d_norm_out, hipStream_t st, int n_partial = kNormBlocks) {
   JH_LAUNCH(jh_adam_kernel<false>, dim3(kNormBlocks), dim3(256), 0, st, n->n_params, n->params, n->grads, n->m, n->v,
-            n->norm_partial, n_partial, n->hyper, max_norm, d_norm_out, (const float*)nullptr, 0, (int64_t)0);
+            (const float*)n->params, (const float*)n->m, (const float*)n->v, (const float*)n->norm_partial, n_partial, n->hyper, max_norm, d_norm_out, (const float*)nullptr, 0, (int64_t)0);
   JH_LAUNCH_CHECK();
   return JH_OK;
 }
@@ -1146,7 +1106,7 @@
 static int pponet_adam_fused(jh_pponet* n, int B, float max_norm, float* d_norm_out, hipStream_t st) {
   const int t32 = n->H / 32;
   JH_LAUNCH(jh_adam_kernel<true>, dim3(kNormBlocks), dim3(256), 0, st, n->n_params, n->params, n->grads, n->m, n->v,
-            n->ssq_part, t32 * t32 + t32, n->hyper, max_norm, d_norm_out, (const float*)n->part_w1, (B + 15) / 16,
+            (const float*)jh_pponet_cur_p(n), (const float*)jh_pponet_cur_m(n), (const float*)jh_pponet_cur_v(n), (const float*)n->ssq_part, t32 * t32 + t32, n->hyper, max_norm, d_norm_out, (const float*)n->part_w1, (B + 15) / 16,
             (int64_t)n->H * n->S + n->H);
   JH_LAUNCH_CHECK();
   return JH_OK;
@@ -1154,6 +1114,7 @@
 
 JH_EXPORT int jh_pponet_adam_step(jh_pponet* n, float max_norm, float* d_norm_out, jh_stream stream) {
   JH_ARG(n != nullptr);
+  JH_NO_PENDING(n, "jh_pponet_adam_step");
   hipStream_t st = jh_s(stream);
   JH_LAUNCH(jh_gradnorm_kernel, dim3(kNormBlocks), dim3(256), 0, st, n->n_params, n->grads, n->norm_partial, n->hyper);
   JH_LAUNCH_CHECK();
@@ -1168,22 +1129,54 @@
 int jh_ppo_critic_select(int B, float* d_sums, float vf, float ent, float* d_gv, int ldv, const float* d_dv2, const float* d_stats_local,
                          float* d_stats_out, hipStream_t st, jh_peer* peer);
 
+static bool pponet_adam_fused_ok(const jh_pponet* n, int B);
+static int pponet_adam_fused(jh_pponet* n, int B, float max_norm, float* d_norm_out, hipStream_t st);
+JH_EXPORT int jh_pponet_adam_flush(jh_pponet* n, jh_stream stream) {
+  JH_ARG(n != nullptr);
+  if (!n->pend) return JH_OK;
+  const int rc = pponet_adam_fused(n, n->pend_B, n->pend_max_norm, nullptr, jh_s(stream));
+  if (rc) return rc;
+  n->pend = 0;
+  n->cur = 0;
+  return JH_OK;
+}
+JH_EXPORT int32_t jh_pponet_adam_pending(const jh_pponet* n) { return n && n->pend ? 1 : 0; }
+
 JH_EXPORT int jh_pponet_ppo_update(jh_pponet* n, int32_t B, const float* d_x, const int64_t* d_idx, const float* d_action,
                                    const float* d_adv, const float* d_ret, const float* d_value_old,
                                    const float* d_logp_old, float eps_clip, float vf_coef, float ent_coef, float max_norm,
                                    int32_t do_adam, float* d_stats, jh_stream stream) {
   JH_ARG(n && d_x && d_action && d_adv && d_ret && d_value_old && d_logp_old);
   JH_ARG(B > 0 && B <= 1024 && B <= n->max_rows);
+  JH_ARG(do_adam >= 0 && do_adam <= 2);
   if (!jh_pmb_eligible(n, B)) return jh_fail(JH_ERR_ARG, "jh_pponet_ppo_update needs hidden_size %% 32 == 0 and at most 8 head outputs (H = %d, %d outputs: A + 1 discrete, 2 A + 1 continuous)", n->H, n->n_out);
   hipStream_t st = jh_s(stream);
-  int rc = pponet_forward_partials(n, B, d_x, d_idx, st);
+  const bool defer = do_adam == 2 && pponet_adam_fused_ok(n, B) && jh_pmb_defer_eligible(n);
+  int rc;
+  if (do_adam == 2 && !defer) {
+    rc = jh_pponet_adam_flush(n, stream);
+    if (rc) return rc;
+  }
+  if (!defer) { JH_NO_PENDING(n, "jh_pponet_ppo_update (do_adam 0 / 1)"); }
+  if (defer && n->pend) {
+    const float* src = jh_pponet_cur_p(n);
+    n->cur ^= 1;
+    rc = jh_pmb_forward_deferred(n, B, d_x, d_idx, pmb_heads(n, src), n->pend_B, n->pend_max_norm, st);
+    n->pend = 0;
+  } else {
+    rc = pponet_forward_partials(n, B, d_x, d_idx, st);
+  }
   if (rc) return rc;
   const bool fused = do_adam && pponet_adam_fused_ok(n, B);
   rc = jh_ppo_loss_from_partials(n->ctx, n->cont, B, n->A, n->fwd_part, n->H / 16, n->max_rows, (n->cont ? 2 * n->A + 1 : n->A + 1) <= 4 ? 4 : 8, d_idx, d_action, d_adv, d_ret,
                                  d_value_old, d_logp_old, eps_clip, vf_coef, ent_coef, n->g_all, d_stats, fused ? n->hyper : nullptr, nullptr, nullptr, st);
   if (rc) return rc;
-  rc = jh_pmb_backward(n, B, d_x, d_idx, pmb_heads(n), fused, st);
-  if (rc) return rc;
+  rc = jh_pmb_backward(n, B, d_x, d_idx, pmb_heads(n, jh_pponet_cur_p(n)), fused, st);
+  if (rc) return rc;
+  if (defer) {
+    n->pend = 1; n->pend_B = B; n->pend_max_norm = max_norm;
+    return JH_OK;
+  }
   if (fused) return pponet_adam_fused(n, B, max_norm, nullptr, st);
   rc = jh_pmb_finalize(n, B, do_adam != 0, st);
   if (rc) return rc;
@@ -1199,6 +1192,7 @@
                                         float max_norm, int32_t do_adam, float* d_stats, jh_stream stream) {
   JH_ARG(n && d_x && d_action && d_adv && d_ret && d_value_old && d_logp_old);
   JH_ARG(B > 0 && B <= n->max_rows);
+  JH_NO_PENDING(n, "jh_pponet_ppo_update_rows");
   const size_t rows = (size_t)n->max_rows, A = (size_t)n->A;
   float* ws = n->upd_ws;
   float *h0 = ws, *h1 = h0 + rows * A, *hv = h1 + rows * A, *g0 = hv + rows, *g1 = g0 + rows * A, *gv = g1 + rows * A, *dv2 = gv + rows;
@@ -1235,6 +1229,7 @@
   JH_ARG(n && d_x && d_action && d_adv && d_ret && d_value_old && d_logp_old && d_critic_sums);
   JH_ARG(B > 0 && B <= 1024 && B <= n->max_rows);
   if (!jh_pmb_eligible(n, B)) return jh_fail(JH_ERR_ARG, "jh_pponet_ppo_update_dp_begin needs hidden_size %% 32 == 0 and at most 8 head outputs (H = %d, %d outputs: A + 1 discrete, 2 A + 1 continuous)", n->H, n->n_out);
+  JH_NO_PENDING(n, "jh_pponet_ppo_update_dp_begin");
   hipStream_t st = jh_s(stream);
   int rc = pponet_forward_partials(n, B, d_x, d_idx, st);
   if (rc) return rc;
@@ -1270,6 +1265,7 @@
 
 static inline int pponet_zld(const jh_pponet* n) { return n->n_out <= 8 ? 8 : n->n_out; }
 static int pponet_act_raw(jh_pponet* n, int32_t W, const float* h_obs, float* z_out, hipStream_t st) {
+  JH_NO_PENDING(n, "jh_pponet_act_*");
   const int H = n->H;
   if (n->n_out > 8) {
     memcpy(n->obs_pin_h, h_obs, sizeof(float) * (size_t)W * n->S);
diff --git a/jorldy_amd/csrc/jh_persist.hip b/jorldy_amd/csrc/jh_persist.hip
--- a/jorldy_amd/csrc/jh_persist.hip
+++ b/jorldy_amd/csrc/jh_persist.hip
@@ -381,6 +381,7 @@
 int jh_persist_begin(jh_persist* p, int W, int T, hipStream_t st, int split) {
   jh_pponet* n = p->net;
   JH_ARG(W > 0 && W <= 32 && W * n->S <= kPersistMaxGranules && T > 0 && (!split || W == 32));
+  if (n->pend) return jh_fail(JH_ERR_STATE, "jh_persist_begin: a deferred optimizer step is pending (jh_pponet_ppo_update with do_adam == 2): call jh_pponet_adam_flush first");
   const int win = split ? 16 * n->S : W * n->S;
   const int pi = ((win + 1) / 2 + 63) / 64;
   PersistArgs a{};
diff --git a/jorldy_amd/csrc/jh_ppo_mb.h b/jorldy_amd/csrc/jh_ppo_mb.h
--- a/jorldy_amd/csrc/jh_ppo_mb.h
+++ b/jorldy_amd/csrc/jh_ppo_mb.h
@@ -12,6 +12,8 @@
 bool jh_pmb_eligible(const jh_pponet* n, int B);
 int jh_pmb_forward(jh_pponet* n, int M, const float* d_x, const int64_t* d_idx, const PmbHeads& hd, const float* h1_in,
                    bool store_act, hipStream_t st);
+bool jh_pmb_defer_eligible(const jh_pponet* n);
+int jh_pmb_forward_deferred(jh_pponet* n, int M, const float* d_x, const int64_t* d_idx, const PmbHeads& hd, int pend_B, float max_norm, hipStream_t st);
 int jh_pmb_heads_finish(jh_pponet* n, int M, float* d_head0, float* d_head1, float* d_value, hipStream_t st);
 int jh_pmb_backward(jh_pponet* n, int B, const float* d_x, const int64_t* d_idx, const PmbHeads& hd, bool emit_ssq, hipStream_t st);
 int jh_pmb_finalize(jh_pponet* n, int B, bool with_norm, hipStream_t st);
diff --git a/jorldy_amd/csrc/jh_ppo_mb.hip b/jorldy_amd/csrc/jh_ppo_mb.hip
--- a/jorldy_amd/csrc/jh_ppo_mb.hip
+++ b/jorldy_amd/csrc/jh_ppo_mb.hip
@@ -16,6 +16,41 @@
   float* part;
   int part_rows, part_ld;
 };
+
+template <int SV>
+__device__ __forceinline__ float4 pmb_l1_quad(const float* xr, const float* w1s, const float* b1s, int k, int S, int ws) {
+  constexpr bool VEC = SV == 1 || SV == 2;
+  constexpr int XS = SV == 3 ? 16 : 8;
+  const float4 bb = *reinterpret_cast<const float4*>(b1s + k);
+  const float bj[4] = {bb.x, bb.y, bb.z, bb.w};
+  float a[4];
+#pragma unroll
+  for (int j = 0; j < 4; ++j) {
+    float t = 0.f;
+    if (VEC) {
+#pragma unroll
+      for (int q = 0; q < SV; ++q) {
+        const float4 w = *reinterpret_cast<const float4*>(w1s + (size_t)(k + j) * S + 4 * q);
+        t = fmaf(xr[4 * q], w.x, t); t = fmaf(xr[4 * q + 1], w.y, t); t = fmaf(xr[4 * q + 2], w.z, t); t = fmaf(xr[4 * q + 3], w.w, t);
+      }
+    } else if (SV == 3) {
+#pragma unroll
+      for (int q = 0; q < XS / 4; ++q) {
+        if (4 * q < ws) {
+          const float4 w = *reinterpret_cast<const float4*>(w1s + (size_t)(k + j) * ws + 4 * q);
+          t = fmaf(xr[4 * q], w.x, t); t = fmaf(xr[4 * q + 1], w.y, t); t = fmaf(xr[4 * q + 2], w.z, t); t = fmaf(xr[4 * q + 3], w.w, t);
+        }
+      }
+    } else {
+#pragma unroll
+      for (int s = 0; s < XS; ++s)
+        if (s < S) t = fmaf(xr[s], w1s[(size_t)(k + j) * S + s], t);
+    }
+    t += bj[j];
+    a[j] = t > 0.f ? t : 0.f;
+  }
+  return make_float4(a[0], a[1], a[2], a[3]);
+}
 
 template <int SV, bool GEN, int U>
 __global__ void __launch_bounds__(256) jh_pmb_fwd_kernel(PmbFwd g) {
@@ -133,35 +168,7 @@
       const int kc = kb < kend ? kb : kbeg;
       const bool ok = m_ok && kb < kend;
       if (GEN) {
-        const float4 bb = *reinterpret_cast<const float4*>(b1s + (kc - kbeg));
-        const float bj[4] = {bb.x, bb.y, bb.z, bb.w};
-        float a[4];
-#pragma unroll
-        for (int j = 0; j < 4; ++j) {
-          float t = 0.f;
-          if (VEC) {
-#pragma unroll
-            for (int q = 0; q < SV; ++q) {
-              const float4 w = *reinterpret_cast<const float4*>(w1s + (size_t)(kc - kbeg + j) * g.S + 4 * q);
-              t = fmaf(xr[4 * q], w.x, t); t = fmaf(xr[4 * q + 1], w.y, t); t = fmaf(xr[4 * q + 2], w.z, t); t = fmaf(xr[4 * q + 3], w.w, t);
-            }
-          } else if (SV == 3) {
-#pragma unroll
-            for (int q = 0; q < XS / 4; ++q) {
-              if (4 * q < ws) {
-                const float4 w = *reinterpret_cast<const float4*>(w1s + (size_t)(kc - kbeg + j) * ws + 4 * q);
-                t = fmaf(xr[4 * q], w.x, t); t = fmaf(xr[4 * q + 1], w.y, t); t = fmaf(xr[4 * q + 2], w.z, t); t = fmaf(xr[4 * q + 3], w.w, t);
-              }
-            }
-          } else {
-#pragma unroll
-            for (int s = 0; s < XS; ++s)
-              if (s < g.S) t = fmaf(xr[s], w1s[(size_t)(kc - kbeg + j) * g.S + s], t);
-          }
-          t += bj[j];
-          a[j] = t > 0.f ? t : 0.f;
-        }
-        av[u] = make_float4(a[0], a[1], a[2], a[3]);
+        av[u] = pmb_l1_quad<SV>(xr, w1s, b1s, kc - kbeg, g.S, ws);
         if (st_h1 && ok) *reinterpret_cast<float4*>(g.h1_out + (size_t)m * K + kb) = av[u];
       }
       if (!ok) av[u] = make_float4(0.f, 0.f, 0.f, 0.f);
@@ -207,6 +214,231 @@
       if (r == 0 && mm < g.M) {
         if (tn == 0) p += *g.hb[o];
         g.part[((size_t)tn * g.part_rows + mm) * g.part_ld + o] = p;
+      }
+    }
+  }
+}
+
+struct PmbDef {
+  const float *p, *m, *v;
+  float *po, *mo, *vo;
+  const float* grads;
+  const float* ssq;
+  int n_ssq;
+  const float* part;
+  int tiles_m;
+  const float* hyper;
+  float max_norm;
+};
+
+template <int SV, int U>
+__global__ void __launch_bounds__(256) jh_pmb_fwd_def_kernel(PmbFwd g, PmbDef d) {
+  constexpr bool VEC = SV == 1 || SV == 2;
+  __shared__ float s_acc[2][4][64][4];
+  __shared__ float s_red[16];
+  extern __shared__ __attribute__((aligned(16))) float s_dyn[];
+  const int lane = threadIdx.x & 63, wid = threadIdx.x >> 6, r = lane & 15, kq = lane >> 4;
+  const int K = g.H, tiles_n = K / 16;
+  const int tp = blockIdx.x / tiles_n, tn = blockIdx.x - tp * tiles_n;
+  const int n = tn * 16 + r;
+  const int kper = ((K + 63) / 64) * 16, kbeg = wid * kper;
+  const int kend = kbeg + kper < K ? kbeg + kper : K;
+  const int kn = kend > kbeg ? kend - kbeg : 0;
+  const bool wr_col = tp == 0, wr_all = blockIdx.x == 0;
+  const int64_t n_head = (int64_t)K * g.S + K, h4 = n_head >> 2;
+  float* s_g1 = s_dyn;
+  float* w1s = s_dyn + n_head + (size_t)wid * kper * (g.S + 1);
+  float* b1s = w1s + (size_t)kper * g.S;
+  int m0[2], mrow[2];
+  bool m_ok[2];
+  int64_t row[2];
+#pragma unroll
+  for (int t = 0; t < 2; ++t) {
+    m0[t] = (2 * tp + t) * 16;
+    mrow[t] = m0[t] + r;
+    m_ok[t] = mrow[t] < g.M;
+    const int mc = m_ok[t] ? mrow[t] : g.M - 1;
+    row[t] = g.x_rows ? g.x_rows[mc] : (int64_t)mc;
+  }
+  const int n_el = kn * g.S;
+  const int kb0 = kn > 0 ? kbeg : 0;
+  int64_t ew[4];
+  bool ew_ok[4];
+#pragma unroll
+  for (int q = 0; q < 4; ++q) {
+    const int i = (lane + 64 * q) * 4;
+    ew_ok[q] = i < n_el;
+    ew[q] = (int64_t)kb0 * g.S + (ew_ok[q] ? i : 0);
+  }
+  const bool eb_ok = 4 * lane < kn;
+  const int64_t eb = (int64_t)K * g.S + kb0 + (eb_ok ? 4 * lane : 0);
+  float4 wp[4], wm[4], wv[4], bp1, bm1, bv1;
+  if (VEC) {
+#pragma unroll
+    for (int q = 0; q < 4; ++q) {
+      wp[q] = *reinterpret_cast<const float4*>(d.p + ew[q]);
+      wm[q] = *reinterpret_cast<const float4*>(d.m + ew[q]);
+      wv[q] = *reinterpret_cast<const float4*>(d.v + ew[q]);
+    }
+    bp1 = *reinterpret_cast<const float4*>(d.p + eb);
+    bm1 = *reinterpret_cast<const float4*>(d.m + eb);
+    bv1 = *reinterpret_cast<const float4*>(d.v + eb);
+  }
+  float xr[2][8];
+#pragma unroll
+  for (int t = 0; t < 2; ++t) {
+    if (VEC) {
+#pragma unroll
+      for (int q = 0; q < SV; ++q) {
+        const float4 v = *reinterpret_cast<const float4*>(g.x + row[t] * g.S + 4 * q);
+        xr[t][4 * q] = v.x; xr[t][4 * q + 1] = v.y; xr[t][4 * q + 2] = v.z; xr[t][4 * q + 3] = v.w;
+      }
+    } else {
+#pragma unroll
+      for (int s = 0; s < 8; ++s) xr[t][s] = s < g.S ? g.x[row[t] * g.S + s] : 0.f;
+    }
+  }
+  const int64_t o_w2 = g.W2 - d.p;
+  float4 bw[U], bg[U], bm[U], bv[U];
+#pragma unroll
+  for (int u = 0; u < U; ++u) {
+    const int kb = kbeg + 16 * u + 4 * kq;
+    const int kc = kb < kend ? kb : (kbeg < K ? kbeg : 0);
+    const int64_t e = o_w2 + (int64_t)n * K + kc;
+    bw[u] = *reinterpret_cast<const float4*>(d.p + e);
+    bg[u] = *reinterpret_cast<const float4*>(d.grads + e);
+    bm[u] = *reinterpret_cast<const float4*>(d.m + e);
+    bv[u] = *reinterpret_cast<const float4*>(d.v + e);
+  }
+  const int64_t e_b2 = (g.b2 - d.p) + n;
+  float b2 = d.p[e_b2], b2g = d.grads[e_b2], b2m = d.m[e_b2], b2v = d.v[e_b2];
+  float whv[8], whg[8], whm[8], whvv[8], hbp[8], hbg[8], hbm[8], hbv[8];
+#pragma unroll
+  for (int o = 0; o < 8; ++o) {
+    whv[o] = whg[o] = whm[o] = whvv[o] = hbp[o] = hbg[o] = hbm[o] = hbv[o] = 0.f;
+    if (o < g.n_out) {
+      const int64_t e = (g.wh[o] - d.p) + n, eh = g.hb[o] - d.p;
+      whv[o] = d.p[e]; whg[o] = d.grads[e]; whm[o] = d.m[e]; whvv[o] = d.v[e];
+      hbp[o] = d.p[eh]; hbg[o] = d.grads[eh]; hbm[o] = d.m[eh]; hbv[o] = d.v[eh];
+    }
+  }
+  const float total = jh_adam_total_norm<true>(d.ssq, d.n_ssq, d.part, d.tiles_m, h4, s_red, [&](int64_t i, const float4& q) {
+    reinterpret_cast<float4*>(s_g1)[i] = q;
+  });
+  const JhAdamStep a = jh_adam_step_scalars(d.hyper, total, d.max_norm);
+  if (VEC) {
+#pragma unroll
+    for (int q = 0; q < 4; ++q) {
+      float4 gq = *reinterpret_cast<const float4*>(s_g1 + ew[q]);
+      jh_adam_upd4(a, wp[q], gq, wm[q], wv[q]);
+      *reinterpret_cast<float4*>(w1s + (ew[q] - (int64_t)kb0 * g.S)) = wp[q];
+      if (wr_all && ew_ok[q]) {
+        *reinterpret_cast<float4*>(d.po + ew[q]) = wp[q];
+        *reinterpret_cast<float4*>(d.mo + ew[q]) = wm[q];
+        *reinterpret_cast<float4*>(d.vo + ew[q]) = wv[q];
+      }
+    }
+    float4 gq = *reinterpret_cast<const float4*>(s_g1 + eb);
+    jh_adam_upd4(a, bp1, gq, bm1, bv1);
+    *reinterpret_cast<float4*>(b1s + (eb - (int64_t)K * g.S - kb0)) = bp1;
+    if (wr_all && eb_ok) {
+      *reinterpret_cast<float4*>(d.po + eb) = bp1;
+      *reinterpret_cast<float4*>(d.mo + eb) = bm1;
+      *reinterpret_cast<float4*>(d.vo + eb) = bv1;
+    }
+  } else {
+    for (int i = lane; i < n_el + kn; i += 64) {
+      const int64_t e = i < n_el ? (int64_t)kbeg * g.S + i : (int64_t)K * g.S + kbeg + (i - n_el);
+      float pi = d.p[e], gi = s_g1[e], mi = d.m[e], vi = d.v[e];
+      jh_adam_upd(a, pi, gi, mi, vi);
+      if (i < n_el) w1s[i] = pi;
+      else b1s[i - n_el] = pi;
+      if (wr_all) { d.po[e] = pi; d.mo[e] = mi; d.vo[e] = vi; }
+    }
+  }
+  __builtin_amdgcn_wave_barrier();
+  __builtin_amdgcn_fence(__ATOMIC_RELEASE, "workgroup");
+#pragma unroll
+  for (int u = 0; u < U; ++u) {
+    const int kb = kbeg + 16 * u + 4 * kq;
+    jh_adam_upd4(a, bw[u], bg[u], bm[u], bv[u]);
+    if (wr_col && kb < kend) {
+      const int64_t e = o_w2 + (int64_t)n * K + kb;
+      *reinterpret_cast<float4*>(d.po + e) = bw[u];
+      *reinterpret_cast<float4*>(d.mo + e) = bm[u];
+      *reinterpret_cast<float4*>(d.vo + e) = bv[u];
+    }
+  }
+  jh_adam_upd(a, b2, b2g, b2m, b2v);
+  const bool wr_n = wr_col && wid == 0 && kq == 0;
+  if (wr_n) { d.po[e_b2] = b2; d.mo[e_b2] = b2m; d.vo[e_b2] = b2v; }
+#pragma unroll
+  for (int o = 0; o < 8; ++o) {
+    if (o < g.n_out) {
+      jh_adam_upd(a, whv[o], whg[o], whm[o], whvv[o]);
+      jh_adam_upd(a, hbp[o], hbg[o], hbm[o], hbv[o]);
+      if (wr_n) {
+        const int64_t e = (g.wh[o] - d.p) + n;
+        d.po[e] = whv[o]; d.mo[e] = whm[o]; d.vo[e] = whvv[o];
+      }
+      if (wr_all && threadIdx.x == 0) {
+        const int64_t eh = g.hb[o] - d.p;
+        d.po[eh] = hbp[o]; d.mo[eh] = hbm[o]; d.vo[eh] = hbv[o];
+      }
+    }
+  }
+  f32x4 acc[2] = {(f32x4){0.f, 0.f, 0.f, 0.f}, (f32x4){0.f, 0.f, 0.f, 0.f}};
+  const bool st_h1 = g.h1_out && tn == 0;
+#pragma unroll
+  for (int u = 0; u < U; ++u) {
+    const int kb = kbeg + 16 * u + 4 * kq;
+    const int kc = kb < kend ? kb : kbeg;
+#pragma unroll
+    for (int t = 0; t < 2; ++t) {
+      const bool ok = m_ok[t] && kb < kend;
+      float4 av = pmb_l1_quad<SV>(xr[t], w1s, b1s, kc - kbeg, g.S, g.S);
+      if (st_h1 && ok) *reinterpret_cast<float4*>(g.h1_out + (size_t)mrow[t] * K + kb) = av;
+      if (!ok) av = make_float4(0.f, 0.f, 0.f, 0.f);
+      acc[t] = __builtin_amdgcn_mfma_f32_16x16x4f32(av.x, bw[u].x, acc[t], 0, 0, 0);
+      acc[t] = __builtin_amdgcn_mfma_f32_16x16x4f32(av.y, bw[u].y, acc[t], 0, 0, 0);
+      acc[t] = __builtin_amdgcn_mfma_f32_16x16x4f32(av.z, bw[u].z, acc[t], 0, 0, 0);
+      acc[t] = __builtin_amdgcn_mfma_f32_16x16x4f32(av.w, bw[u].w, acc[t], 0, 0, 0);
+    }
+  }
+#pragma unroll
+  for (int t = 0; t < 2; ++t)
+#pragma unroll
+    for (int i = 0; i < 4; ++i) s_acc[t][wid][lane][i] = acc[t][i];
+  __syncthreads();
+  if (wid != 0) return;
+#pragma unroll
+  for (int t = 0; t < 2; ++t) {
+    float hv[4];
+#pragma unroll
+    for (int i = 0; i < 4; ++i) {
+      const int mm = m0[t] + kq * 4 + i;
+      float v = ((s_acc[t][0][lane][i] + s_acc[t][1][lane][i]) + s_acc[t][2][lane][i]) + s_acc[t][3][lane][i];
+      v += b2;
+      v = v > 0.f ? v : 0.f;
+      hv[i] = mm < g.M ? v : 0.f;
+      if (mm < g.M && g.h2_out) g.h2_out[(size_t)mm * K + n] = v;
+    }
+#pragma unroll
+    for (int o = 0; o < 8; ++o) {
+      if (o >= g.n_out) break;
+      const float w = whv[o];
+#pragma unroll
+      for (int i = 0; i < 4; ++i) {
+        float p = hv[i] * w;
+        p += __shfl_xor(p, 1, 64);
+        p += __shfl_xor(p, 2, 64);
+        p += __shfl_xor(p, 4, 64);
+        p += __shfl_xor(p, 8, 64);
+        const int mm = m0[t] + kq * 4 + i;
+        if (r == 0 && mm < g.M) {
+          if (tn == 0) p += hbp[o];
+          g.part[((size_t)tn * g.part_rows + mm) * g.part_ld + o] = p;
+        }
       }
     }
   }
@@ -616,7 +848,8 @@
                    bool store_act, hipStream_t st) {
   PmbFwd g{};
   g.M = M; g.H = n->H; g.S = n->S; g.x = d_x; g.x_rows = d_idx;
-  g.W1 = n->params + n->o_w1; g.b1 = n->params + n->o_b1; g.W2 = n->params + n->o_w2; g.b2 = n->params + n->o_b2;
+  const float* params = jh_pponet_cur_p(n);
+  g.W1 = params + n->o_w1; g.b1 = params + n->o_b1; g.W2 = params + n->o_w2; g.b2 = params + n->o_b2;
   g.h1_in = h1_in; g.h1_out = store_act ? n->h1 : nullptr; g.h2_out = store_act ? n->h2 : nullptr;
   for (int o = 0; o < hd.n_out; ++o) { g.wh[o] = hd.w[o]; g.hb[o] = hd.b[o]; }
   g.n_out = hd.n_out; g.part = n->fwd_part; g.part_rows = n->max_rows; g.part_ld = hd.n_out <= 4 ? 4 : 8;
@@ -628,6 +861,40 @@
   return pmb_fwd_launch<0, true>(g, st);
 }
 
+bool jh_pmb_defer_eligible(const jh_pponet* n) { return n->S <= 8 && n->H <= 512 && n->H % 32 == 0 && n->n_out <= 8 && n->o_w1 == 0 && n->o_b1 == (int64_t)n->H * n->S; }
+
+template <int SV>
+static int pmb_fwd_def_launch(const PmbFwd& g, const PmbDef& d, hipStream_t st) {
+  const int tiles = (((g.M + 15) / 16 + 1) / 2) * (g.H / 16);
+  const int kper = ((g.H + 63) / 64) * 16;
+  const double fl = 2.0 * g.M * (double)g.H * (g.S + g.H + g.n_out);
+  const size_t lds = sizeof(float) * ((size_t)g.H * (g.S + 1) + 4 * (size_t)kper * (g.S + 1));
+  if (kper > 64) JH_LAUNCH_IDEM("jh_pmb_fwd_def", fl, (jh_pmb_fwd_def_kernel<SV, 8>), dim3(tiles), dim3(256), lds, st, g, d);
+  else if (kper > 32) JH_LAUNCH_IDEM("jh_pmb_fwd_def", fl, (jh_pmb_fwd_def_kernel<SV, 4>), dim3(tiles), dim3(256), lds, st, g, d);
+  else JH_LAUNCH_IDEM("jh_pmb_fwd_def", fl, (jh_pmb_fwd_def_kernel<SV, 2>), dim3(tiles), dim3(256), lds, st, g, d);
+  JH_LAUNCH_CHECK();
+  return JH_OK;
+}
+
+int jh_pmb_forward_deferred(jh_pponet* n, int M, const float* d_x, const int64_t* d_idx, const PmbHeads& hd, int pend_B, float max_norm, hipStream_t st) {
+  PmbDef d{};
+  d.po = jh_pponet_cur_p(n); d.mo = jh_pponet_cur_m(n); d.vo = jh_pponet_cur_v(n);
+  d.p = n->cur ? n->params : n->sh_params; d.m = n->cur ? n->m : n->sh_m; d.v = n->cur ? n->v : n->sh_v;
+  d.grads = n->grads; d.ssq = n->ssq_part; d.n_ssq = (n->H / 32) * (n->H / 32) + n->H / 32;
+  d.part = n->part_w1; d.tiles_m = (pend_B + 15) / 16; d.hyper = n->hyper; d.max_norm = max_norm;
+  PmbFwd g{};
+  g.M = M; g.H = n->H; g.S = n->S; g.x = d_x; g.x_rows = d_idx;
+  g.W1 = d.p + n->o_w1; g.b1 = d.p + n->o_b1; g.W2 = d.p + n->o_w2; g.b2 = d.p + n->o_b2;
+  g.h1_out = n->h1; g.h2_out = n->h2;
+  for (int o = 0; o < hd.n_out; ++o) { g.wh[o] = hd.w[o]; g.hb[o] = hd.b[o]; }
+  g.n_out = hd.n_out; g.part = n->fwd_part; g.part_rows = n->max_rows; g.part_ld = hd.n_out <= 4 ? 4 : 8;
+  const uintptr_t bits = (uintptr_t)d_x | (uintptr_t)d.p | (uintptr_t)d.m | (uintptr_t)d.v | (uintptr_t)d.po | (uintptr_t)d.mo | (uintptr_t)d.vo | (uintptr_t)d.grads;
+  const bool al = (bits & 15) == 0;
+  if (n->S == 4 && al) return pmb_fwd_def_launch<1>(g, d, st);
+  if (n->S == 8 && al) return pmb_fwd_def_launch<2>(g, d, st);
+  return pmb_fwd_def_launch<0>(g, d, st);
+}
+
 int jh_pmb_heads_finish(jh_pponet* n, int M, float* d_head0, float* d_head1, float* d_value, hipStream_t st) {
   JH_LAUNCH(jh_pmb_heads_finish_kernel, dim3((M + 255) / 256), dim3(256), 0, st, M, n->H / 16, n->max_rows, (n->cont ? 2 * n->A + 1 : n->A + 1) <= 4 ? 4 : 8, n->fwd_part, n->A,
             n->cont, d_head0, d_head1, d_value);
@@ -638,7 +905,7 @@
 int jh_pmb_backward(jh_pponet* n, int B, const float* d_x, const int64_t* d_idx, const PmbHeads& hd, bool emit_ssq, hipStream_t st) {
   PmbBwd g{};
   g.B = B; g.H = n->H; g.S = n->S; g.n_out = hd.n_out; g.x = d_x; g.x_rows = d_idx;
-  g.h1 = n->h1; g.h2 = n->h2; g.g_all = n->g_all; g.W2 = n->params + n->o_w2;
+  g.h1 = n->h1; g.h2 = n->h2; g.g_all = n->g_all; g.W2 = jh_pponet_cur_p(n) + n->o_w2;
   g.dW2 = n->grads + n->o_w2; g.db2 = n->grads + n->o_b2;
   for (int o = 0; o < hd.n_out; ++o) { g.wh[o] = hd.w[o]; g.dwh[o] = hd.dw[o]; g.dbh[o] = hd.db[o]; }
   g.part_w1 = n->part_w1;
diff --git a/jorldy_amd/ops.py b/jorldy_amd/ops.py
--- a/jorldy_amd/ops.py
+++ b/jorldy_amd/ops.py
@@ -583,7 +583,14 @@
         B = int(idx.numel()) if idx is not None else int(x.shape[0])
         L.check(self.lib.jh_pponet_ppo_update(self.h, B, L.ptr(_f32(x)), L.ptr(idx), L.ptr(_f32(action)), L.ptr(_f32(adv).reshape(-1)), L.ptr(_f32(ret).reshape(-1)),
                                               L.ptr(_f32(value_old).reshape(-1)), L.ptr(_f32(logp_old)), float(eps_clip), float(vf_coef), float(ent_coef),
-                                              float(max_norm if max_norm else 0.0), int(bool(do_adam)), L.ptr(stats), L.stream_ptr()))
+                                              float(max_norm if max_norm else 0.0), 2 if do_adam == "defer" else int(bool(do_adam)), L.ptr(stats), L.stream_ptr()))
+
+    def adam_flush(self):
+        L.check(self.lib.jh_pponet_adam_flush(self.h, L.stream_ptr()))
+
+    @property
+    def adam_pending(self):
+        return bool(self.lib.jh_pponet_adam_pending(self.h))
 
     def ppo_update_rows(self, x, idx, action, adv, ret, value_old, logp_old, eps_clip, vf_coef, ent_coef, max_norm, stats, do_adam=True):
         B = int(idx.numel()) if idx is not None else int(x.shape[0])
```

Measured after the change: 1.035 million. -11.5%, worse.
